# aleju/face-generator

Hardware: NVIDIA H100
Metric: 32x32 GAN train images/sec (1 D-iter + 1 G-iter per batch, batch 256/GPU) (higher is better)
Workload: dtype f32

## Files before the change

face_generator_b200/csrc/capi.cu:

```cuda
#include <algorithm>
#include <cstdarg>
#include <cstdlib>
#include <cstring>

#include "fg_internal.h"
#include "k_conv_tc.h"

static thread_local char g_err[1024] = "";
void fg_set_error(const char* fmt, ...) {
  va_list ap;
  va_start(ap, fmt);
  vsnprintf(g_err, sizeof(g_err), fmt, ap);
  va_end(ap);
}

#define ENTER(c)                                      \
  do {                                                \
    if (!(c)) {                                       \
      fg_set_error("null fg_ctx");                    \
      return FG_ERR_INVALID;                          \
    }                                                 \
    FG_CUDA(cudaSetDevice((c)->device));              \
  } while (0)

bool fg_is_dev(const void* p) {
  cudaPointerAttributes a;
  if (cudaPointerGetAttributes(&a, p) != cudaSuccess) {
    cudaGetLastError();
    return false;
  }
  return a.type == cudaMemoryTypeDevice || a.type == cudaMemoryTypeManaged;
}
int fg_to_dev(fg_ctx* c, const float* p, size_t n, float* staging, const float** out) {
  if (fg_is_dev(p)) {
    *out = p;
    return FG_OK;
  }
  FG_CUDA(cudaMemcpyAsync(staging, p, n * sizeof(float), cudaMemcpyHostToDevice, c->stream));
  *out = staging;
  return FG_OK;
}
int fg_to_user(fg_ctx* c, float* dst, const float* src_dev, size_t n) {
  if (dst == src_dev) return FG_OK;
  const bool dev = fg_is_dev(dst);
  FG_CUDA(cudaMemcpyAsync(dst, src_dev, n * sizeof(float), dev ? cudaMemcpyDeviceToDevice : cudaMemcpyDeviceToHost,
                          c->stream));
  if (!dev) FG_CUDA(cudaStreamSynchronize(c->stream));
  return FG_OK;
}
int64_t debug_tensor_copy(fg_ctx* c, const char* what, const DebugTensor* ents, size_t n_ents, const char* name, float* dst,
                          int64_t max_elems) {
  for (size_t i = 0; i < n_ents; ++i) {
    const DebugTensor& e = ents[i];
    if (strcmp(e.name, name)) continue;
    const int64_t n = e.per * e.B;
    if (!e.p) {
      fg_set_error("%s: '%s' has not been produced (Dstep.*: option \"debug_keep\" + a train step)", what, name);
      return -1;
    }
    if (dst) {
      if (n > max_elems) return -2;
      if (fg_to_user(c, dst, e.p, n) != FG_OK) return -3;
    }
    return n;
  }
  fg_set_error("%s: unknown tensor '%s'", what, name);
  return -1;
}

namespace {
int ctx_alloc(fg_ctx* c) {
  const size_t B = c->maxB, C = c->C;
  auto dalloc = [c](auto** p, size_t n) { return fg_dalloc(c, c->allocs, reinterpret_cast<float**>(p), n); };
  FG_TRY(dalloc(&c->lop_sx, 2));
  FG_TRY(dalloc(&c->lop_sy, 2));
  FG_TRY(dalloc(&c->seed_dev, 2 * kMaxIters));
  c->splitk_ws_elems = (size_t)c->sm_count * 4 * 128 * 128;
  FG_TRY(dalloc(&c->splitk_ws, c->splitk_ws_elems));
  c->red_ws_elems = (size_t)4 << 20;
  FG_TRY(dalloc(&c->red_ws, 2 * c->red_ws_elems));
  FG_TRY(dalloc(&c->red_ws_opt, 2 * kOptRedRows));
  FG_TRY(dalloc(&c->red_ticket, 2));
  FG_TRY(dalloc(&c->bwd_claim, 1));
  FG_TRY(dalloc(&c->small_ws, (size_t)kSmallMaxParts * 9 * 4 * 128));
  FG_TRY(dalloc(&c->bn_acc, 4 * 256 * 2));
  FG_TRY(dalloc(&c->bn_slice_acc, 32 * 4 * 256 * 2 + 64));
  FG_TRY(dalloc(&c->bn_parts, B * 3072));
  c->io_dev_elems = std::max<size_t>(B * 1024 * C, B * kMaskPerSample);
  return dalloc(&c->io_dev, c->io_dev_elems);
}
void ctx_free(fg_ctx* c) {
  for (void* p : c->allocs) cudaFree(p);
  c->allocs.clear();
  for (int i = 0; i < 8; ++i)
    if (c->scratch[i]) cudaFree(c->scratch[i]);
}
}

extern "C" {

const char* fg_version(void) { return "fg_b200 0.1 (sm_90a)"; }
const char* fg_last_error(void) { return g_err; }

void fg_hyper_default(fg_hyper* h) {
  if (!h) return;
  h->lr_D = 1e-3f; h->lr_G = 1e-3f;
  h->beta1 = 0.9f; h->beta2 = 0.999f; h->eps = 1e-8f;
  h->D_L1 = 0.f; h->D_L2 = 1e-4f;
  h->G_L1 = 0.f; h->G_L2 = 0.f;
  h->D_clamp = 1.f; h->G_clamp = 5.f;
  h->D_maxAcc = 1.01f;
  h->accs_interval = 20;
  h->p_spatial = 0.2f; h->p_drop = 0.5f;
}

int fg_create(fg_ctx** out, int device, int max_batch, int channels) {
  if (!out) { fg_set_error("fg_create: out is null"); return FG_ERR_INVALID; }
  *out = nullptr;
  FG_REQUIRE(channels == 1 || channels == 3, "fg_create: channels must be 1 or 3 (got %d)", channels);
  FG_REQUIRE(max_batch >= 4 && max_batch % 2 == 0, "fg_create: max_batch must be even and >= 4 (got %d)", max_batch);
  int ndev = 0;
  FG_CUDA(cudaGetDeviceCount(&ndev));
  FG_REQUIRE(device >= 0 && device < ndev, "fg_create: device %d not present (%d CUDA devices); there is no CPU fallback",
             device, ndev);
  FG_CUDA(cudaSetDevice(device));
  cudaDeviceProp prop;
  FG_CUDA(cudaGetDeviceProperties(&prop, device));
  if (prop.major != 9 || prop.minor != 0) {
    fg_set_error("fg_create: device %d is sm_%d%d; this library only contains sm_90a code", device, prop.major, prop.minor);
    return FG_ERR_UNSUPPORTED;
  }
  fg_ctx* c = new fg_ctx();
  c->device = device;
  c->maxB = max_batch;
  c->C = channels;
  c->sm_count = prop.multiProcessorCount;
  if (const char* e = getenv("FG_MMA_F16")) c->mma_f16 = atoi(e) != 0;
  if (const char* e = getenv("FG_DP_OVERLAP")) c->dp_overlap = atoi(e) != 0;
  if (cudaStreamCreateWithFlags(&c->stream, cudaStreamNonBlocking) != cudaSuccess) {
    fg_set_error("fg_create: cudaStreamCreate failed");
    delete c;
    return FG_ERR_CUDA;
  }
  int r = ctx_alloc(c);
  if (r == FG_OK) r = net32_alloc(c);
  if (r == FG_OK) r = tc_init(c);
  if (r != FG_OK) {
    net32_free(c);
    ctx_free(c);
    cudaStreamDestroy(c->stream);
    delete c;
    return r;
  }
  *out = c;
  return FG_OK;
}

int fg_destroy(fg_ctx* c) {
  if (!c) return FG_OK;
  cudaSetDevice(c->device);
  cudaStreamSynchronize(c->stream);
  if (c->comm_stream) {
    cudaStreamSynchronize(c->comm_stream);
    cudaStreamDestroy(c->comm_stream);
    cudaEventDestroy(c->ev_fork);
    cudaEventDestroy(c->ev_join);
  }
  tc_destroy(c);
  net32_free(c);
  ctx_free(c);
  for (auto& kv : c->timers)
    for (auto& pr : kv.second.pending) {
      cudaEventDestroy(pr.first);
      cudaEventDestroy(pr.second);
    }
  if (c->own_stream && c->stream) cudaStreamDestroy(c->stream);
  delete c;
  return FG_OK;
}

int fg_set_stream(fg_ctx* c, void* s) {
  ENTER(c);
  c->graph_epoch++;
  FG_CUDA(cudaStreamSynchronize(c->stream));
  if (s) {
    if (c->own_stream) cudaStreamDestroy(c->stream);
    c->stream = (cudaStream_t)s;
    c->own_stream = false;
  } else if (!c->own_stream) {
    FG_CUDA(cudaStreamCreateWithFlags(&c->stream, cudaStreamNonBlocking));
    c->own_stream = true;
  }
  return FG_OK;
}
int fg_sync(fg_ctx* c) {
  ENTER(c);
  FG_CUDA(cudaStreamSynchronize(c->stream));
  return FG_OK;
}
int fg_set_option(fg_ctx* c, const char* key, int64_t v) {
  ENTER(c);
  c->graph_epoch++;
  if (!strcmp(key, "conv_impl")) {
    FG_REQUIRE(v >= 0 && v <= 2, "conv_impl must be 0 (simt), 1 (tc dense) or 2 (tc collapsed)");
    c->conv_impl = (int)v;
    return FG_OK;
  }
  if (!strcmp(key, "params_dirty")) {
    NetPair& p = net32_pair(c);
    p.G_pack = p.D_pack = -1;
// ... 185 lines not shown
```

face_generator_b200/csrc/convl.cu:

```cuda
#include "convl.h"

#include "k_conv_tc.h"
#include "k_misc.h"

int convl_dalloc(ConvLEnv& e, float** p, size_t elems) { return fg_dalloc(e.c, *e.allocs, p, elems); }

int ScalePairs::alloc(fg_ctx* c, std::vector<void*>& allocs, int pairs) {
  n = pairs;
  used = 0;
  return fg_dalloc(c, allocs, &base, 2 * (size_t)pairs);
}
int ScalePairs::take(float** pair) {
  if (used == n) {
    fg_set_error("a block of %d FP16 scale pairs is full", n);
    return FG_ERR_UNSUPPORTED;
  }
  *pair = base + 2 * used++;
  return FG_OK;
}
int ScalePairs::reset(fg_ctx* c) const {
  if (!tc_f16(c)) return FG_OK;
  FG_CUDA(cudaMemset2DAsync(base, 2 * sizeof(float), 0, sizeof(float), n, c->stream));
  return FG_OK;
}

namespace {
inline bool tc_f(const fg_ctx* c, const ConvL& L, int B) { return c->conv_impl != FG_CONV_SIMT && tc_conv_eligible(L.geom_k(B)); }
inline bool tc_d(const fg_ctx* c, const ConvL& L, int B) { return c->conv_impl != FG_CONV_SIMT && tc_conv_eligible(L.geom_d(B)); }
inline bool tc_w(const fg_ctx* c, const ConvL& L, int B) { return tc_f(c, L, B) && L.Cout % 128 == 0 && L.geom_k(B).Cin % 64 == 0; }
}

bool convl_tc_fwd(const fg_ctx* c, const ConvL& L) { return tc_f(c, L, 1); }
bool convl_tc_bwd(const fg_ctx* c, const ConvL& L) { return tc_f(c, L, 1) && tc_d(c, L, 1); }

int tc_op_split(fg_ctx* c, TcOp& op, const float* x, int64_t n, bool f16) {
  if (!f16) {
    if (op.split_ready) {
      op.split_ready = false;
      return FG_OK;
    }
    return tc_split(c, x, op.hi, op.lo, n);
  }
  if (op.amax_ready) op.amax_ready = false;
  else FG_TRY(tc_amax(c, x, n, op.s));
  return tc_split_h(c, x, op.hi, op.lo, n, op.s);
}

int convl_alloc(ConvLEnv& e, ConvL& L) {
  const size_t nw = (size_t)L.k * L.k * L.Cout * L.Cin;
  FG_TRY(convl_dalloc(e, &L.Wp, nw));
  FG_TRY(convl_dalloc(e, &L.Wpd, nw));
  if (L.nA) FG_TRY(convl_dalloc(e, &L.bp, L.Cout));
  if (!L.x.s) FG_TRY(convl_dalloc(e, &L.x.s, 2));
  if (!e.dy.s) FG_TRY(convl_dalloc(e, &e.dy.s, 2));
  if (tc_conv_eligible(L.geom_k(e.maxB))) {
    const int K = L.geom_k(e.maxB).Cin;
    const size_t nk = (size_t)L.k * L.k * L.Cout * K, nx = (size_t)e.maxB * L.H * L.H * K;
    FG_TRY(convl_dalloc(e, &L.Wf_hi, nk));
    FG_TRY(convl_dalloc(e, &L.Wf_lo, nk));
    FG_TRY(convl_dalloc(e, &L.x.hi, nx));
    FG_TRY(convl_dalloc(e, &L.x.lo, nx));
    if (L.kpad) {
      FG_TRY(convl_dalloc(e, &L.Wpad, nk));
      FG_TRY(convl_dalloc(e, &L.xpad, nx));
    }
  }
  if (L.need_dgrad && tc_conv_eligible(L.geom_d(e.maxB))) {
    FG_TRY(convl_dalloc(e, &L.Wd_hi, nw));
    FG_TRY(convl_dalloc(e, &L.Wd_lo, nw));
  }
  const int B = e.maxB;
  if (L.pad_out && !(tc_conv_eligible(ConvGeom{B, L.H, L.H, L.Cin, L.pad_out, L.k, 1}) &&
                     tc_conv_eligible(ConvGeom{B, L.H, L.H, L.pad_out, L.Cin, L.k, 1}) && L.Cin % 128 == 0))
    L.pad_out = 0;
  if (L.pad_dy && !(L.x.hi && tc_conv_eligible(ConvGeom{B, L.H, L.H, L.Cin, L.pad_dy, L.k, 1}) && L.Cin % 64 == 0))
    L.pad_dy = 0;
  if (L.pad_out) {
    const size_t nq = (size_t)L.k * L.k * L.pad_out * L.Cin;
    FG_TRY(convl_dalloc(e, &L.Wq_hi, nq));
    FG_TRY(convl_dalloc(e, &L.Wq_lo, nq));
    const size_t nx = (size_t)B * L.H * L.H * L.Cin;
    FG_TRY(convl_dalloc(e, &L.x.hi, nx));
    FG_TRY(convl_dalloc(e, &L.x.lo, nx));
  }
  return FG_OK;
}

int convl_pack(fg_ctx* c, ConvL& L, const float* P) {
  const int KK = L.k * L.k;
  const bool tc_on = c->conv_impl != FG_CONV_SIMT;
  const bool h = tc_on && tc_f16(c) && L.geom_k(1).Cin % 64 == 0 && (L.Cout % 64 == 0 || L.pad_out);
  L.packed_f16 = h;
  if (KK > 1 && tc_on && !L.nA && !L.cA && !L.pad_out && !L.kpad && L.Wf_hi && (L.Wd_hi || !L.need_dgrad) && tc_f(c, L, 1) &&
      (!L.need_dgrad || tc_d(c, L, 1))) {
    if (h) return tc_pack_split_h(c, P + L.w_off, L.Wf_hi, L.Wf_lo, L.Wd_hi, L.Wd_lo, L.Cout, L.Cin, KK);
    return tc_pack_split(c, P + L.w_off, L.Wf_hi, L.Wf_lo, L.Wd_hi, L.Wd_lo, L.Cout, L.Cin, KK);
  }
  FG_TRY(k_pack_weights(c, P + L.w_off, L.Wp, L.need_dgrad ? L.Wpd : nullptr, L.Cout, L.Cin, KK, L.nA, L.nS, L.cA, L.cS));
  if (L.bp) FG_TRY(k_pack_weights(c, P + L.b_off, L.bp, nullptr, L.Cout, 1, 1, L.nA, L.nS, 0, 0));
  if (!tc_on) return FG_OK;
  if (L.kpad && L.Wf_hi) {
    FG_CUDA(cudaMemcpy2DAsync(L.Wpad, L.kpad * sizeof(float), L.Wp, L.Cin * sizeof(float), L.Cin * sizeof(float), L.Cout,
                              cudaMemcpyDeviceToDevice, c->stream));
    if (h) return tc_split_h(c, L.Wpad, L.Wf_hi, L.Wf_lo, (int64_t)L.Cout * L.kpad);
    return tc_split(c, L.Wpad, L.Wf_hi, L.Wf_lo, (int64_t)L.Cout * L.kpad);
  }
  const int64_t nw = (int64_t)KK * L.Cout * L.Cin;
  if (h) {
    if (L.Wf_hi) FG_TRY(tc_split_h(c, L.Wp, L.Wf_hi, L.Wf_lo, nw));
    if (L.Wd_hi) FG_TRY(tc_split_h(c, L.Wpd, L.Wd_hi, L.Wd_lo, nw));
    if (L.pad_out) FG_TRY(k_pack_pad_split_h(c, P + L.w_off, L.Wq_hi, L.Wq_lo, L.Cout, L.pad_out, L.Cin, KK));
    return FG_OK;
  }
  if (L.Wf_hi) FG_TRY(tc_split(c, L.Wp, L.Wf_hi, L.Wf_lo, nw));
  if (L.Wd_hi) FG_TRY(tc_split(c, L.Wpd, L.Wd_hi, L.Wd_lo, nw));
  if (L.pad_out) FG_TRY(k_pack_pad_split(c, P + L.w_off, L.Wq_hi, L.Wq_lo, L.Cout, L.pad_out, L.Cin, KK));
  return FG_OK;
}

int convl_fwd(ConvLEnv& e, ConvL& L, const float* in, const float* P, float* out, int B) {
  fg_ctx* c = e.c;
  const ConvGeom g = L.geom(B);
  const float* bias = L.bp ? L.bp : P + L.b_off;
  const bool h = L.packed_f16;
  const float* os = h ? L.x.s + 1 : nullptr;
  if (L.pad_out && c->conv_impl != FG_CONV_SIMT) {
    FG_TRY(tc_op_split(c, L.x, in, (int64_t)B * L.H * L.H * L.Cin, h));
    {
      ScopedTimer t(c, L.tf);
      FG_TRY(tc_conv_fwd(c, L.x.hi, L.x.lo, L.Wq_hi, L.Wq_lo, nullptr, e.ga, ConvGeom{B, L.H, L.H, L.Cin, L.pad_out, L.k, 1}, 0,
                         nullptr, nullptr, h, os));
    }
    return k_compact_bias(c, e.ga, bias, out, (int64_t)B * L.H * L.H, L.Cout, L.pad_out);
  }
  if (tc_f(c, L, B)) {
    const ConvGeom gk = L.geom_k(B);
    if (L.kpad) {
      FG_CUDA(cudaMemcpy2DAsync(L.xpad, L.kpad * sizeof(float), in, L.Cin * sizeof(float), L.Cin * sizeof(float), (size_t)B * L.H * L.H,
                                cudaMemcpyDeviceToDevice, c->stream));
      in = L.xpad;
    }
    FG_TRY(tc_op_split(c, L.x, in, (int64_t)B * L.H * L.H * gk.Cin, h));
    ScopedTimer t(c, L.tf);
    return tc_conv_fwd(c, L.x.hi, L.x.lo, L.Wf_hi, L.Wf_lo, bias, out, gk, 0, nullptr, nullptr, h, os);
  }
  ScopedTimer t(c, L.tf);
  if (c->edge_impl && k_edge_eligible(g)) return k_conv_edge(c, in, L.Wp, bias, out, g);
  return k_small_eligible(g) ? k_conv_small(c, in, L.Wp, bias, out, g) : k_conv_simt(c, in, L.Wp, bias, out, g);
}

int convl_bwd(ConvLEnv& e, ConvL& L, const float* in, const float* dy, float* G, float* din, int B) {
  fg_ctx* c = e.c;
  const ConvGeom g = L.geom(B), gd = L.geom_d(B);
  const bool w_tc = G && tc_w(c, L, B), d_tc = din && tc_d(c, L, B);
  const bool h = L.packed_f16;
  float* sdy = L.sdy ? L.sdy : e.dy.s;
  const bool split_ready = e.dy.split_ready, amax_ready = e.dy.amax_ready, bias_ready = e.dy.bias_ready;
  e.dy.split_ready = e.dy.amax_ready = e.dy.bias_ready = false;
  const float *osy = h ? sdy + 1 : nullptr, *osx = h ? L.x.s + 1 : nullptr;
  const bool tc_on = c->conv_impl != FG_CONV_SIMT;
  const int64_t P = (int64_t)B * L.H * L.H;
  if (h && !amax_ready && (w_tc || d_tc || (G && tc_on && (L.pad_out || L.pad_dy)))) FG_TRY(tc_amax(c, dy, P * L.Cout, sdy));
  if (w_tc || d_tc) {
    if (h) FG_TRY(tc_split_h(c, dy, e.dy.hi, e.dy.lo, P * L.Cout, sdy));
    else if (!split_ready) FG_TRY(tc_split(c, dy, e.dy.hi, e.dy.lo, P * L.Cout));
  }
  if (G && tc_on && L.pad_out) {
    if (h) FG_TRY(k_pad_split_h(c, dy, e.pad.hi, e.pad.lo, P, L.Cout, L.pad_out, sdy));
    else FG_TRY(k_pad_split(c, dy, e.pad.hi, e.pad.lo, P, L.Cout, L.pad_out));
    {
      ScopedTimer t(c, L.tw);
      FG_TRY(tc_conv_wgrad(c, e.pad.hi, e.pad.lo, L.x.hi, L.x.lo, e.ws, ConvGeom{B, L.H, L.H, L.pad_out, L.Cin, L.k, 1}, h, osy, osx));
    }
    FG_TRY(k_unpack_wgrad_swapped(c, e.ws, G + L.w_off, L.Cout, L.pad_out, L.Cin, L.k * L.k));
    if (!bias_ready) FG_TRY(k_colsum_add(c, dy, G + L.b_off, P, L.Cout, 0, 0));
  } else if (G && tc_on && L.pad_dy && !w_tc) {
    if (h) FG_TRY(k_pad_split_h(c, dy, e.pad.hi, e.pad.lo, P, L.Cout, L.pad_dy, sdy));
    else FG_TRY(k_pad_split(c, dy, e.pad.hi, e.pad.lo, P, L.Cout, L.pad_dy));
    {
      ScopedTimer t(c, L.tw);
      FG_TRY(tc_conv_wgrad(c, L.x.hi, L.x.lo, e.pad.hi, e.pad.lo, e.ws, ConvGeom{B, L.H, L.H, L.Cin, L.pad_dy, L.k, 1}, h, osy, osx));
    }
    FG_TRY(k_unpack_wgrad_pad(c, e.ws, G + L.w_off, L.Cout, L.pad_dy, L.Cin, L.k * L.k));
    if (!bias_ready) FG_TRY(k_colsum_add(c, dy, G + L.b_off, P, L.Cout, 0, 0));
  } else if (G) {
    const int64_t koff = L.kpad && w_tc ? (int64_t)L.Cout * L.Cin : 0;
    {
      ScopedTimer t(c, L.tw);
// ... 101 lines not shown
```

face_generator_b200/csrc/convl.h:

```cpp
#pragma once
#include <vector>

#include "fg_internal.h"

inline bool tc_f16(const fg_ctx* c) { return c->mma_f16 && c->conv_impl == FG_CONV_TC_COLLAPSED; }

struct AmaxInto {
  fg_ctx* c;
  AmaxInto(fg_ctx* c_, TcOp& op) : AmaxInto(c_, op.s, &op.amax_ready) {}
  AmaxInto(fg_ctx* c_, float* pair, bool* done) : c(c_) {
    if (tc_f16(c)) {
      c->amax_out = reinterpret_cast<unsigned*>(pair);
      c->amax_done = done;
    }
  }
  ~AmaxInto() { c->amax_out = nullptr; }
};

inline unsigned* take_amax(fg_ctx* c) {
  unsigned* p = c->amax_out;
  if (p) *c->amax_done = true;
  return p;
}

int tc_op_split(fg_ctx* c, TcOp& op, const float* x, int64_t n, bool f16);

inline int pack_key(const fg_ctx* c) { return c->conv_impl | (c->mma_f16 << 4); }
int convl_dalloc(ConvLEnv& e, float** p, size_t elems);
int convl_alloc(ConvLEnv& e, ConvL& L);
bool convl_tc_fwd(const fg_ctx* c, const ConvL& L);
bool convl_tc_bwd(const fg_ctx* c, const ConvL& L);
int convl_pack(fg_ctx* c, ConvL& L, const float* P);
int convl_fwd(ConvLEnv& e, ConvL& L, const float* in, const float* P, float* out, int B);
int convl_bwd(ConvLEnv& e, ConvL& L, const float* in, const float* dy, float* G, float* din, int B);

bool upsl_tc(const fg_ctx* c, const UpsL& U);
int upsl_alloc(ConvLEnv& e, UpsL& U);
int upsl_pack(fg_ctx* c, UpsL& U, const float* P);
int upsl_fwd(ConvLEnv& e, UpsL& U, const float* h, const float* P, float* z, int B, int* parts = nullptr);
int upsl_bwd(ConvLEnv& e, UpsL& U, TcOp& dy, const float* h, const float* dz, float* G, float* dh, int B, bool* pooled);

int gen_alloc(ConvLEnv& e, UpsGen& G, const GenDesc& d);
int gen_pack(fg_ctx* c, UpsGen& G, NetPair& p);
int gen_forward(ConvLEnv& e, UpsGen& G, NetPair& p, const float* noise, int B, bool training);
int gen_backward(ConvLEnv& e, UpsGen& G, NetPair& p, const float* dy, float* dnoise);
void gen_debug_rows(const UpsGen& G, std::vector<DebugTensor>& rows);
```

face_generator_b200/csrc/fg_internal.h:

```cpp
#pragma once
#include <cuda_runtime.h>
#include <cstdint>
#include <cstdio>
#include <deque>
#include <functional>
#include <initializer_list>
#include <map>
#include <string>
#include <vector>

#include "fg_b200.h"

void fg_set_error(const char* fmt, ...);

#define FG_CUDA(call)                                                                               \
  do {                                                                                              \
    cudaError_t e__ = (call);                                                                       \
    if (e__ != cudaSuccess) {                                                                       \
      fg_set_error("%s:%d: %s -> %s", __FILE__, __LINE__, #call, cudaGetErrorString(e__));          \
      return FG_ERR_CUDA;                                                                           \
    }                                                                                               \
  } while (0)
#define FG_TRY(call)                  \
  do {                                \
    int r__ = (call);                 \
    if (r__ != FG_OK) return r__;     \
  } while (0)
#define FG_REQUIRE(cond, ...)         \
  do {                                \
    if (!(cond)) {                    \
      fg_set_error(__VA_ARGS__);      \
      return FG_ERR_INVALID;          \
    }                                 \
  } while (0)
#define LAUNCH_CHECK(c)                 \
  do {                                  \
    (c)->launches++;                    \
    FG_CUDA(cudaGetLastError());        \
  } while (0)
inline int grid_for(int64_t n, int block, int cap = 132 * 16) {
  int64_t g = (n + block - 1) / block;
  if (g > cap) g = cap;
  if (g < 1) g = 1;
  return (int)g;
}
#define GRID_STRIDE(i, n) \
  for (int64_t i = blockIdx.x * (int64_t)blockDim.x + threadIdx.x; i < (n); i += (int64_t)gridDim.x * blockDim.x)

constexpr int kMaskPerSample = 1984;
constexpr int kNoiseDim = 100;
constexpr int kSmallMaxParts = 2048;
constexpr int kGradTail = 8;
constexpr int kOptRedRows = 132 * 2;

struct ConvGeom {
  int B, H, W, Cin, Cout, k, ups;
};

struct GLayout {
  int64_t L1W, L1b, a1, C1W, C1b, g1, be1, a2, C2W, C2b, g2, be2, a3, C3W, C3b, total;
};
GLayout make_g_layout(int C, int side);

struct DeviceStats {
  float loss_D, loss_G;
  int conf[4];
  int trained_D;
  int t_D, t_G;
  float acc_D;
  int acc_count, acc_head;
  float step_D, step_G;
  int do_train_D, do_train_G;
};
constexpr int kAccHistMax = 1024;
constexpr int kMaxIters = 16;
constexpr int kBnState = 768;

struct StepGraph {
  std::vector<uint8_t> key;
  cudaGraphExec_t exec = nullptr;
  int64_t launches = 0;
  bool failed = false;
};

struct NetPair {
  int64_t nG = 0, nD = 0;
  float *PG = nullptr, *PD = nullptr, *gG = nullptr, *gD = nullptr;
  float *tailG = nullptr, *tailD = nullptr;
  float *mG = nullptr, *vG = nullptr, *mD = nullptr, *vD = nullptr;
  float* bnG = nullptr;
  DeviceStats* dstats = nullptr;
  DeviceStats* hstats = nullptr;
  float* acc_hist = nullptr;
  int G_pack = -1, D_pack = -1;
  std::vector<StepGraph> graphs;
  const char* optim_timer[2] = {nullptr, nullptr};
  struct Keep {
    const char* name;
    const float* src;
    int64_t per;
    float* copy = nullptr;
  };
  std::vector<Keep> keep;
  int keep_B = 0;
};

struct ScalePairs {
  float* base = nullptr;
  int n = 0, used = 0;
  int alloc(fg_ctx* c, std::vector<void*>& allocs, int pairs);
  int take(float** pair);
  int reset(fg_ctx* c) const;
};

struct TcOp {
  float *hi = nullptr, *lo = nullptr;
  float* s = nullptr;
  bool split_ready = false, amax_ready = false, bias_ready = false;
};
struct ConvL {
  int Cin = 0, Cout = 0, k = 1, H = 1;
  int64_t w_off = 0, b_off = 0;
  int cA = 0, cS = 0;
  int nA = 0, nS = 0;
  float *Wp = nullptr, *Wpd = nullptr;
  float* bp = nullptr;
  float *Wf_hi = nullptr, *Wf_lo = nullptr, *Wd_hi = nullptr, *Wd_lo = nullptr;
  TcOp x;
  float* sdy = nullptr;
  int kpad = 0;
  float *xpad = nullptr, *Wpad = nullptr;
  bool packed_f16 = false;
  int pad_out = 0, pad_dy = 0;
  float *Wq_hi = nullptr, *Wq_lo = nullptr;
  bool need_dgrad = true;
  const char *tf = "", *td = "", *tw = "";
  ConvGeom geom(int B) const { return ConvGeom{B, H, H, Cin, Cout, k, 1}; }
  ConvGeom geom_k(int B) const { return ConvGeom{B, H, H, kpad ? kpad : Cin, Cout, k, 1}; }
  ConvGeom geom_d(int B) const { return ConvGeom{B, H, H, Cout, Cin, k, 1}; }
};

struct UpsL {
  int Cin = 0, Cout = 0, H = 0;
  int64_t w_off = 0, b_off = 0;
  float *Wp = nullptr, *Wpd = nullptr;
  float *Wf_hi = nullptr, *Wf_lo = nullptr, *Wd_hi = nullptr, *Wd_lo = nullptr;
  float *Wx_hi = nullptr, *Wx_lo = nullptr;
  TcOp x;
  const char *tf = "", *td = "", *tw = "", *tb = nullptr;
  ConvGeom geom(int B) const { return ConvGeom{B, H, H, Cin, Cout, 5, 2}; }
};

struct ConvLEnv {
  fg_ctx* c = nullptr;
  int maxB = 0;
  std::vector<void*>* allocs = nullptr;
  float *ga = nullptr;
  TcOp dy;
  TcOp pad;
  float* ws = nullptr;
};

struct GenDesc {
  int side;
  const char* prefix;
  int l1_kpad;
  bool bwd_merge;
};

struct UpsGen {
  int S = 32, C = 3;
  GLayout gl;
  ConvL GL1, GC3;
  UpsL GU[2];
  ScalePairs pairs;
  float* sdz[2] = {nullptr, nullptr};
  float *noise = nullptr, *z0 = nullptr, *h0 = nullptr, *z1 = nullptr, *h1 = nullptr, *z2 = nullptr, *h2 = nullptr,
        *z3 = nullptr, *y = nullptr;
  float *dz3 = nullptr, *dfull = nullptr, *dz2 = nullptr, *dz1 = nullptr, *dz0 = nullptr;
  float *bn_mean[2] = {nullptr, nullptr}, *bn_istd[2] = {nullptr, nullptr}, *bn_mg = nullptr;
  int B = 0;
  bool train = true, valid = false;
  std::deque<std::string> names;
  const char *t_bn2_finalize = nullptr, *t_bn2_stats = nullptr, *t_bn2_apply = nullptr, *t_bn2_bwd_reduce = nullptr,
             *t_bn2_bwd_apply = nullptr;
};

struct TimerRec {
  double ms = 0;
  int64_t launches = 0;
  std::vector<std::pair<cudaEvent_t, cudaEvent_t>> pending;
};

struct IterStage {
  float* p[8] = {};
  size_t cap[8] = {};
  int reserve(fg_ctx* c, std::vector<void*>& allocs, int k, size_t n);
  int in(fg_ctx* c, std::vector<void*>& allocs, int k, const float* p, size_t n, size_t cap_n, const float** out);
};

struct Net32;

struct fg_ctx {
  int device = 0, maxB = 0, C = 3;
  cudaStream_t stream = nullptr;
  bool own_stream = true;
  int64_t launches = 0;
  int conv_impl = FG_CONV_TC_COLLAPSED;
  int sm_count = 132;
  int opt_D = 0, opt_G = 0;
  float sgd_mom_D = 0.f, sgd_mom_G = 0.f;
  std::vector<void*> allocs;
  Net32* n32 = nullptr;
  float* small_ws = nullptr;
  float* splitk_ws = nullptr;
  size_t splitk_ws_elems = 0;
  double* red_ws = nullptr;
  size_t red_ws_elems = 0;
  double* red_ws_opt = nullptr;
  unsigned* red_ticket = nullptr;
  double* bn_slice_acc = nullptr;
  float* bn_parts = nullptr;
  int edge_impl = 1;
  int bn_epilogue = 1;
  int mma_f16 = 1;
  float* lop_sx = nullptr;
  float* lop_sy = nullptr;
  unsigned* amax_out = nullptr;
  bool* amax_done = nullptr;
  double* bn_acc = nullptr;
  float* io_dev = nullptr;
  size_t io_dev_elems = 0;
  float* scratch[8] = {nullptr, nullptr, nullptr, nullptr, nullptr, nullptr, nullptr, nullptr};
  size_t scratch_elems[8] = {0, 0, 0, 0, 0, 0, 0, 0};
  void* nccl_comm = nullptr;
  int world = 1, rank = 0;
  int dp_overlap = 1;
  int reserve_sms = 0;
  int last_conv_kind = 0, last_conv_tile_m = 0, last_conv_tile_n = 0, last_conv_format = 0, last_conv_splits = 0;
  int bwd_merge = 1, bwd_merge_ctas = 0;
  int* bwd_claim = nullptr;
  int use_graph = 1, graph_epoch = 0;
  uint64_t* seed_dev = nullptr;
  cudaStream_t comm_stream = nullptr;
  cudaEvent_t ev_fork = nullptr, ev_join = nullptr;
  bool debug_keep = false;
  cudaEvent_t events[16] = {};
  bool timing = false;
  std::map<std::string, TimerRec> timers;
};

inline void note_conv(fg_ctx* c, int kind, int tile_m, int tile_n, int format, int splits) {
  c->last_conv_kind = kind;
  c->last_conv_tile_m = tile_m;
  c->last_conv_tile_n = tile_n;
  c->last_conv_format = format;
  c->last_conv_splits = splits;
}

struct ScopedTimer {
  fg_ctx* c;
  TimerRec* rec = nullptr;
  cudaEvent_t e0 = nullptr, e1 = nullptr;
  ScopedTimer(fg_ctx* c_, const char* name) : c(c_) {
    if (c->timing && name) {
      rec = &c->timers[name];
      cudaEventCreate(&e0);
      cudaEventCreate(&e1);
      cudaEventRecord(e0, c->stream);
    }
  }
  ~ScopedTimer() {
    if (rec) {
      cudaEventRecord(e1, c->stream);
      rec->pending.emplace_back(e0, e1);
    }
  }
};

int k_fill(fg_ctx* c, float* p, float v, int64_t n);
int k_nchw_to_nhwc(fg_ctx* c, const float* src, float* dst, int B, int C, int HW);
int k_nhwc_to_nchw(fg_ctx* c, const float* src, float* dst, int B, int C, int HW);
int k_pack_weights(fg_ctx* c, const float* W, float* Wp, float* Wpd, int N, int Cc, int KK, int nA, int nS, int cA,
                   int cS);
int k_unpack_wgrad(fg_ctx* c, const float* dWp, float* dW, int N, int Cc, int KK, int nA, int nS, int cA, int cS);
int k_colsum_add(fg_ctx* c, const float* X, float* out, int64_t P, int N, int nA, int nS);
int k_prelu_fwd(fg_ctx* c, const float* z, const float* slope, float* h, int64_t n);
int k_prelu_bwd(fg_ctx* c, const float* dh, const float* z, const float* slope, float* dz, float* dslope, int B, int H,
                int W, int C, int pool);
int k_bn_stats(fg_ctx* c, const float* z, double* acc2C, int64_t P, int C);
bool k_bn4_ok(int C);
int k_bn_stats4(fg_ctx* c, const float* z, double* acc, int64_t P, int C);
int k_bn_bwd_reduce4(fg_ctx* c, const float* dh, const float* z, const float* mean, const float* istd, const float* gamma,
                     const float* beta, const float* slope, double* acc, float* dslope, int64_t P, int C);
int k_bn_finalize(fg_ctx* c, double* acc2C, float* mean, float* istd, float* run_mean, float* run_var, int64_t P,
                  int C);
int k_bn_finalize_parts(fg_ctx* c, const float* part, int nparts, int nphase, float* mean, float* istd, float* run_mean,
                        float* run_var, int64_t P, int C);
int k_bn_eval_prep(fg_ctx* c, const float* run_mean, const float* run_var, float* mean, float* istd, int C);
int k_bn_prelu_apply(fg_ctx* c, const float* z, const float* mean, const float* istd, const float* gamma,
                     const float* beta, const float* slope, float* h, int64_t P, int C, float* hi = nullptr,
                     float* lo = nullptr);
int k_bn_prelu_bwd_reduce(fg_ctx* c, const float* dh, const float* z, const float* mean, const float* istd,
                          const float* gamma, const float* beta, const float* slope, double* acc2C, float* dslope,
                          int B, int H, int W, int C, int pool);
int k_bn_bwd_finalize(fg_ctx* c, double* acc2C, float* mg2C, float* dgamma, float* dbeta, int64_t P, int C);
int k_bn_prelu_bwd_apply(fg_ctx* c, const float* dh, const float* z, const float* mean, const float* istd,
                         const float* gamma, const float* beta, const float* slope, const float* mg2C, float* dz,
                         int B, int H, int W, int C, int pool, float* hi = nullptr, float* lo = nullptr,
                         float* dbias = nullptr);
int k_sigmoid_fwd(fg_ctx* c, const float* z, float* y, int64_t n);
int k_sigmoid_bwd(fg_ctx* c, const float* dy, const float* y, float* dz, int64_t n);
int k_masks_generate(fg_ctx* c, float* masks, int B, uint64_t seed, float p_spatial, float p_drop,
                     const uint64_t* seed_dev = nullptr);
int k_set_u64(fg_ctx* c, uint64_t* dst, uint64_t v);
int k_seed_roots(fg_ctx* c, uint64_t* roots, int n);
int k_d_act_pool_fwd(fg_ctx* c, const float* z, const float* slope, const float* masks, int moff, float eval_scale,
                     float* p, int B, int H, int W, int C, float* hi = nullptr, float* lo = nullptr);
int k_d_act_pool_bwd(fg_ctx* c, const float* dp, const float* z, const float* slope, const float* masks, int moff,
                     float eval_scale, float* dz, float* dslope, int B, int H, int W, int C, float* hi = nullptr,
                     float* lo = nullptr, float* dbias = nullptr);
int k_lin_act_drop_fwd(fg_ctx* c, const float* z, const float* slope, const float* masks, int moff, float scale,
                       float* h, int B, int N);
int k_lin_act_drop_bwd(fg_ctx* c, const float* dh, const float* z, const float* slope, const float* masks, int moff,
                       float scale, float* dz, float* dslope, int B, int N);
int k_sigmoid_bce(fg_ctx* c, const float* logit, float* out, float* dlogit, float* loss_out, float* tail4, int B,
                  int n_ones);
int k_bce_fwd(fg_ctx* c, const float* x, const float* t, int n, float* loss_out);
int k_bce_bwd(fg_ctx* c, const float* x, const float* t, int n, float* dx);
int k_sigmoid_grad_mul(fg_ctx* c, const float* dout, const float* out, float* dlogit, int n);
int k_penalty_loss(fg_ctx* c, const float* p, int64_t n, float l1, float l2, float* loss_inout);
int k_gate_and_prep(fg_ctx* c, DeviceStats* st, float* acc_hist, int net, const fg_hyper* h, const float* tail4, int B,
                    float world, bool accumulate = false);
int k_optim_prep(fg_ctx* c, DeviceStats* st, int net, const fg_hyper* h);
int k_gemv_fwd(fg_ctx* c, const float* x, const float* w, const float* bias, float* out, int B, int K);
int k_gemv_dgrad(fg_ctx* c, const float* dy, const float* w, float* dx, int B, int K);
int k_gemv_wgrad_add(fg_ctx* c, const float* x, const float* dy, float* dw, float* db, int B, int K);
int k_adam(fg_ctx* c, float* p, const float* g, float* m, float* v, int64_t n, float beta1, float beta2, float eps,
           float l1_grad, float l2, float clampv, float grad_scale, const float* step_dev, const int* flag_dev,
           float step_host, float* g_out);
int k_optim_update(fg_ctx* c, int mode, float* p, float* g, float* m, float* v, int64_t n, float beta1, float beta2, float eps,
                   float mom, float l1_grad, float l2, float clampv, float grad_scale, const float* step_dev,
                   const int* flag_dev, const int* t_dev);

int k_conv_simt(fg_ctx* c, const float* in, const float* Wp, const float* bias, float* out, ConvGeom g);
int k_wgrad_simt(fg_ctx* c, const float* in, const float* dY, float* dWp, ConvGeom g);
bool k_small_eligible(const ConvGeom& g);
int k_conv_small(fg_ctx* c, const float* in, const float* Wp, const float* bias, float* out, ConvGeom g);
int k_wgrad_small(fg_ctx* c, const float* in, const float* dY, float* dWp, ConvGeom g);

bool k_edge_eligible(const ConvGeom& g);
int k_conv_edge(fg_ctx* c, const float* in, const float* Wp, const float* bias, float* out, ConvGeom g);

inline int red_check(fg_ctx* c, int64_t rows, int64_t n) {
  if (rows * n > (int64_t)c->red_ws_elems) {
    fg_set_error("ordered reduction of %lld x %lld partials exceeds its workspace", (long long)rows, (long long)n);
    return FG_ERR_UNSUPPORTED;
  }
  return FG_OK;
}
int k_splitk_reduce(fg_ctx* c, const float* parts, int splits, int64_t n, float* out);

int tc_init(fg_ctx* c);
void tc_destroy(fg_ctx* c);

int net32_alloc(fg_ctx* c);
void net32_free(fg_ctx* c);
NetPair& net32_pair(fg_ctx* c);

int net_allreduce(fg_ctx* c, float* buf, int64_t n);
int net_broadcast(fg_ctx* c, void* buf, size_t bytes);
int net_group(bool start);

int fg_dalloc(fg_ctx* c, std::vector<void*>& allocs, float** p, size_t n);
int pair_alloc(fg_ctx* c, std::vector<void*>& allocs, NetPair& p, int64_t nG, int64_t nD, bool bn);
void pair_clear_graphs(NetPair& p);
void pair_free(NetPair& p);
int pair_zero_grads(fg_ctx* c, NetPair& p, int net);
int pair_allreduce_grads(fg_ctx* c, NetPair& p, int net);
int pair_gate(fg_ctx* c, NetPair& p, int net, const fg_hyper* h, int B, float world, bool accumulate = false);
int pair_optim(fg_ctx* c, NetPair& p, int net, const fg_hyper* h, float grad_scale);
int k_adam_prep(fg_ctx* c, int* t_dev, float* step_dev, float lr, float beta1, float beta2);
int pair_broadcast(fg_ctx* c, NetPair& p);
int pair_step_stats(fg_ctx* c, const NetPair& p, fg_step_stats* stats);
int pair_set_params(fg_ctx* c, NetPair& p, int net, const float* src);
int pair_get_params(fg_ctx* c, const NetPair& p, int net, float* dst);
int pair_get_grads(fg_ctx* c, const NetPair& p, int net, float* dst);
int pair_set_adam_state(fg_ctx* c, NetPair& p, int net, const float* m, const float* v, int t);
int pair_get_adam_state(fg_ctx* c, const NetPair& p, int net, float* m, float* v, int* t);
int pair_set_bn_state(fg_ctx* c, NetPair& p, const float* src);
int pair_get_bn_state(fg_ctx* c, const NetPair& p, float* dst);
int net_graph_run(fg_ctx* c, NetPair& p, int B, const void* hyper, size_t hyper_bytes, std::initializer_list<const void*> inputs,
                  uint64_t seed, const std::function<int()>& body, int nd = 1, int ng = 1);

int step_check(fg_ctx* c, const char* what, int B, int nd, int ng, bool inputs, const fg_dataset* d = nullptr, bool fed = false);
struct StepNets {
  StepNets(fg_ctx* c, NetPair& pair, const fg_hyper* h, int B, float* logit, float* out, float* dlogit, float* masks,
           int64_t mask, bool gate, bool overlap)
      : c(c), pair(&pair), h(h), B(B), logit(logit), out(out), dlogit(dlogit), masks(masks), mask(mask), gate(gate),
        overlap(overlap) {}
  fg_ctx* c;
  NetPair* pair;
  const fg_hyper* h;
  int B;
  float *logit, *out, *dlogit;
  float* masks;
  int64_t mask;
  bool gate;
  bool overlap;
  virtual int g_forward(int j, bool d_iter) = 0;
  virtual int d_input(int j) = 0;
  virtual int draw_masks(int kind, const uint64_t* root) = 0;
  virtual int d_forward(bool on_g) = 0;
  virtual int d_backward(bool want_wgrad, bool want_dx) = 0;
  virtual int g_backward() = 0;
};
int pair_train_step(StepNets& s, int nd, int ng, const float* masksD, const float* masksG, uint64_t seed,
                    std::initializer_list<const void*> inputs, const std::function<int()>* feed, fg_step_stats* stats);
struct DebugTensor;
void pair_keep_rows(const NetPair& p, std::vector<DebugTensor>& ents);

int k_relu_fwd(fg_ctx* c, const float* z, float* h, int64_t n);
int k_relu_bwd(fg_ctx* c, const float* dh, const float* z, float* dz, int64_t n);
int k_tanh_dropout_fwd(fg_ctx* c, const float* z, const float* masks_in, const uint64_t* seed_dev, float p, float* code, float* h,
                       float* flags_out, int64_t n);
int k_tanh_dropout_bwd(fg_ctx* c, const float* dh, const float* masks, float p, const float* code, float* dz, int64_t n);
int k_abs_criterion(fg_ctx* c, bool sigmoid, const float* z, const float* t, float* y, float* dz, int64_t n, float* loss);

bool fg_is_dev(const void* p);
int fg_to_dev(fg_ctx* c, const float* p, size_t n, float* staging, const float** out);
int fg_to_user(fg_ctx* c, float* dst, const float* src_dev, size_t n);
struct DebugTensor {
  const char* name;
  const float* p;
  int64_t per;
  int B;
};
int64_t debug_tensor_copy(fg_ctx* c, const char* what, const DebugTensor* ents, size_t n_ents, const char* name, float* dst,
                          int64_t max_elems);

struct JpegScratch;
void jpeg_scratch_free(JpegScratch* s);
struct fg_dataset {
  fg_ctx* c = nullptr;
  int64_t N = 0;
  int Cs = 3, Hs = 64, Ws = 64;
  uint8_t* data = nullptr;
  int32_t* idx = nullptr;
  JpegScratch* jpeg = nullptr;
};
int dataset_check_feed(const fg_dataset* d, const fg_ctx* c, const char* what);
int dataset_draw_gather(fg_dataset* d, uint64_t seed, int B, int size, float* out_dev, const uint64_t* root = nullptr,
                        uint64_t kinds = 0);
int dataset_draw_gather_c2f(fg_dataset* d, uint64_t seed, int B, int fine_size, int coarse_size, float* fine, float* coarse,
                            float* diff, const uint64_t* root = nullptr, uint64_t kinds = 0);
int noise_uniform_dev(fg_ctx* c, uint64_t seed, int64_t n, float* out_dev, const uint64_t* root = nullptr, uint64_t kinds = 0);
```

face_generator_b200/csrc/gen.cu:

```cuda
#include "convl.h"

GLayout make_g_layout(int C, int side) {
  const int64_t n0 = 128 * (side / 4) * (side / 4);
  GLayout L;
  int64_t o = 0;
  L.L1W = o; o += n0 * kNoiseDim;
  L.L1b = o; o += n0;
  L.a1 = o; o += 1;
  L.C1W = o; o += 256 * 128 * 25;
  L.C1b = o; o += 256;
  L.g1 = o; o += 256;
  L.be1 = o; o += 256;
  L.a2 = o; o += 1;
  L.C2W = o; o += 128 * 256 * 25;
  L.C2b = o; o += 128;
  L.g2 = o; o += 128;
  L.be2 = o; o += 128;
  L.a3 = o; o += 1;
  L.C3W = o; o += (int64_t)C * 128 * 9;
  L.C3b = o; o += C;
  L.total = o;
  return L;
}

int gen_alloc(ConvLEnv& e, UpsGen& G, const GenDesc& d) {
  fg_ctx* c = e.c;
  const int S = d.side, C = c->C;
  G.S = S;
  G.C = C;
  G.gl = make_g_layout(C, S);
  const GLayout& gl = G.gl;
  auto timer = [&](const char* name) {
    G.names.push_back(std::string(d.prefix) + name);
    return G.names.back().c_str();
  };
  FG_TRY(G.pairs.alloc(c, *e.allocs, 8));
  ConvL& L1 = G.GL1;
  L1.Cin = kNoiseDim; L1.Cout = 128 * (S / 4) * (S / 4); L1.k = 1; L1.H = 1;
  L1.w_off = gl.L1W; L1.b_off = gl.L1b;
  L1.nA = 128; L1.nS = (S / 4) * (S / 4);
  L1.kpad = d.l1_kpad;
  L1.tf = timer("G.L1.fwd"); L1.td = timer("G.L1.dgrad"); L1.tw = timer("G.L1.wgrad");
  ConvL& C3 = G.GC3;
  C3.Cin = 128; C3.Cout = C; C3.k = 3; C3.H = S;
  C3.w_off = gl.C3W; C3.b_off = gl.C3b;
  C3.tf = timer("G.C3.fwd"); C3.td = timer("G.C3.dgrad"); C3.tw = timer("G.C3.wgrad");
  for (ConvL* L : {&L1, &C3}) {
    FG_TRY(G.pairs.take(&L->x.s));
    FG_TRY(G.pairs.take(&L->sdy));
    FG_TRY(convl_alloc(e, *L));
  }
  static const char* uf[2] = {"G.C1.fwd", "G.C2.fwd"};
  static const char* ud[2] = {"G.C1.dgrad", "G.C2.dgrad"};
  static const char* uw[2] = {"G.C1.wgrad", "G.C2.wgrad"};
  static const char* ub[2] = {"G.C1.wgrad+dgrad", "G.C2.wgrad+dgrad"};
  const int ci[2] = {128, 256}, co[2] = {256, 128}, hs[2] = {S / 2, S};
  const int64_t wo[2] = {gl.C1W, gl.C2W}, bo[2] = {gl.C1b, gl.C2b};
  for (int i = 0; i < 2; ++i) {
    UpsL& U = G.GU[i];
    U.Cin = ci[i]; U.Cout = co[i]; U.H = hs[i];
    U.w_off = wo[i]; U.b_off = bo[i];
    U.tf = timer(uf[i]); U.td = timer(ud[i]); U.tw = timer(uw[i]);
    U.tb = d.bwd_merge ? timer(ub[i]) : nullptr;
    FG_TRY(G.pairs.take(&U.x.s));
    FG_TRY(G.pairs.take(&G.sdz[i]));
    FG_TRY(upsl_alloc(e, U));
  }
  G.t_bn2_finalize = timer("G.bn2.finalize");
  G.t_bn2_stats = timer("hbm.G.bn2.stats");
  G.t_bn2_apply = timer("hbm.G.bn2.apply");
  G.t_bn2_bwd_reduce = timer("hbm.G.bn2.bwd_reduce");
  G.t_bn2_bwd_apply = timer("hbm.G.bn2.bwd_apply");
  const size_t B = e.maxB, n0 = L1.Cout, n1 = (size_t)256 * (S / 2) * (S / 2), n2 = (size_t)128 * S * S, n3 = (size_t)C * S * S;
  for (auto [p, n] : {std::pair<float**, size_t>{&G.noise, kNoiseDim}, {&G.z0, n0}, {&G.h0, n0}, {&G.z1, n1}, {&G.h1, n1},
                      {&G.z2, n2}, {&G.h2, n2}, {&G.z3, n3}, {&G.y, n3}, {&G.dz3, n3},
                      {&G.dfull, (size_t)256 * S * S},
                      {&G.dz2, n2}, {&G.dz1, n1}, {&G.dz0, n0}})
    FG_TRY(convl_dalloc(e, p, B * n));
  for (int i = 0; i < 2; ++i) {
    FG_TRY(convl_dalloc(e, &G.bn_mean[i], co[i]));
    FG_TRY(convl_dalloc(e, &G.bn_istd[i], co[i]));
  }
  return convl_dalloc(e, &G.bn_mg, 512);
}

int gen_pack(fg_ctx* c, UpsGen& G, NetPair& p) {
  if (p.G_pack == pack_key(c)) return FG_OK;
  FG_TRY(convl_pack(c, G.GL1, p.PG));
  for (int i = 0; i < 2; ++i) FG_TRY(upsl_pack(c, G.GU[i], p.PG));
  FG_TRY(convl_pack(c, G.GC3, p.PG));
  p.G_pack = pack_key(c);
  return FG_OK;
}

namespace {
int bn_stats(fg_ctx* c, UpsGen& G, NetPair& p, int i, const float* z, int B, bool training, int parts, const char* t_finalize,
             const char* t_stats) {
  const int Cc = G.GU[i].Cout;
  const int64_t P = (int64_t)B * G.GU[i].H * G.GU[i].H;
  float *rm = p.bnG + (i == 0 ? 0 : 512), *rv = rm + Cc;
  if (!training) return k_bn_eval_prep(c, rm, rv, G.bn_mean[i], G.bn_istd[i], Cc);
  if (parts) {
    ScopedTimer tm(c, t_finalize);
    return k_bn_finalize_parts(c, c->bn_parts, parts, 4, G.bn_mean[i], G.bn_istd[i], rm, rv, P, Cc);
  }
  {
    ScopedTimer tm(c, t_stats);
    FG_TRY(k_bn_stats(c, z, c->bn_acc, P, Cc));
  }
  return k_bn_finalize(c, c->bn_acc, G.bn_mean[i], G.bn_istd[i], rm, rv, P, Cc);
}
}

int gen_forward(ConvLEnv& e, UpsGen& G, NetPair& p, const float* noise, int B, bool training) {
  fg_ctx* c = e.c;
  FG_REQUIRE(B >= 1 && B <= e.maxB, "G forward: batch %d out of range [1,%d]", B, e.maxB);
  FG_TRY(gen_pack(c, G, p));
  const GLayout& L = G.gl;
  const float* P = p.PG;
  const int S = G.S;
  if (noise != G.noise)
    FG_CUDA(cudaMemcpyAsync(G.noise, noise, sizeof(float) * B * kNoiseDim, cudaMemcpyDeviceToDevice, c->stream));
  G.B = B;
  G.train = training;
  FG_TRY(G.pairs.reset(c));
  FG_TRY(convl_fwd(e, G.GL1, G.noise, P, G.z0, B));
  {
    AmaxInto am(c, G.GU[0].x);
    FG_TRY(k_prelu_fwd(c, G.z0, P + L.a1, G.h0, (int64_t)B * G.GL1.Cout));
  }
  int parts = training ? 1 : 0;
  FG_TRY(upsl_fwd(e, G.GU[0], G.h0, P, G.z1, B, &parts));
  FG_TRY(bn_stats(c, G, p, 0, G.z1, B, training, parts, nullptr, nullptr));
  UpsL& C2 = G.GU[1];
  C2.x.split_ready = training && upsl_tc(c, C2) && !tc_f16(c);
  {
    AmaxInto am(c, C2.x);
    FG_TRY(k_bn_prelu_apply(c, G.z1, G.bn_mean[0], G.bn_istd[0], P + L.g1, P + L.be1, P + L.a2, G.h1,
                            (int64_t)B * (S / 2) * (S / 2), 256, C2.x.split_ready ? C2.x.hi : nullptr,
                            C2.x.split_ready ? C2.x.lo : nullptr));
  }
  parts = training ? 1 : 0;
  FG_TRY(upsl_fwd(e, C2, G.h1, P, G.z2, B, &parts));
  FG_TRY(bn_stats(c, G, p, 1, G.z2, B, training, parts, G.t_bn2_finalize, G.t_bn2_stats));
  {
    ScopedTimer tm(c, G.t_bn2_apply);
    FG_TRY(k_bn_prelu_apply(c, G.z2, G.bn_mean[1], G.bn_istd[1], P + L.g2, P + L.be2, P + L.a3, G.h2, (int64_t)B * S * S, 128));
  }
  FG_TRY(convl_fwd(e, G.GC3, G.h2, P, G.z3, B));
  FG_TRY(k_sigmoid_fwd(c, G.z3, G.y, (int64_t)B * S * S * G.C));
  G.valid = true;
  return FG_OK;
}

int gen_backward(ConvLEnv& e, UpsGen& G, NetPair& p, const float* dy, float* dnoise) {
  fg_ctx* c = e.c;
  if (!G.valid || !G.train) {
    fg_set_error("G backward needs a preceding training-mode G forward");
    return FG_ERR_STATE;
  }
  const GLayout& L = G.gl;
  const float* P = p.PG;
  float* g = p.gG;
  const int B = G.B, S = G.S, h = S / 2;
  FG_TRY(G.pairs.reset(c));
  FG_TRY(k_sigmoid_bwd(c, dy, G.y, G.dz3, (int64_t)B * S * S * G.C));
  FG_TRY(convl_bwd(e, G.GC3, G.h2, G.dz3, g, G.dfull, B));
  {
    ScopedTimer tm(c, G.t_bn2_bwd_reduce);
    FG_TRY(k_bn_prelu_bwd_reduce(c, G.dfull, G.z2, G.bn_mean[1], G.bn_istd[1], P + L.g2, P + L.be2, P + L.a3, c->bn_acc,
                                 g + L.a3, B, S, S, 128, 0));
  }
  FG_TRY(k_bn_bwd_finalize(c, c->bn_acc, G.bn_mg, g + L.g2, g + L.be2, (int64_t)B * S * S, 128));
  const bool tf32 = !tc_f16(c);
  TcOp dz2{e.dy.hi, e.dy.lo, G.sdz[1]};
  dz2.split_ready = upsl_tc(c, G.GU[1]) && tf32;
  {
    ScopedTimer tm(c, G.t_bn2_bwd_apply);
    AmaxInto am(c, dz2);
    FG_TRY(k_bn_prelu_bwd_apply(c, G.dfull, G.z2, G.bn_mean[1], G.bn_istd[1], P + L.g2, P + L.be2, P + L.a3, G.bn_mg, G.dz2,
                                B, S, S, 128, 0, dz2.split_ready ? dz2.hi : nullptr, dz2.split_ready ? dz2.lo : nullptr,
                                g + L.C2b));
  }
  bool pooled = false;
  FG_TRY(upsl_bwd(e, G.GU[1], dz2, G.h1, G.dz2, g, G.dfull, B, &pooled));
  FG_TRY(k_bn_prelu_bwd_reduce(c, G.dfull, G.z1, G.bn_mean[0], G.bn_istd[0], P + L.g1, P + L.be1, P + L.a2, c->bn_acc,
                               g + L.a2, B, h, h, 256, pooled ? 0 : 1));
  FG_TRY(k_bn_bwd_finalize(c, c->bn_acc, G.bn_mg, g + L.g1, g + L.be1, (int64_t)B * h * h, 256));
  TcOp dz1{e.dy.hi, e.dy.lo, G.sdz[0]};
  dz1.split_ready = upsl_tc(c, G.GU[0]) && tf32 && pooled;
  {
    AmaxInto am(c, dz1);
    FG_TRY(k_bn_prelu_bwd_apply(c, G.dfull, G.z1, G.bn_mean[0], G.bn_istd[0], P + L.g1, P + L.be1, P + L.a2, G.bn_mg, G.dz1,
                                B, h, h, 256, pooled ? 0 : 1, dz1.split_ready ? dz1.hi : nullptr,
                                dz1.split_ready ? dz1.lo : nullptr, g + L.C1b));
  }
  FG_TRY(upsl_bwd(e, G.GU[0], dz1, G.h0, G.dz1, g, G.dfull, B, &pooled));
  {
    AmaxInto am(c, G.GL1.sdy, &e.dy.amax_ready);
    FG_TRY(k_prelu_bwd(c, G.dfull, G.z0, P + L.a1, G.dz0, g + L.a1, B, S / 4, S / 4, 128, pooled ? 0 : 1));
  }
  return convl_bwd(e, G.GL1, G.noise, G.dz0, g, dnoise, B);
}

void gen_debug_rows(const UpsGen& G, std::vector<DebugTensor>& rows) {
  const int64_t n0 = G.GL1.Cout, n1 = 256 * (G.S / 2) * (G.S / 2), n2 = 128 * G.S * G.S, n3 = (int64_t)G.C * G.S * G.S;
  const int B = G.B;
  for (const DebugTensor& r : {DebugTensor{"G.z0", G.z0, n0, B}, {"G.h0", G.h0, n0, B}, {"G.z1", G.z1, n1, B},
                               {"G.h1", G.h1, n1, B}, {"G.z2", G.z2, n2, B}, {"G.h2", G.h2, n2, B}, {"G.z3", G.z3, n3, B},
                               {"G.y", G.y, n3, B}, {"G.dz2", G.dz2, n2, B}, {"G.dz1", G.dz1, n1, B}, {"G.dz0", G.dz0, n0, B},
                               {"G.bn_mean1", G.bn_mean[0], 256, 1}, {"G.bn_istd1", G.bn_istd[0], 256, 1},
                               {"G.bn_mean2", G.bn_mean[1], 128, 1}, {"G.bn_istd2", G.bn_istd[1], 128, 1}})
    rows.push_back({r.name, G.valid ? r.p : nullptr, r.per, r.B});
}
```

face_generator_b200/csrc/k_bn.cu:

```cuda
#include "fg_internal.h"
#include "k_ordered.cuh"

namespace {
template <bool BWD>
__global__ void __launch_bounds__(256) bn_reduce4_kernel(const float* __restrict__ z, const float* __restrict__ dh,
                                                         const float* __restrict__ mean, const float* __restrict__ istd,
                                                         const float* __restrict__ gamma, const float* __restrict__ beta,
                                                         const float* __restrict__ slope, double* __restrict__ acc,
                                                         float* __restrict__ dslope, int64_t P, int C,
                                                         int64_t rows_per_block, double* __restrict__ ws,
                                                         unsigned* __restrict__ ticket) {
  extern __shared__ double sm[];
  const int C4 = C >> 2;
  const int lanes = blockDim.x / C4;
  const int c4 = threadIdx.x % C4, lane = threadIdx.x / C4;
  const int ch = c4 * 4;
  const int64_t r0 = blockIdx.x * rows_per_block, r1 = min(P, r0 + rows_per_block);
  const float4* z4 = reinterpret_cast<const float4*>(z);
  const float4* d4 = reinterpret_cast<const float4*>(dh);
  double s[4] = {0, 0, 0, 0}, q[4] = {0, 0, 0, 0}, ss = 0;
  float m[4], is[4], ga[4], be[4];
  float a = 1.f;
  bool act = false;
  if (BWD) {
#pragma unroll
    for (int j = 0; j < 4; ++j) {
      m[j] = mean[ch + j];
      is[j] = istd[ch + j];
      ga[j] = gamma[ch + j];
      be[j] = beta[ch + j];
    }
    act = slope != nullptr;
    if (act) a = *slope;
  }
  if (lane < lanes) {
    int64_t r = r0 + lane;
    if (!BWD) {
      for (; r + 3 * (int64_t)lanes < r1; r += 4 * (int64_t)lanes) {
        const float4 v0 = z4[r * C4 + c4], v1 = z4[(r + lanes) * C4 + c4], v2 = z4[(r + 2 * (int64_t)lanes) * C4 + c4],
                     v3 = z4[(r + 3 * (int64_t)lanes) * C4 + c4];
        const float a[4][4] = {{v0.x, v0.y, v0.z, v0.w}, {v1.x, v1.y, v1.z, v1.w}, {v2.x, v2.y, v2.z, v2.w}, {v3.x, v3.y, v3.z, v3.w}};
#pragma unroll
        for (int j = 0; j < 4; ++j) {
          s[j] += ((double)a[0][j] + (double)a[1][j]) + ((double)a[2][j] + (double)a[3][j]);
          q[j] += (double)a[0][j] * (double)a[0][j] + (double)a[1][j] * (double)a[1][j] + (double)a[2][j] * (double)a[2][j] +
                  (double)a[3][j] * (double)a[3][j];
        }
      }
    }
    auto bwd_row = [&](const float4& v, const float4& d) {
      const float zv[4] = {v.x, v.y, v.z, v.w};
      const float dv[4] = {d.x, d.y, d.z, d.w};
#pragma unroll
      for (int j = 0; j < 4; ++j) {
        const float xh = (zv[j] - m[j]) * is[j];
        float g = dv[j];
        if (act) {
          const float u = ga[j] * xh + be[j];
          if (!(u > 0.f)) {
            g = a * dv[j];
            ss += (double)dv[j] * (double)u;
          }
        }
        s[j] += (double)g;
        q[j] += (double)g * (double)xh;
      }
    };
    if (BWD) {
      for (; r + lanes < r1; r += 2 * (int64_t)lanes) {
        const float4 v0 = z4[r * C4 + c4], d0 = d4[r * C4 + c4], v1 = z4[(r + lanes) * C4 + c4], d1 = d4[(r + lanes) * C4 + c4];
        bwd_row(v0, d0);
        bwd_row(v1, d1);
      }
    }
    for (; r < r1; r += lanes) {
      const float4 v = z4[r * C4 + c4];
      if (!BWD) {
        const float zv[4] = {v.x, v.y, v.z, v.w};
#pragma unroll
        for (int j = 0; j < 4; ++j) {
          s[j] += (double)zv[j];
          q[j] += (double)zv[j] * (double)zv[j];
        }
      } else {
        bwd_row(v, d4[r * C4 + c4]);
      }
    }
  }
  double* s0 = sm;
  double* s1 = sm + (size_t)lanes * C;
  if (lane < lanes) {
#pragma unroll
    for (int j = 0; j < 4; ++j) {
      s0[lane * C + ch + j] = s[j];
      s1[lane * C + ch + j] = q[j];
    }
  }
  __syncthreads();
  double* row = ws + (int64_t)blockIdx.x * (2 * C + 1);
  for (int i = threadIdx.x; i < C; i += blockDim.x) {
    double a0 = 0, a1 = 0;
    for (int l = 0; l < lanes; ++l) {
      a0 += s0[l * C + i];
      a1 += s1[l * C + i];
    }
    row[i] = a0;
    row[C + i] = a1;
  }
  if (threadIdx.x == 0) row[2 * C] = 0.0;
  if (BWD && act && dslope) {
    __shared__ double red[32];
    __syncthreads();
#pragma unroll
    for (int o = 16; o > 0; o >>= 1) ss += __shfl_xor_sync(0xffffffffu, ss, o);
    if ((threadIdx.x & 31) == 0) red[threadIdx.x >> 5] = ss;
    __syncthreads();
    if (threadIdx.x < 32) {
      double v = threadIdx.x < (blockDim.x >> 5) ? red[threadIdx.x] : 0.0;
#pragma unroll
      for (int o = 16; o > 0; o >>= 1) v += __shfl_xor_sync(0xffffffffu, v, o);
      if (threadIdx.x == 0) row[2 * C] = v;
    }
  }
  if (ordered_last_block(ticket)) {
    for (int i = threadIdx.x; i < 2 * C; i += blockDim.x) acc[i] += ordered_sum(ws, gridDim.x, 2 * C + 1, i);
    if (BWD && dslope && threadIdx.x == 0) *dslope += (float)ordered_sum(ws, gridDim.x, 2 * C + 1, 2 * C);
    ordered_release(ticket);
  }
}
}

bool k_bn4_ok(int C) { return C % 4 == 0 && C >= 16 && C <= 1024 && 256 % (C / 4) == 0; }

int k_bn_stats4(fg_ctx* c, const float* z, double* acc, int64_t P, int C) {
  FG_CUDA(cudaMemsetAsync(acc, 0, sizeof(double) * 2 * C, c->stream));
  const int lanes = 256 / (C / 4);
  int grid = (int)std::min<int64_t>((int64_t)c->sm_count * 8, (P + lanes * 4 - 1) / (lanes * 4));
  if (grid < 1) grid = 1;
  const int64_t rpb = (P + grid - 1) / grid;
  FG_TRY(red_check(c, grid, 2 * C + 1));
  bn_reduce4_kernel<false><<<grid, 256, sizeof(double) * 2 * lanes * C, c->stream>>>(z, nullptr, nullptr, nullptr, nullptr, nullptr,
                                                                                   nullptr, acc, nullptr, P, C, rpb, c->red_ws,
                                                                                   c->red_ticket);
  LAUNCH_CHECK(c);
  return FG_OK;
}
int k_bn_bwd_reduce4(fg_ctx* c, const float* dh, const float* z, const float* mean, const float* istd, const float* gamma,
                     const float* beta, const float* slope, double* acc, float* dslope, int64_t P, int C) {
  FG_CUDA(cudaMemsetAsync(acc, 0, sizeof(double) * 2 * C, c->stream));
  const int lanes = 256 / (C / 4);
  int grid = (int)std::min<int64_t>((int64_t)c->sm_count * 8, (P + lanes * 4 - 1) / (lanes * 4));
  if (grid < 1) grid = 1;
  const int64_t rpb = (P + grid - 1) / grid;
  FG_TRY(red_check(c, grid, 2 * C + 1));
  bn_reduce4_kernel<true><<<grid, 256, sizeof(double) * 2 * lanes * C, c->stream>>>(z, dh, mean, istd, gamma, beta, slope, acc,
                                                                                  dslope, P, C, rpb, c->red_ws, c->red_ticket);
  LAUNCH_CHECK(c);
  return FG_OK;
}
```

face_generator_b200/csrc/k_elem.cu:

```cuda
#include <cmath>

#include "convl.h"
#include "fg_internal.h"
#include "k_f16split.cuh"
#include "k_ordered.cuh"

__device__ __forceinline__ int perm_idx(int j, int A, int S) {
  if (A == 0) return j;
  return (j % S) * A + (j / S);
}

__device__ __forceinline__ double warp_sum(double v) {
#pragma unroll
  for (int o = 16; o > 0; o >>= 1) v += __shfl_xor_sync(0xffffffffu, v, o);
  return v;
}
__device__ __forceinline__ double block_sum(double v) {
  __shared__ double red[32];
  __syncthreads();
  v = warp_sum(v);
  if ((threadIdx.x & 31) == 0) red[threadIdx.x >> 5] = v;
  __syncthreads();
  if (threadIdx.x < 32) {
    v = threadIdx.x < (blockDim.x + 31) / 32 ? red[threadIdx.x] : 0.0;
    v = warp_sum(v);
  }
  return v;
}

__global__ void fill_kernel(float* p, float v, int64_t n) {
  for (int64_t i = blockIdx.x * (int64_t)blockDim.x + threadIdx.x; i < n; i += (int64_t)gridDim.x * blockDim.x) p[i] = v;
}
int k_fill(fg_ctx* c, float* p, float v, int64_t n) {
  if (n <= 0) return FG_OK;
  fill_kernel<<<grid_for(n, 256), 256, 0, c->stream>>>(p, v, n);
  LAUNCH_CHECK(c);
  return FG_OK;
}

__global__ void nchw_to_nhwc_kernel(const float* __restrict__ src, float* __restrict__ dst, int B, int C, int HW) {
  const int64_t n = (int64_t)B * C * HW;
  for (int64_t i = blockIdx.x * (int64_t)blockDim.x + threadIdx.x; i < n; i += (int64_t)gridDim.x * blockDim.x) {
    const int ch = (int)(i % C);
    const int64_t r = i / C;
    const int p = (int)(r % HW);
    const int b = (int)(r / HW);
    dst[i] = src[((int64_t)b * C + ch) * HW + p];
  }
}
__global__ void nhwc_to_nchw_kernel(const float* __restrict__ src, float* __restrict__ dst, int B, int C, int HW) {
  const int64_t n = (int64_t)B * C * HW;
  for (int64_t i = blockIdx.x * (int64_t)blockDim.x + threadIdx.x; i < n; i += (int64_t)gridDim.x * blockDim.x) {
    const int p = (int)(i % HW);
    const int64_t r = i / HW;
    const int ch = (int)(r % C);
    const int b = (int)(r / C);
    dst[i] = src[((int64_t)b * HW + p) * C + ch];
  }
}
int k_nchw_to_nhwc(fg_ctx* c, const float* src, float* dst, int B, int C, int HW) {
  nchw_to_nhwc_kernel<<<grid_for((int64_t)B * C * HW, 256), 256, 0, c->stream>>>(src, dst, B, C, HW);
  LAUNCH_CHECK(c);
  return FG_OK;
}
int k_nhwc_to_nchw(fg_ctx* c, const float* src, float* dst, int B, int C, int HW) {
  nhwc_to_nchw_kernel<<<grid_for((int64_t)B * C * HW, 256), 256, 0, c->stream>>>(src, dst, B, C, HW);
  LAUNCH_CHECK(c);
  return FG_OK;
}

__global__ void pack_weights_kernel(const float* __restrict__ W, float* __restrict__ Wp, float* __restrict__ Wpd, int N,
                                    int Cc, int KK, int nA, int nS, int cA, int cS) {
  const int64_t total = (int64_t)N * Cc * KK;
  for (int64_t i = blockIdx.x * (int64_t)blockDim.x + threadIdx.x; i < total; i += (int64_t)gridDim.x * blockDim.x) {
    const int t = (int)(i % KK);
    const int64_t r = i / KK;
    const int ch = (int)(r % Cc);
    const int n = (int)(r / Cc);
    const int n2 = perm_idx(n, nA, nS), c2 = perm_idx(ch, cA, cS);
    const float w = W[i];
    if (Wp) Wp[((int64_t)t * N + n2) * Cc + c2] = w;
    if (Wpd) Wpd[((int64_t)(KK - 1 - t) * Cc + c2) * N + n2] = w;
  }
}
int k_pack_weights(fg_ctx* c, const float* W, float* Wp, float* Wpd, int N, int Cc, int KK, int nA, int nS, int cA,
                   int cS) {
  pack_weights_kernel<<<grid_for((int64_t)N * Cc * KK, 256), 256, 0, c->stream>>>(W, Wp, Wpd, N, Cc, KK, nA, nS, cA, cS);
  LAUNCH_CHECK(c);
  return FG_OK;
}
__global__ void unpack_wgrad_kernel(const float* __restrict__ dWp, float* __restrict__ dW, int N, int Cc, int KK, int nA,
                                    int nS, int cA, int cS) {
  const int64_t total = (int64_t)N * Cc * KK;
  for (int64_t i = blockIdx.x * (int64_t)blockDim.x + threadIdx.x; i < total; i += (int64_t)gridDim.x * blockDim.x) {
    const int t = (int)(i % KK);
    const int64_t r = i / KK;
    const int ch = (int)(r % Cc);
    const int n = (int)(r / Cc);
    const int n2 = perm_idx(n, nA, nS), c2 = perm_idx(ch, cA, cS);
    dW[i] += dWp[((int64_t)t * N + n2) * Cc + c2];
  }
}
int k_unpack_wgrad(fg_ctx* c, const float* dWp, float* dW, int N, int Cc, int KK, int nA, int nS, int cA, int cS) {
  unpack_wgrad_kernel<<<grid_for((int64_t)N * Cc * KK, 256), 256, 0, c->stream>>>(dWp, dW, N, Cc, KK, nA, nS, cA, cS);
  LAUNCH_CHECK(c);
  return FG_OK;
}

__global__ void colsum_kernel(const float* __restrict__ X, float* __restrict__ out, int64_t P, int N, int nA, int nS,
                              int64_t rows_per_block, double* __restrict__ ws, unsigned* __restrict__ ticket) {
  __shared__ double sm[8][33];
  const int col = blockIdx.x * 32 + threadIdx.x;
  const int64_t r0 = blockIdx.y * rows_per_block;
  const int64_t r1 = min(P, r0 + rows_per_block);
  double s = 0;
  if (col < N)
    for (int64_t r = r0 + threadIdx.y; r < r1; r += 8) s += X[r * N + col];
  sm[threadIdx.y][threadIdx.x] = s;
  __syncthreads();
  if (threadIdx.y == 0 && col < N) {
    double t = 0;
#pragma unroll
    for (int i = 0; i < 8; ++i) t += sm[i][threadIdx.x];
    const int j = nA == 0 ? col : (col % nA) * nS + (col / nA);
    ws[(int64_t)blockIdx.y * N + j] = t;
  }
  if (ordered_last_block(ticket)) {
    for (int j = threadIdx.y * blockDim.x + threadIdx.x; j < N; j += blockDim.x * blockDim.y)
      out[j] += (float)ordered_sum(ws, gridDim.y, N, j);
    ordered_release(ticket);
  }
}
int k_colsum_add(fg_ctx* c, const float* X, float* out, int64_t P, int N, int nA, int nS) {
  int gy = (int)std::min<int64_t>(256, (P + 255) / 256);
  if (gy < 1) gy = 1;
  const int64_t rpb = (P + gy - 1) / gy;
  dim3 grid((N + 31) / 32, gy), block(32, 8);
  FG_TRY(red_check(c, gy, N));
  colsum_kernel<<<grid, block, 0, c->stream>>>(X, out, P, N, nA, nS, rpb, c->red_ws, c->red_ticket);
  LAUNCH_CHECK(c);
  return FG_OK;
}

__global__ void prelu_fwd_kernel(const float* __restrict__ z, const float* __restrict__ slope, float* __restrict__ h,
                                 int64_t n, unsigned* __restrict__ amax) {
  const float a = *slope;
  float am = 0.f;
  for (int64_t i = blockIdx.x * (int64_t)blockDim.x + threadIdx.x; i < n; i += (int64_t)gridDim.x * blockDim.x) {
    const float v = z[i];
    const float o = v > 0.f ? v : a * v;
    h[i] = o;
    am = fmaxf(am, finite_abs(o));
  }
  amax_commit(amax, am);
}
int k_prelu_fwd(fg_ctx* c, const float* z, const float* slope, float* h, int64_t n) {
  prelu_fwd_kernel<<<grid_for(n, 256), 256, 0, c->stream>>>(z, slope, h, n, take_amax(c));
  LAUNCH_CHECK(c);
  return FG_OK;
}

__device__ __forceinline__ float load_dh(const float* __restrict__ dh, int b, int y, int x, int ch, int H, int W, int C,
                                         int pool) {
  if (!pool) return dh[(((int64_t)b * H + y) * W + x) * C + ch];
  const int64_t base = (((int64_t)b * 2 * H + 2 * y) * 2 * W + 2 * x) * C + ch;
  const int64_t rs = (int64_t)2 * W * C;
  return (dh[base] + dh[base + C]) + (dh[base + rs] + dh[base + rs + C]);
}

__global__ void prelu_bwd_kernel(const float* __restrict__ dh, const float* __restrict__ z,
                                 const float* __restrict__ slope, float* __restrict__ dz, float* __restrict__ dslope, int B,
                                 int H, int W, int C, int pool, unsigned* __restrict__ amax, double* __restrict__ ws,
                                 unsigned* __restrict__ ticket) {
  const float a = *slope;
  const int64_t n = (int64_t)B * H * W * C;
  double s = 0;
  float am = 0.f;
  for (int64_t i = blockIdx.x * (int64_t)blockDim.x + threadIdx.x; i < n; i += (int64_t)gridDim.x * blockDim.x) {
    const int ch = (int)(i % C);
    int64_t r = i / C;
    const int x = (int)(r % W);
    r /= W;
    const int y = (int)(r % H);
    const int b = (int)(r / H);
    const float g = load_dh(dh, b, y, x, ch, H, W, C, pool);
    const float v = z[i];
    if (v > 0.f) {
      dz[i] = g;
      am = fmaxf(am, finite_abs(g));
    } else {
      dz[i] = a * g;
      am = fmaxf(am, finite_abs(a * g));
      s += (double)g * (double)v;
    }
  }
  amax_commit(amax, am);
  s = block_sum(s);
  if (!dslope) return;
  if (threadIdx.x == 0) ws[blockIdx.x] = s;
  if (ordered_last_block(ticket)) {
    if (threadIdx.x == 0) *dslope += (float)ordered_sum(ws, gridDim.x, 1, 0);
    ordered_release(ticket);
  }
}
int k_prelu_bwd(fg_ctx* c, const float* dh, const float* z, const float* slope, float* dz, float* dslope, int B, int H,
                int W, int C, int pool) {
  const int64_t n = (int64_t)B * H * W * C;
  prelu_bwd_kernel<<<grid_for(n, 256, 132 * 8), 256, 0, c->stream>>>(dh, z, slope, dz, dslope, B, H, W, C, pool, take_amax(c),
                                                                    c->red_ws, c->red_ticket);
  LAUNCH_CHECK(c);
  return FG_OK;
}

__global__ void bn_stats_kernel(const float* __restrict__ z, double* __restrict__ acc, int64_t P, int C,
                                int64_t rows_per_block, double* __restrict__ ws, unsigned* __restrict__ ticket) {
  extern __shared__ double sm[];
  const int lanes = blockDim.x / C;
  const int ch = threadIdx.x % C, lane = threadIdx.x / C;
  const int64_t r0 = blockIdx.x * rows_per_block, r1 = min(P, r0 + rows_per_block);
  double s = 0, s2 = 0;
  for (int64_t r = r0 + lane; r < r1; r += lanes) {
    const double v = z[r * C + ch];
    s += v;
    s2 += v * v;
  }
  sm[threadIdx.x] = s;
  sm[blockDim.x + threadIdx.x] = s2;
  __syncthreads();
  if (lane == 0) {
    for (int l = 1; l < lanes; ++l) {
      s += sm[l * C + ch];
      s2 += sm[blockDim.x + l * C + ch];
    }
    ws[(int64_t)blockIdx.x * 2 * C + ch] = s;
    ws[(int64_t)blockIdx.x * 2 * C + C + ch] = s2;
  }
  if (ordered_last_block(ticket)) {
    for (int i = threadIdx.x; i < 2 * C; i += blockDim.x) acc[i] += ordered_sum(ws, gridDim.x, 2 * C, i);
    ordered_release(ticket);
  }
}
static inline int bn_block(int C) {
  int lanes = 256 / C;
  if (lanes < 1) lanes = 1;
  return C * lanes;
}
int k_bn_stats(fg_ctx* c, const float* z, double* acc, int64_t P, int C) {
  if (k_bn4_ok(C)) return k_bn_stats4(c, z, acc, P, C);
  if (C > 1024) {
    fg_set_error("BatchNorm with C=%d > 1024 unsupported", C);
    return FG_ERR_UNSUPPORTED;
  }
  FG_CUDA(cudaMemsetAsync(acc, 0, sizeof(double) * 2 * C, c->stream));
  const int block = bn_block(C);
  int grid = (int)std::min<int64_t>(c->sm_count * 4, (P + 63) / 64);
  if (grid < 1) grid = 1;
  const int64_t rpb = (P + grid - 1) / grid;
  FG_TRY(red_check(c, grid, 2 * C));
  bn_stats_kernel<<<grid, block, sizeof(double) * 2 * block, c->stream>>>(z, acc, P, C, rpb, c->red_ws, c->red_ticket);
  LAUNCH_CHECK(c);
  return FG_OK;
}
__global__ void bn_finalize_kernel(const double* __restrict__ acc, float* __restrict__ mean, float* __restrict__ istd,
                                   float* __restrict__ run_mean, float* __restrict__ run_var, int64_t P, int C) {
  const int ch = blockIdx.x * blockDim.x + threadIdx.x;
  if (ch >= C) return;
  const double n = (double)P;
  const double m = acc[ch] / n;
  double var = acc[C + ch] / n - m * m;
  if (var < 0) var = 0;
  mean[ch] = (float)m;
  istd[ch] = (float)(1.0 / sqrt(var + 1e-5));
  if (run_mean) run_mean[ch] = 0.9f * run_mean[ch] + 0.1f * (float)m;
  if (run_var) run_var[ch] = 0.9f * run_var[ch] + 0.1f * (float)(P > 1 ? var * n / (n - 1.0) : var);
}
int k_bn_finalize(fg_ctx* c, double* acc, float* mean, float* istd, float* run_mean, float* run_var, int64_t P, int C) {
  bn_finalize_kernel<<<(C + 127) / 128, 128, 0, c->stream>>>(acc, mean, istd, run_mean, run_var, P, C);
  LAUNCH_CHECK(c);
  return FG_OK;
}
constexpr int kBnSlices = 32;
constexpr double kBnOnePassRatio = 16.0;
__device__ __forceinline__ double bn_tile_count(int i, int nphase, int64_t phase_pixels) {
  return (double)min((int64_t)128, phase_pixels - (int64_t)(i / nphase) * 128);
}
__global__ void __launch_bounds__(256) bn_finalize_parts_kernel(const float* __restrict__ part, int nparts, int nphase,
                                                                double* __restrict__ slice_acc,
                                                                unsigned int* __restrict__ ticket, float* __restrict__ mean,
                                                                float* __restrict__ istd, float* __restrict__ run_mean,
                                                                float* __restrict__ run_var, int64_t P, int C) {
  __shared__ double sm[4][8][32];
  __shared__ bool last;
  const int lane = threadIdx.x & 31, g = threadIdx.x >> 5;
  const int ch = blockIdx.x * 32 + lane;
  const int per = (nparts + kBnSlices - 1) / kBnSlices;
  const int i0 = blockIdx.y * per, i1 = min(nparts, i0 + per);
  const int64_t pp = P / nphase;
  const double r = ch < C ? (double)part[ch] / bn_tile_count(0, nphase, pp) : 0.0;
  double s = 0, q = 0, ds = 0, dq = 0;
  if (ch < C)
    for (int i = i0 + g; i < i1; i += 8) {
      const double si = (double)part[((int64_t)i * 3 + 0) * C + ch];
      s += si;
      q += (double)part[((int64_t)i * 3 + 1) * C + ch];
      const double n = bn_tile_count(i, nphase, pp), d = si - n * r;
      ds += d;
      dq += (double)part[((int64_t)i * 3 + 2) * C + ch] + d * d * (n == 128.0 ? 1.0 / 128 : 1.0 / n);
    }
  sm[0][g][lane] = s;
  sm[1][g][lane] = q;
  sm[2][g][lane] = ds;
  sm[3][g][lane] = dq;
  __syncthreads();
  if (g == 0 && ch < C) {
    for (int k = 1; k < 8; ++k) {
      s += sm[0][k][lane];
      q += sm[1][k][lane];
      ds += sm[2][k][lane];
      dq += sm[3][k][lane];
    }
    slice_acc[((int64_t)blockIdx.y * 4 + 0) * C + ch] = s;
    slice_acc[((int64_t)blockIdx.y * 4 + 1) * C + ch] = q;
    slice_acc[((int64_t)blockIdx.y * 4 + 2) * C + ch] = ds;
    slice_acc[((int64_t)blockIdx.y * 4 + 3) * C + ch] = dq;
  }
  __threadfence();
  __syncthreads();
  if (threadIdx.x == 0) last = atomicAdd(ticket + blockIdx.x, 1u) == (unsigned)kBnSlices - 1;
  __syncthreads();
  if (!last) return;
  __threadfence();
  if (threadIdx.x == 0) ticket[blockIdx.x] = 0;
  if (g != 0 || ch >= C) return;
  s = q = ds = dq = 0;
  for (int k = 0; k < kBnSlices; ++k) {
    s += slice_acc[((int64_t)k * 4 + 0) * C + ch];
    q += slice_acc[((int64_t)k * 4 + 1) * C + ch];
    ds += slice_acc[((int64_t)k * 4 + 2) * C + ch];
    dq += slice_acc[((int64_t)k * 4 + 3) * C + ch];
  }
  const double n = (double)P;
  const double m = s / n;
  double var = q / n - m * m;
  if (var < 0) var = 0;
  if (q / n > kBnOnePassRatio * (var + 1e-5)) var = fmax(0.0, (dq - ds * (ds / n)) / n);
  mean[ch] = (float)m;
  istd[ch] = (float)(1.0 / sqrt(var + 1e-5));
  if (run_mean) run_mean[ch] = 0.9f * run_mean[ch] + 0.1f * (float)m;
  if (run_var) run_var[ch] = 0.9f * run_var[ch] + 0.1f * (float)(P > 1 ? var * n / (n - 1.0) : var);
}
int k_bn_finalize_parts(fg_ctx* c, const float* part, int nparts, int nphase, float* mean, float* istd, float* run_mean,
                        float* run_var, int64_t P, int C) {
  double* acc = c->bn_slice_acc;
  unsigned int* ticket = reinterpret_cast<unsigned int*>(acc + (size_t)kBnSlices * 4 * 256);
  bn_finalize_parts_kernel<<<dim3((C + 31) / 32, kBnSlices), 256, 0, c->stream>>>(part, nparts, nphase, acc, ticket, mean, istd,
                                                                                run_mean, run_var, P, C);
  LAUNCH_CHECK(c);
  return FG_OK;
}
__global__ void bn_eval_prep_kernel(const float* __restrict__ rm, const float* __restrict__ rv, float* __restrict__ mean,
                                    float* __restrict__ istd, int C) {
  const int ch = blockIdx.x * blockDim.x + threadIdx.x;
  if (ch >= C) return;
  mean[ch] = rm[ch];
  istd[ch] = 1.0f / sqrtf(rv[ch] + 1e-5f);
}
int k_bn_eval_prep(fg_ctx* c, const float* rm, const float* rv, float* mean, float* istd, int C) {
  bn_eval_prep_kernel<<<(C + 127) / 128, 128, 0, c->stream>>>(rm, rv, mean, istd, C);
  LAUNCH_CHECK(c);
  return FG_OK;
}
__global__ void bn_prelu_apply_kernel(const float* __restrict__ z, const float* __restrict__ mean,
                                      const float* __restrict__ istd, const float* __restrict__ gamma,
                                      const float* __restrict__ beta, const float* __restrict__ slope,
                                      float* __restrict__ h, float* __restrict__ hi, float* __restrict__ lo, int64_t n4,
                                      int C, unsigned* __restrict__ amax) {
  float am = 0.f;
  const bool act = slope != nullptr;
  const float a = act ? *slope : 1.f;
  const float4* z4 = reinterpret_cast<const float4*>(z);
  float4* h4 = reinterpret_cast<float4*>(h);
  float4* hi4 = reinterpret_cast<float4*>(hi);
  float4* lo4 = reinterpret_cast<float4*>(lo);
  for (int64_t i = blockIdx.x * (int64_t)blockDim.x + threadIdx.x; i < n4; i += (int64_t)gridDim.x * blockDim.x) {
    const int ch = (int)((i * 4) % C);
    const float4 v = z4[i];
    const float4 m = *reinterpret_cast<const float4*>(mean + ch);
    const float4 s = *reinterpret_cast<const float4*>(istd + ch);
    const float4 g = make_float4(gamma[ch], gamma[ch + 1], gamma[ch + 2], gamma[ch + 3]);
    const float4 b = make_float4(beta[ch], beta[ch + 1], beta[ch + 2], beta[ch + 3]);
    float4 o;
    o.x = g.x * ((v.x - m.x) * s.x) + b.x;
    o.y = g.y * ((v.y - m.y) * s.y) + b.y;
    o.z = g.z * ((v.z - m.z) * s.z) + b.z;
    o.w = g.w * ((v.w - m.w) * s.w) + b.w;
    if (act) {
      o.x = o.x > 0.f ? o.x : a * o.x;
      o.y = o.y > 0.f ? o.y : a * o.y;
      o.z = o.z > 0.f ? o.z : a * o.z;
      o.w = o.w > 0.f ? o.w : a * o.w;
    }
    if (h) h4[i] = o;
    am = amax4(am, o.x, o.y, o.z, o.w);
    if (hi) {
      float4 vh, vl;
      vh.x = __uint_as_float((__float_as_uint(o.x) + 0x1000u) & 0xFFFFE000u);
      vh.y = __uint_as_float((__float_as_uint(o.y) + 0x1000u) & 0xFFFFE000u);
      vh.z = __uint_as_float((__float_as_uint(o.z) + 0x1000u) & 0xFFFFE000u);
      vh.w = __uint_as_float((__float_as_uint(o.w) + 0x1000u) & 0xFFFFE000u);
      vl = make_float4(o.x - vh.x, o.y - vh.y, o.z - vh.z, o.w - vh.w);
      hi4[i] = vh;
      lo4[i] = vl;
    }
  }
  amax_commit(amax, am);
}
__global__ void bn_prelu_apply_scalar_kernel(const float* __restrict__ z, const float* __restrict__ mean,
                                             const float* __restrict__ istd, const float* __restrict__ gamma,
                                             const float* __restrict__ beta, const float* __restrict__ slope,
                                             float* __restrict__ h, int64_t n, int C) {
  const bool act = slope != nullptr;
  const float a = act ? *slope : 1.f;
  for (int64_t i = blockIdx.x * (int64_t)blockDim.x + threadIdx.x; i < n; i += (int64_t)gridDim.x * blockDim.x) {
    const int ch = (int)(i % C);
    float o = gamma[ch] * ((z[i] - mean[ch]) * istd[ch]) + beta[ch];
    if (act) o = o > 0.f ? o : a * o;
    h[i] = o;
  }
}
int k_bn_prelu_apply(fg_ctx* c, const float* z, const float* mean, const float* istd, const float* gamma,
                     const float* beta, const float* slope, float* h, int64_t P, int C, float* hi, float* lo) {
  const int64_t n = P * C;
  if (C % 4 == 0) {
    bn_prelu_apply_kernel<<<grid_for(n / 4, 256), 256, 0, c->stream>>>(z, mean, istd, gamma, beta, slope, h, hi, lo, n / 4, C,
                                                                       take_amax(c));
  } else {
    if (hi || !h) {
      fg_set_error("bn_prelu_apply: hi/lo outputs need C %% 4 == 0");
      return FG_ERR_UNSUPPORTED;
    }
    bn_prelu_apply_scalar_kernel<<<grid_for(n, 256), 256, 0, c->stream>>>(z, mean, istd, gamma, beta, slope, h, n, C);
  }
  LAUNCH_CHECK(c);
  return FG_OK;
}

__global__ void bn_prelu_bwd_reduce_kernel(const float* __restrict__ dh, const float* __restrict__ z,
                                           const float* __restrict__ mean, const float* __restrict__ istd,
                                           const float* __restrict__ gamma, const float* __restrict__ beta,
                                           const float* __restrict__ slope, double* __restrict__ acc,
                                           float* __restrict__ dslope, int B, int H, int W, int C, int pool,
                                           int64_t rows_per_block, double* __restrict__ ws, unsigned* __restrict__ ticket) {
  extern __shared__ double sm[];
  const int lanes = blockDim.x / C;
  const int ch = threadIdx.x % C, lane = threadIdx.x / C;
  const int64_t P = (int64_t)B * H * W;
  const int64_t r0 = blockIdx.x * rows_per_block, r1 = min(P, r0 + rows_per_block);
  const bool act = slope != nullptr;
  const float a = act ? *slope : 1.f;
  const float m = mean[ch], is = istd[ch], ga = gamma[ch], be = beta[ch];
  double sg = 0, sgx = 0, ss = 0;
  for (int64_t r = r0 + lane; r < r1; r += lanes) {
    float d;
    if (pool) {
      const uint32_t ru = (uint32_t)r;
      const int x = (int)(ru % (uint32_t)W);
      const uint32_t q = ru / (uint32_t)W;
      d = load_dh(dh, (int)(q / (uint32_t)H), (int)(q % (uint32_t)H), x, ch, H, W, C, 1);
    } else {
      d = dh[r * C + ch];
    }
    const float xh = (z[r * C + ch] - m) * is;
    float g = d;
    if (act) {
      const float u = ga * xh + be;
      if (!(u > 0.f)) {
        g = a * d;
        ss += (double)d * (double)u;
      }
    }
    sg += g;
    sgx += (double)g * (double)xh;
  }
  sm[threadIdx.x] = sg;
  sm[blockDim.x + threadIdx.x] = sgx;
  __syncthreads();
  if (lane == 0) {
    for (int l = 1; l < lanes; ++l) {
      sg += sm[l * C + ch];
      sgx += sm[blockDim.x + l * C + ch];
    }
    ws[(int64_t)blockIdx.x * (2 * C + 1) + ch] = sg;
    ws[(int64_t)blockIdx.x * (2 * C + 1) + C + ch] = sgx;
  }
  if (act) ss = block_sum(ss);
  if (threadIdx.x == 0) ws[(int64_t)blockIdx.x * (2 * C + 1) + 2 * C] = ss;
  if (ordered_last_block(ticket)) {
    for (int i = threadIdx.x; i < 2 * C; i += blockDim.x) acc[i] += ordered_sum(ws, gridDim.x, 2 * C + 1, i);
    if (act && dslope && threadIdx.x == 0) *dslope += (float)ordered_sum(ws, gridDim.x, 2 * C + 1, 2 * C);
    ordered_release(ticket);
  }
}
int k_bn_prelu_bwd_reduce(fg_ctx* c, const float* dh, const float* z, const float* mean, const float* istd,
                          const float* gamma, const float* beta, const float* slope, double* acc, float* dslope, int B,
                          int H, int W, int C, int pool) {
  if (!pool && k_bn4_ok(C))
    return k_bn_bwd_reduce4(c, dh, z, mean, istd, gamma, beta, slope, acc, dslope, (int64_t)B * H * W, C);
  if (C > 1024) return FG_ERR_UNSUPPORTED;
  FG_CUDA(cudaMemsetAsync(acc, 0, sizeof(double) * 2 * C, c->stream));
  const int64_t P = (int64_t)B * H * W;
  const int block = bn_block(C);
  int grid = (int)std::min<int64_t>(c->sm_count * 4, (P + 63) / 64);
  if (grid < 1) grid = 1;
  const int64_t rpb = (P + grid - 1) / grid;
  FG_TRY(red_check(c, grid, 2 * C + 1));
  bn_prelu_bwd_reduce_kernel<<<grid, block, sizeof(double) * 2 * block, c->stream>>>(dh, z, mean, istd, gamma, beta, slope,
                                                                                  acc, dslope, B, H, W, C, pool, rpb, c->red_ws,
                                                                                  c->red_ticket);
  LAUNCH_CHECK(c);
  return FG_OK;
}
__global__ void bn_bwd_finalize_kernel(const double* __restrict__ acc, float* __restrict__ mg, float* __restrict__ dgamma,
                                       float* __restrict__ dbeta, int64_t P, int C) {
  const int ch = blockIdx.x * blockDim.x + threadIdx.x;
  if (ch >= C) return;
  mg[ch] = (float)(acc[ch] / (double)P);
  mg[C + ch] = (float)(acc[C + ch] / (double)P);
  if (dgamma) dgamma[ch] += (float)acc[C + ch];
  if (dbeta) dbeta[ch] += (float)acc[ch];
}
int k_bn_bwd_finalize(fg_ctx* c, double* acc, float* mg, float* dgamma, float* dbeta, int64_t P, int C) {
  bn_bwd_finalize_kernel<<<(C + 127) / 128, 128, 0, c->stream>>>(acc, mg, dgamma, dbeta, P, C);
  LAUNCH_CHECK(c);
  return FG_OK;
}
__global__ void bn_prelu_bwd_apply_kernel(const float* __restrict__ dh, const float* __restrict__ z,
                                          const float* __restrict__ mean, const float* __restrict__ istd,
                                          const float* __restrict__ gamma, const float* __restrict__ beta,
                                          const float* __restrict__ slope, const float* __restrict__ mg,
                                          float* __restrict__ dz, int B, int H, int W, int C, int pool) {
  const bool act = slope != nullptr;
  const float a = act ? *slope : 1.f;
  const int64_t n = (int64_t)B * H * W * C;
  for (int64_t i = blockIdx.x * (int64_t)blockDim.x + threadIdx.x; i < n; i += (int64_t)gridDim.x * blockDim.x) {
    const int ch = (int)(i % C);
    int64_t r = i / C;
    const int x = (int)(r % W);
    r /= W;
    const int y = (int)(r % H);
    const int b = (int)(r / H);
    const float d = load_dh(dh, b, y, x, ch, H, W, C, pool);
    const float is = istd[ch], ga = gamma[ch];
    const float xh = (z[i] - mean[ch]) * is;
    float g = d;
    if (act) {
      const float u = ga * xh + beta[ch];
      if (!(u > 0.f)) g = a * d;
    }
    dz[i] = ga * is * (g - mg[ch] - xh * mg[C + ch]);
  }
}
__device__ void block_colsum_rows(const float (&bs)[4], int C, int n, double* ws, unsigned* ticket, float* dst,
                                  float* extra_dst, double extra = 0.0) {
  __shared__ float tb[256][4];
#pragma unroll
  for (int j = 0; j < 4; ++j) tb[threadIdx.x][j] = bs[j];
  __syncthreads();
  const int C4 = C / 4;
  double* row = ws + (int64_t)blockIdx.x * n;
  for (int i = threadIdx.x; i < C; i += blockDim.x) {
    double s = 0;
    for (int t = i / 4; t < (int)blockDim.x; t += C4) s += tb[t][i & 3];
    row[i] = s;
  }
  if (n > C && threadIdx.x == 0) row[C] = extra;
  if (ordered_last_block(ticket)) {
    if (dst)
      for (int i = threadIdx.x; i < C; i += blockDim.x) dst[i] += (float)ordered_sum(ws, gridDim.x, n, i);
    if (extra_dst && threadIdx.x == 0) *extra_dst += (float)ordered_sum(ws, gridDim.x, n, C);
    ordered_release(ticket);
  }
}

__global__ void bn_prelu_bwd_apply4_kernel(const float* __restrict__ dh, const float* __restrict__ z,
                                           const float* __restrict__ mean, const float* __restrict__ istd,
                                           const float* __restrict__ gamma, const float* __restrict__ beta,
                                           const float* __restrict__ slope, const float* __restrict__ mg,
                                           float* __restrict__ dz, float* __restrict__ hi, float* __restrict__ lo,
                                           float* __restrict__ dbias, int64_t n4, int C, unsigned* __restrict__ amax,
                                           double* __restrict__ ws, unsigned* __restrict__ ticket) {
  float am = 0.f;
  float bs[4] = {0.f, 0.f, 0.f, 0.f};
  const bool act = slope != nullptr;
  const float a = act ? *slope : 1.f;
  const float4* dh4 = reinterpret_cast<const float4*>(dh);
  const float4* z4 = reinterpret_cast<const float4*>(z);
  float4* dz4 = reinterpret_cast<float4*>(dz);
  float4* hi4 = reinterpret_cast<float4*>(hi);
  float4* lo4 = reinterpret_cast<float4*>(lo);
  const int C4 = C / 4;
  for (int64_t i = blockIdx.x * (int64_t)blockDim.x + threadIdx.x; i < n4; i += (int64_t)gridDim.x * blockDim.x) {
    const int ch = (int)(i % C4) * 4;
    const float4 d = dh4[i], v = z4[i];
    const float dv[4] = {d.x, d.y, d.z, d.w}, zv[4] = {v.x, v.y, v.z, v.w};
    float o[4];
#pragma unroll
    for (int j = 0; j < 4; ++j) {
      const float is = istd[ch + j], ga = gamma[ch + j];
      const float xh = (zv[j] - mean[ch + j]) * is;
      float g = dv[j];
      if (act) {
        const float u = ga * xh + beta[ch + j];
        if (!(u > 0.f)) g = a * g;
      }
      o[j] = ga * is * (g - mg[ch + j] - xh * mg[C + ch + j]);
    }
    dz4[i] = make_float4(o[0], o[1], o[2], o[3]);
    am = amax4(am, o[0], o[1], o[2], o[3]);
    bs[0] += o[0]; bs[1] += o[1]; bs[2] += o[2]; bs[3] += o[3];
    if (hi) {
      float h[4];
#pragma unroll
      for (int j = 0; j < 4; ++j) h[j] = __uint_as_float((__float_as_uint(o[j]) + 0x1000u) & 0xFFFFE000u);
      hi4[i] = make_float4(h[0], h[1], h[2], h[3]);
      lo4[i] = make_float4(o[0] - h[0], o[1] - h[1], o[2] - h[2], o[3] - h[3]);
    }
  }
  amax_commit(amax, am);
  if (dbias) block_colsum_rows(bs, C, C, ws, ticket, dbias, nullptr);
}
int k_bn_prelu_bwd_apply(fg_ctx* c, const float* dh, const float* z, const float* mean, const float* istd,
                         const float* gamma, const float* beta, const float* slope, const float* mg, float* dz, int B,
                         int H, int W, int C, int pool, float* hi, float* lo, float* dbias) {
  const int64_t n = (int64_t)B * H * W * C;
  if (!pool && C % 4 == 0 && C <= 1024 && 256 % (C / 4) == 0) {
    const int grid = grid_for(n / 4, 256);
    FG_TRY(red_check(c, grid, C));
    bn_prelu_bwd_apply4_kernel<<<grid, 256, 0, c->stream>>>(dh, z, mean, istd, gamma, beta, slope, mg, dz, hi, lo, dbias, n / 4,
                                                           C, take_amax(c), c->red_ws, c->red_ticket);
    LAUNCH_CHECK(c);
    return FG_OK;
  }
  if (hi) {
    fg_set_error("bn_prelu_bwd_apply: hi/lo outputs need the un-pooled float4 path");
    return FG_ERR_UNSUPPORTED;
  }
  bn_prelu_bwd_apply_kernel<<<grid_for(n, 256), 256, 0, c->stream>>>(dh, z, mean, istd, gamma, beta, slope, mg, dz, B, H,
                                                                    W, C, pool);
  LAUNCH_CHECK(c);
  if (dbias) return k_colsum_add(c, dz, dbias, (int64_t)B * H * W, C, 0, 0);
  return FG_OK;
}

__device__ __forceinline__ float sigmoidf_(float x) { return 1.0f / (1.0f + expf(-x)); }
__global__ void sigmoid_fwd_kernel(const float* __restrict__ z, float* __restrict__ y, int64_t n) {
  for (int64_t i = blockIdx.x * (int64_t)blockDim.x + threadIdx.x; i < n; i += (int64_t)gridDim.x * blockDim.x)
    y[i] = sigmoidf_(z[i]);
}
int k_sigmoid_fwd(fg_ctx* c, const float* z, float* y, int64_t n) {
  sigmoid_fwd_kernel<<<grid_for(n, 256), 256, 0, c->stream>>>(z, y, n);
  LAUNCH_CHECK(c);
  return FG_OK;
}
__global__ void sigmoid_bwd_kernel(const float* __restrict__ dy, const float* __restrict__ y, float* __restrict__ dz,
                                   int64_t n) {
  for (int64_t i = blockIdx.x * (int64_t)blockDim.x + threadIdx.x; i < n; i += (int64_t)gridDim.x * blockDim.x) {
    const float v = y[i];
    dz[i] = dy[i] * v * (1.0f - v);
  }
}
int k_sigmoid_bwd(fg_ctx* c, const float* dy, const float* y, float* dz, int64_t n) {
  sigmoid_bwd_kernel<<<grid_for(n, 256), 256, 0, c->stream>>>(dy, y, dz, n);
  LAUNCH_CHECK(c);
  return FG_OK;
}
int k_sigmoid_grad_mul(fg_ctx* c, const float* dout, const float* out, float* dlogit, int n) {
  return k_sigmoid_bwd(c, dout, out, dlogit, n);
}

__device__ __forceinline__ uint64_t splitmix64(uint64_t x) {
  x += 0x9E3779B97F4A7C15ull;
  x = (x ^ (x >> 30)) * 0xBF58476D1CE4E5B9ull;
  x = (x ^ (x >> 27)) * 0x94D049BB133111EBull;
  return x ^ (x >> 31);
}
__global__ void masks_generate_kernel(float* __restrict__ masks, int B, uint64_t seed, float p_spatial, float p_drop,
                                      const uint64_t* __restrict__ seed_dev) {
  if (seed_dev) seed += *seed_dev * 2;
  const int64_t n = (int64_t)B * kMaskPerSample;
  for (int64_t i = blockIdx.x * (int64_t)blockDim.x + threadIdx.x; i < n; i += (int64_t)gridDim.x * blockDim.x) {
    const int j = (int)(i % kMaskPerSample);
    const uint64_t r = splitmix64(seed * 0x100000001B3ull + (uint64_t)i);
    const float u = (float)(r >> 40) * (1.0f / 16777216.0f);
    masks[i] = u >= (j < 960 ? p_spatial : p_drop) ? 1.f : 0.f;
  }
}
__global__ void set_u64_kernel(uint64_t* dst, uint64_t v) { *dst = v; }
int k_set_u64(fg_ctx* c, uint64_t* dst, uint64_t v) {
  set_u64_kernel<<<1, 1, 0, c->stream>>>(dst, v);
  LAUNCH_CHECK(c);
  return FG_OK;
}
__global__ void seed_roots_kernel(uint64_t* roots, int n) {
  const int j = threadIdx.x;
  if (j >= 1 && j < n) roots[j] = (1ull << 60) | (roots[0] << 8) | (uint64_t)j;
}
int k_seed_roots(fg_ctx* c, uint64_t* roots, int n) {
  seed_roots_kernel<<<1, 32, 0, c->stream>>>(roots, n);
  LAUNCH_CHECK(c);
  return FG_OK;
}
int k_masks_generate(fg_ctx* c, float* masks, int B, uint64_t seed, float p_spatial, float p_drop, const uint64_t* seed_dev) {
  masks_generate_kernel<<<grid_for((int64_t)B * kMaskPerSample, 256), 256, 0, c->stream>>>(masks, B, seed, p_spatial,
                                                                                          p_drop, seed_dev);
  LAUNCH_CHECK(c);
  return FG_OK;
}

__device__ __forceinline__ float4 prelu4(float4 v, float a) {
  v.x = v.x > 0.f ? v.x : a * v.x;
  v.y = v.y > 0.f ? v.y : a * v.y;
  v.z = v.z > 0.f ? v.z : a * v.z;
  v.w = v.w > 0.f ? v.w : a * v.w;
  return v;
}
__device__ __forceinline__ void split4(const float4& o, float4* hi, float4* lo, uint32_t i) {
  float4 h;
  h.x = __uint_as_float((__float_as_uint(o.x) + 0x1000u) & 0xFFFFE000u);
  h.y = __uint_as_float((__float_as_uint(o.y) + 0x1000u) & 0xFFFFE000u);
  h.z = __uint_as_float((__float_as_uint(o.z) + 0x1000u) & 0xFFFFE000u);
  h.w = __uint_as_float((__float_as_uint(o.w) + 0x1000u) & 0xFFFFE000u);
  hi[i] = h;
  lo[i] = make_float4(o.x - h.x, o.y - h.y, o.z - h.z, o.w - h.w);
}
__global__ void d_act_pool_fwd_kernel(const float* __restrict__ z, const float* __restrict__ slope,
                                      const float* __restrict__ masks, int moff, float eval_scale, float* __restrict__ p,
                                      float4* __restrict__ hi, float4* __restrict__ lo, int B, int H, int W, int C,
                                      unsigned* __restrict__ amax) {
  float am = 0.f;
  const float a = *slope;
  const uint32_t Ho = H / 2, Wo = W / 2, C4 = C / 4;
  const uint32_t n = (uint32_t)B * Ho * Wo * C4;
  const float4* z4 = reinterpret_cast<const float4*>(z);
  float4* p4 = reinterpret_cast<float4*>(p);
  for (uint32_t i = blockIdx.x * blockDim.x + threadIdx.x; i < n; i += gridDim.x * blockDim.x) {
    const uint32_t c4 = i % C4;
    uint32_t r = i / C4;
    const uint32_t xo = r % Wo;
    r /= Wo;
    const uint32_t yo = r % Ho, b = r / Ho;
    float4 m = make_float4(eval_scale, eval_scale, eval_scale, eval_scale);
    if (masks) m = *reinterpret_cast<const float4*>(masks + (size_t)b * kMaskPerSample + moff + c4 * 4);
    const uint32_t base = ((b * H + 2 * yo) * W + 2 * xo) * C4 + c4, rs = (uint32_t)W * C4;
    const float4 v0 = prelu4(z4[base], a), v1 = prelu4(z4[base + C4], a), v2 = prelu4(z4[base + rs], a),
                 v3 = prelu4(z4[base + rs + C4], a);
    float4 o;
    o.x = (v0.x * m.x + v1.x * m.x + v2.x * m.x + v3.x * m.x) * 0.25f;
    o.y = (v0.y * m.y + v1.y * m.y + v2.y * m.y + v3.y * m.y) * 0.25f;
    o.z = (v0.z * m.z + v1.z * m.z + v2.z * m.z + v3.z * m.z) * 0.25f;
    o.w = (v0.w * m.w + v1.w * m.w + v2.w * m.w + v3.w * m.w) * 0.25f;
    p4[i] = o;
    am = amax4(am, o.x, o.y, o.z, o.w);
    if (hi) split4(o, hi, lo, i);
  }
  amax_commit(amax, am);
}
int k_d_act_pool_fwd(fg_ctx* c, const float* z, const float* slope, const float* masks, int moff, float eval_scale,
                     float* p, int B, int H, int W, int C, float* hi, float* lo) {
  const int64_t n = (int64_t)B * (H / 2) * (W / 2) * C / 4;
  if (C % 4 || (moff % 4) || (int64_t)B * H * W * C >= ((int64_t)1 << 31)) {
    fg_set_error("d_act_pool_fwd: unsupported shape (C %% 4, size)");
    return FG_ERR_UNSUPPORTED;
  }
  d_act_pool_fwd_kernel<<<grid_for(n, 256), 256, 0, c->stream>>>(z, slope, masks, moff, eval_scale, p, reinterpret_cast<float4*>(hi),
                                                                 reinterpret_cast<float4*>(lo), B, H, W, C, take_amax(c));
  LAUNCH_CHECK(c);
  return FG_OK;
}
__global__ void d_act_pool_bwd_kernel(const float* __restrict__ dp, const float* __restrict__ z,
                                      const float* __restrict__ slope, const float* __restrict__ masks, int moff,
                                      float eval_scale, float* __restrict__ dz, float* __restrict__ dslope,
                                      float4* __restrict__ hi, float4* __restrict__ lo, float* __restrict__ dbias, int B,
                                      int H, int W, int C, unsigned* __restrict__ amax, double* __restrict__ ws,
                                      unsigned* __restrict__ ticket) {
  float am = 0.f;
  float bs[4] = {0.f, 0.f, 0.f, 0.f};
  const float a = *slope;
  const uint32_t Ho = H / 2, Wo = W / 2, C4 = C / 4;
  const uint32_t n = (uint32_t)B * Ho * Wo * C4;
  const float4* z4 = reinterpret_cast<const float4*>(z);
  const float4* dp4 = reinterpret_cast<const float4*>(dp);
  float4* dz4 = reinterpret_cast<float4*>(dz);
  float s = 0.f;
  double sd = 0;
  for (uint32_t i = blockIdx.x * blockDim.x + threadIdx.x; i < n; i += gridDim.x * blockDim.x) {
    const uint32_t c4 = i % C4;
// ... 363 lines not shown
```

face_generator_b200/csrc/nets.cu:

```cuda
#include <algorithm>

#include "convl.h"
#include "fg_internal.h"
#include "k_conv_tc.h"

namespace {
struct DLayout {
  int64_t cW[4], cb[4], ca[4], L1W, L1b, a5, L2W, L2b, a6, L3W, L3b, total;
};

DLayout make_d_layout(int C) {
  DLayout L;
  const int cin[4] = {C, 64, 128, 256}, cout[4] = {64, 128, 256, 512};
  int64_t o = 0;
  for (int i = 0; i < 4; ++i) {
    L.cW[i] = o; o += (int64_t)cout[i] * cin[i] * 9;
    L.cb[i] = o; o += cout[i];
    L.ca[i] = o; o += 1;
  }
  L.L1W = o; o += 512 * 2048;
  L.L1b = o; o += 512;
  L.a5 = o; o += 1;
  L.L2W = o; o += 512 * 512;
  L.L2b = o; o += 512;
// ... 70 lines not shown
  FG_TRY(dalloc(n, &n->io_dev2, c->io_dev_elems));
  {
    ConvLEnv& e = n->env;
    e.c = c;
    e.maxB = c->maxB;
    e.allocs = &n->allocs;
    FG_TRY(dalloc(n, &e.dy.hi, B * 131072));
    FG_TRY(dalloc(n, &e.dy.lo, B * 131072));
    static const GenDesc g32{32, "", 128, true};
    FG_TRY(gen_alloc(e, n->G, g32));
    ScalePairs& sp = n->D_pairs;
    FG_TRY(sp.alloc(c, n->allocs, 1 + 2 * 6));
    FG_TRY(sp.take(&e.dy.s));
    const DLayout& dl = n->dl;
    auto conv = [&](ConvL& L, int Cin, int Cout, int k, int H, int64_t w_off, int64_t b_off, const char* tf, const char* td,
                    const char* tw) {
      L.Cin = Cin; L.Cout = Cout; L.k = k; L.H = H;
      L.w_off = w_off; L.b_off = b_off;
      L.tf = tf; L.td = td; L.tw = tw;
    };
    static const char* tf[4] = {"D.C1.fwd", "D.C2.fwd", "D.C3.fwd", "D.C4.fwd"};
    static const char* td[4] = {"D.C1.dgrad", "D.C2.dgrad", "D.C3.dgrad", "D.C4.dgrad"};
    static const char* tw[4] = {"D.C1.wgrad", "D.C2.wgrad", "D.C3.wgrad", "D.C4.wgrad"};
    for (int i = 0; i < 4; ++i) conv(n->Dc[i], dcin(c, i), kDcout[i], 3, kDhw[i], dl.cW[i], dl.cb[i], tf[i], td[i], tw[i]);
    conv(n->DL1, 2048, 512, 1, 1, dl.L1W, dl.L1b, "D.L1.fwd", "D.L1.dgrad", "D.L1.wgrad");
    n->DL1.cA = 512; n->DL1.cS = 4;
    conv(n->DL2, 512, 512, 1, 1, dl.L2W, dl.L2b, "D.L2.fwd", "D.L2.dgrad", "D.L2.wgrad");
    for (ConvL* L : {&n->Dc[0], &n->Dc[1], &n->Dc[2], &n->Dc[3], &n->DL1, &n->DL2}) {
      FG_TRY(sp.take(&L->x.s));
      FG_TRY(sp.take(&L->sdy));
      FG_TRY(convl_alloc(e, *L));
    }
  }
  FG_TRY(dalloc(n, &n->in_noiseD, B * kNoiseDim));
  FG_TRY(dalloc(n, &n->in_noiseG, B * kNoiseDim));
  p.keep = {{"Dstep.z1", n->D_z[0], 65536}, {"Dstep.z2", n->D_z[1], 32768}, {"Dstep.z3", n->D_z[2], 16384},
            {"Dstep.z4", n->D_z[3], 8192},  {"Dstep.zl1", n->D_zl1, 512},    {"Dstep.zl2", n->D_zl2, 512},
            {"Dstep.logit", n->D_logit, 1}, {"Dstep.out", n->D_out, 1}};
  FG_CUDA(cudaStreamSynchronize(c->stream));
  return FG_OK;
}

int pack_D(Net32* n) {
  fg_ctx* c = n->c;
  if (n->net.D_pack == pack_key(c)) return FG_OK;
  for (int i = 0; i < 4; ++i) FG_TRY(convl_pack(c, n->Dc[i], n->net.PD));
  FG_TRY(convl_pack(c, n->DL1, n->net.PD));
  FG_TRY(convl_pack(c, n->DL2, n->net.PD));
  n->net.D_pack = pack_key(c);
  return FG_OK;
}

int D_forward(Net32* n, const float* x, int B, bool training, const fg_hyper* h) {
  fg_ctx* c = n->c;
  FG_REQUIRE(B >= 1 && B <= c->maxB, "D forward: batch %d out of range [1,%d]", B, c->maxB);
  FG_TRY(pack_D(n));
  FG_TRY(n->D_pairs.reset(c));
  const DLayout& L = n->dl;
  float* P = n->net.PD;
  if (x != n->D_x)
    FG_CUDA(cudaMemcpyAsync(n->D_x, x, sizeof(float) * (size_t)B * 1024 * c->C, cudaMemcpyDeviceToDevice, c->stream));
  n->D_B = B;
  n->D_train = training;
  const float* masks = training ? n->D_masks : nullptr;
  const float* cur = n->D_x;
  for (int i = 0; i < 4; ++i) {
    const int H = kDhw[i];
    FG_TRY(convl_fwd(n->env, n->Dc[i], cur, P, n->D_z[i], B));
    TcOp& nx = (i < 3 ? n->Dc[i + 1] : n->DL1).x;
    nx.split_ready = convl_tc_fwd(c, i < 3 ? n->Dc[i + 1] : n->DL1) && !tc_f16(c);
    {
      AmaxInto am(c, nx);
      FG_TRY(k_d_act_pool_fwd(c, n->D_z[i], P + L.ca[i], masks, kDmoff[i], 1.0f - h->p_spatial, n->D_p[i], B, H, H,
                              kDcout[i], nx.split_ready ? nx.hi : nullptr, nx.split_ready ? nx.lo : nullptr));
    }
    cur = n->D_p[i];
  }
  const float scale = 1.0f / (1.0f - h->p_drop);
  n->D_drop_scale = scale;
  n->D_spatial_eval = 1.0f - h->p_spatial;
  FG_TRY(convl_fwd(n->env, n->DL1, n->D_p[3], P, n->D_zl1, B));
  {
    AmaxInto am(c, n->DL2.x);
    FG_TRY(k_lin_act_drop_fwd(c, n->D_zl1, P + L.a5, masks, 960, scale, n->D_hl1, B, 512));
  }
  FG_TRY(convl_fwd(n->env, n->DL2, n->D_hl1, P, n->D_zl2, B));
  FG_TRY(k_lin_act_drop_fwd(c, n->D_zl2, P + L.a6, masks, 1472, scale, n->D_hl2, B, 512));
  {
    ScopedTimer tm(c, "D.L3.fwd");
    FG_TRY(k_gemv_fwd(c, n->D_hl2, P + L.L3W, P + L.L3b, n->D_logit, B, 512));
  }
  n->D_fwd_valid = true;
  return FG_OK;
}

int D_backward(Net32* n, const float* dlogit, bool want_wgrad, bool want_dx) {
  fg_ctx* c = n->c;
  if (!n->D_fwd_valid) {
    fg_set_error("D backward needs a preceding D forward");
    return FG_ERR_STATE;
  }
  const DLayout& L = n->dl;
  float *P = n->net.PD, *G = n->net.gD;
  const int B = n->D_B;
  const float* masks = n->D_train ? n->D_masks : nullptr;
  const float scale = n->D_drop_scale, eval_scale = n->D_spatial_eval;
  FG_TRY(n->D_pairs.reset(c));
  if (want_wgrad) {
    ScopedTimer tm(c, "D.L3.wgrad");
    FG_TRY(k_gemv_wgrad_add(c, n->D_hl2, dlogit, G + L.L3W, G + L.L3b, B, 512));
  }
  {
    ScopedTimer tm(c, "D.L3.dgrad");
    FG_TRY(k_gemv_dgrad(c, dlogit, P + L.L3W, n->D_dh, B, 512));
  }
  TcOp& dy = n->env.dy;
  float* GD = want_wgrad ? G : nullptr;
  {
    AmaxInto am(c, n->DL2.sdy, &dy.amax_ready);
    FG_TRY(k_lin_act_drop_bwd(c, n->D_dh, n->D_zl2, P + L.a6, masks, 1472, scale, n->D_dzl, want_wgrad ? G + L.a6 : nullptr, B,
                              512));
  }
  FG_TRY(convl_bwd(n->env, n->DL2, n->D_hl1, n->D_dzl, GD, n->D_dh, B));
  {
    AmaxInto am(c, n->DL1.sdy, &dy.amax_ready);
    FG_TRY(k_lin_act_drop_bwd(c, n->D_dh, n->D_zl1, P + L.a5, masks, 960, scale, n->D_dzl, want_wgrad ? G + L.a5 : nullptr, B,
                              512));
  }
  FG_TRY(convl_bwd(n->env, n->DL1, n->D_p[3], n->D_dzl, GD, n->D_dp, B));
  for (int i = 3; i >= 0; --i) {
    const int H = kDhw[i];
    dy.split_ready = convl_tc_bwd(c, n->Dc[i]) && !tc_f16(c);
    dy.bias_ready = want_wgrad;
    {
      AmaxInto am(c, n->Dc[i].sdy, &dy.amax_ready);
      FG_TRY(k_d_act_pool_bwd(c, n->D_dp, n->D_z[i], P + L.ca[i], masks, kDmoff[i], eval_scale, n->D_dz,
                              want_wgrad ? G + L.ca[i] : nullptr, B, H, H, kDcout[i], dy.split_ready ? dy.hi : nullptr,
                              dy.split_ready ? dy.lo : nullptr, want_wgrad ? G + L.cb[i] : nullptr));
    }
    float* din = i > 0 ? n->D_dp : want_dx ? n->D_dx : nullptr;
    FG_TRY(convl_bwd(n->env, n->Dc[i], i == 0 ? n->D_x : n->D_p[i - 1], n->D_dz, GD, din, B));
  }
  return FG_OK;
}

struct NetStep final : StepNets {
  Net32* n;
  const float *real, *noiseD, *noiseG;
  NetStep(Net32* n, const fg_hyper* h, int B, const float* real, const float* noiseD, const float* noiseG)
      : StepNets(n->c, n->net, h, B, n->D_logit, n->D_out, n->D_dlogit, n->D_masks, kMaskPerSample, true, true), n(n),
        real(real), noiseD(noiseD), noiseG(noiseG) {}
  int g_forward(int j, bool d_iter) override {
    const int rows = d_iter ? B / 2 : B;
    return gen_forward(n->env, n->G, n->net, (d_iter ? noiseD : noiseG) + (size_t)j * rows * kNoiseDim, rows, true);
  }
  int d_input(int j) override {
    const int Bh = B / 2;
    const size_t img = (size_t)c->C * 1024;
    FG_TRY(k_nchw_to_nhwc(c, real + (size_t)j * Bh * img, n->D_x, Bh, c->C, 1024));
    FG_CUDA(cudaMemcpyAsync(n->D_x + Bh * img, n->G.y, sizeof(float) * Bh * img, cudaMemcpyDeviceToDevice, c->stream));
    return FG_OK;
  }
  int draw_masks(int kind, const uint64_t* root) override {
    return k_masks_generate(c, n->D_masks, B, kind, h->p_spatial, h->p_drop, root);
  }
  int d_forward(bool on_g) override { return D_forward(n, on_g ? n->G.y : n->D_x, B, true, h); }
  int d_backward(bool want_wgrad, bool want_dx) override { return D_backward(n, n->D_dlogit, want_wgrad, want_dx); }
  int g_backward() override { return gen_backward(n->env, n->G, n->net, n->D_dx, nullptr); }
};
}

int net32_alloc(fg_ctx* c) {
  c->n32 = new Net32();
  c->n32->c = c;
  return n32_alloc(c->n32);
}
void net32_free(fg_ctx* c) {
  Net32* n = c->n32;
  if (!n) return;
  pair_free(n->net);
  for (void* p : n->allocs) cudaFree(p);
  delete n;
  c->n32 = nullptr;
}
NetPair& net32_pair(fg_ctx* c) { return c->n32->net; }

#define ENTER(c)                                      \
  do {                                                \
    if (!(c)) {                                       \
      fg_set_error("null fg_ctx");                    \
      return FG_ERR_INVALID;                          \
    }                                                 \
    FG_CUDA(cudaSetDevice((c)->device));              \
  } while (0)

namespace {
int train_step_iters(fg_ctx* c, const char* what, const fg_hyper* h, int B, int d_iters, int g_iters, const float* real,
                     const float* noise_D, const float* noise_G, const float* masks_D, const float* masks_G, uint64_t seed,
                     fg_step_stats* stats) {
  ENTER(c);
  FG_TRY(step_check(c, what, B, d_iters, g_iters, h && real && noise_D && noise_G));
  Net32* n = c->n32;
  const size_t nd = d_iters, ng = g_iters, Bh = B / 2, M = c->maxB, img = (size_t)c->C * 1024;
  IterStage& s = n->iter_stage;
  const float *r, *zd, *zg, *md, *mg;
  FG_TRY(s.in(c, n->allocs, 0, real, nd * Bh * img, nd * M / 2 * img, &r));
  FG_TRY(s.in(c, n->allocs, 1, noise_D, nd * Bh * kNoiseDim, nd * M / 2 * kNoiseDim, &zd));
  FG_TRY(s.in(c, n->allocs, 2, noise_G, ng * B * kNoiseDim, ng * M * kNoiseDim, &zg));
  FG_TRY(s.in(c, n->allocs, 3, masks_D, nd * B * kMaskPerSample, nd * M * kMaskPerSample, &md));
  FG_TRY(s.in(c, n->allocs, 4, masks_G, ng * B * kMaskPerSample, ng * M * kMaskPerSample, &mg));
  NetStep st(n, h, B, r, zd, zg);
  return pair_train_step(st, d_iters, g_iters, md, mg, seed, {r, zd, zg, md, mg, nullptr}, nullptr, stats);
}

int train_step_dataset_iters(fg_ctx* c, fg_dataset* d, const char* what, const fg_hyper* h, int B, int d_iters, int g_iters,
                             uint64_t seed, fg_step_stats* stats) {
  if (!d || !d->c) {
    fg_set_error("null fg_dataset");
    return FG_ERR_INVALID;
  }
  FG_CUDA(cudaSetDevice(d->c->device));
  FG_TRY(step_check(c, what, B, d_iters, g_iters, h, d, true));
  Net32* n = c->n32;
  const int Bh = B / 2;
  const size_t M = c->maxB, img = (size_t)c->C * 1024;
  IterStage& s = n->iter_stage;
  FG_TRY(s.reserve(c, n->allocs, 0, d_iters * M / 2 * img));
  FG_TRY(s.reserve(c, n->allocs, 1, d_iters * M / 2 * kNoiseDim));
  FG_TRY(s.reserve(c, n->allocs, 2, g_iters * M * kNoiseDim));
  float *real = s.p[0], *zd = s.p[1], *zg = s.p[2];
  const std::function<int()> feed = [&]() -> int {
    for (int j = 0; j < d_iters; ++j) {
      FG_TRY(dataset_draw_gather(d, 0, Bh, 32, real + (size_t)j * Bh * img, c->seed_dev + j, 4));
      FG_TRY(noise_uniform_dev(c, 1, (int64_t)Bh * kNoiseDim, zd + (size_t)j * Bh * kNoiseDim, c->seed_dev + j, 4));
    }
    for (int j = 0; j < g_iters; ++j)
      FG_TRY(noise_uniform_dev(c, 2, (int64_t)B * kNoiseDim, zg + (size_t)j * B * kNoiseDim, c->seed_dev + j, 4));
    return FG_OK;
  };
  NetStep st(n, h, B, real, zd, zg);
  return pair_train_step(st, d_iters, g_iters, nullptr, nullptr, seed, {real, zd, zg, nullptr, nullptr, d}, &feed, stats);
}
}

extern "C" {

int64_t fg_param_count(int net, int channels) {
  if (channels != 1 && channels != 3) return -1;
  return net == FG_NET_G ? make_g_layout(channels, 32).total : net == FG_NET_D ? make_d_layout(channels).total : -1;
}
int fg_set_params(fg_ctx* c, int net, const float* src) {
  ENTER(c);
  FG_REQUIRE(net == FG_NET_G || net == FG_NET_D, "net must be FG_NET_G or FG_NET_D");
  return pair_set_params(c, c->n32->net, net, src);
}
int fg_get_params(fg_ctx* c, int net, float* dst) {
  ENTER(c);
  FG_REQUIRE(net == FG_NET_G || net == FG_NET_D, "net must be FG_NET_G or FG_NET_D");
  return pair_get_params(c, c->n32->net, net, dst);
}
int fg_get_grads(fg_ctx* c, int net, float* dst) {
  ENTER(c);
  FG_REQUIRE(net == FG_NET_G || net == FG_NET_D, "net must be FG_NET_G or FG_NET_D");
  return pair_get_grads(c, c->n32->net, net, dst);
}
int fg_zero_grads(fg_ctx* c, int net) {
  ENTER(c);
  FG_REQUIRE(net == FG_NET_G || net == FG_NET_D, "net must be FG_NET_G or FG_NET_D");
  return pair_zero_grads(c, c->n32->net, net);
}
int fg_bind_params(fg_ctx* c, int net, float* params_dev, float* grads_dev) {
  ENTER(c);
  c->graph_epoch++;
  FG_REQUIRE(net == FG_NET_G || net == FG_NET_D, "net must be FG_NET_G or FG_NET_D");
  for (const float* p : {params_dev, grads_dev}) {
    if (!p) continue;
    FG_REQUIRE(fg_is_dev(p), "fg_bind_params: buffers must be DEVICE memory (CudaTensor:data())");
    FG_REQUIRE(reinterpret_cast<uintptr_t>(p) % 16 == 0, "fg_bind_params: buffers must be 16-byte aligned");
  }
  FG_CUDA(cudaStreamSynchronize(c->stream));
  Net32* n = c->n32;
  NetPair& np = n->net;
  const bool d = net == FG_NET_D;
  (d ? np.PD : np.PG) = params_dev ? params_dev : (d ? n->ownPD : n->ownPG);
  float* own_g = d ? n->ownGD : n->ownGG;
  const int64_t len = d ? np.nD : np.nG;
  (d ? np.gD : np.gG) = grads_dev ? grads_dev : own_g;
  (d ? np.tailD : np.tailG) = grads_dev ? n->tail_sep + (d ? kGradTail : 0) : own_g + len;
  np.G_pack = np.D_pack = -1;
  return FG_OK;
}
float* fg_params_ptr(fg_ctx* c, int net) {
  return !c ? nullptr : net == FG_NET_D ? c->n32->net.PD : net == FG_NET_G ? c->n32->net.PG : nullptr;
}
float* fg_grads_ptr(fg_ctx* c, int net) {
  return !c ? nullptr : net == FG_NET_D ? c->n32->net.gD : net == FG_NET_G ? c->n32->net.gG : nullptr;
}

int fg_set_adam_state(fg_ctx* c, int net, const float* m, const float* v, int t) {
  ENTER(c);
  FG_REQUIRE(net == FG_NET_G || net == FG_NET_D, "net must be FG_NET_G or FG_NET_D");
  return pair_set_adam_state(c, c->n32->net, net, m, v, t);
}
int fg_get_adam_state(fg_ctx* c, int net, float* m, float* v, int* t) {
  ENTER(c);
  FG_REQUIRE(net == FG_NET_G || net == FG_NET_D, "net must be FG_NET_G or FG_NET_D");
  return pair_get_adam_state(c, c->n32->net, net, m, v, t);
}
int fg_set_bn_state(fg_ctx* c, const float* src) {
  ENTER(c);
  return pair_set_bn_state(c, c->n32->net, src);
}
int fg_get_bn_state(fg_ctx* c, float* dst) {
  ENTER(c);
  return pair_get_bn_state(c, c->n32->net, dst);
}

int fg_G_forward(fg_ctx* c, const float* noise, int B, int training, float* images_out) {
  ENTER(c);
  FG_REQUIRE(noise && B >= 1 && B <= c->maxB, "fg_G_forward: bad arguments (B=%d, max %d)", B, c->maxB);
  Net32* n = c->n32;
  n->net.G_pack = -1;
  const float* nd;
  FG_TRY(fg_to_dev(c, noise, (size_t)B * kNoiseDim, n->in_noiseG, &nd));
  FG_TRY(gen_forward(n->env, n->G, n->net, nd, B, training != 0));
  if (images_out) {
    FG_TRY(k_nhwc_to_nchw(c, n->G.y, c->io_dev, B, c->C, 1024));
    FG_TRY(fg_to_user(c, images_out, c->io_dev, (size_t)B * c->C * 1024));
  }
  return FG_OK;
}
int fg_G_backward(fg_ctx* c, const float* d_images, float* d_noise) {
  ENTER(c);
  FG_REQUIRE(d_images, "fg_G_backward: d_images is null");
  Net32* n = c->n32;
  const int B = n->G.B;
  const float* dd;
  FG_TRY(fg_to_dev(c, d_images, (size_t)B * c->C * 1024, c->io_dev, &dd));
  FG_TRY(k_nchw_to_nhwc(c, dd, n->io_dev2, B, c->C, 1024));
  float* dn = nullptr;
  if (d_noise) dn = fg_is_dev(d_noise) ? d_noise : n->in_noiseD;
  FG_TRY(gen_backward(n->env, n->G, n->net, n->io_dev2, dn));
  if (d_noise && dn != d_noise) FG_TRY(fg_to_user(c, d_noise, dn, (size_t)B * kNoiseDim));
  return FG_OK;
}
int fg_D_forward(fg_ctx* c, const float* images, int B, int training, const float* masks, uint64_t seed, float* out) {
  ENTER(c);
  FG_REQUIRE(images && B >= 1 && B <= c->maxB, "fg_D_forward: bad arguments (B=%d, max %d)", B, c->maxB);
  Net32* n = c->n32;
  n->net.D_pack = -1;
  fg_hyper h;
  fg_hyper_default(&h);
  const float* xd;
  FG_TRY(fg_to_dev(c, images, (size_t)B * c->C * 1024, c->io_dev, &xd));
  FG_TRY(k_nchw_to_nhwc(c, xd, n->D_x, B, c->C, 1024));
  if (training) {
    if (masks) {
      FG_CUDA(cudaMemcpyAsync(n->D_masks, masks, sizeof(float) * (size_t)B * kMaskPerSample, cudaMemcpyDefault, c->stream));
    } else {
      FG_TRY(k_masks_generate(c, n->D_masks, B, seed, h.p_spatial, h.p_drop));
    }
  }
  FG_TRY(D_forward(n, n->D_x, B, training != 0, &h));
  FG_TRY(k_sigmoid_fwd(c, n->D_logit, n->D_out, B));
  if (out) FG_TRY(fg_to_user(c, out, n->D_out, B));
  return FG_OK;
}
int fg_D_backward(fg_ctx* c, const float* d_out, int want_wgrad, float* d_images) {
  ENTER(c);
  FG_REQUIRE(d_out, "fg_D_backward: d_out is null");
  Net32* n = c->n32;
  const int B = n->D_B;
  const float* dd;
  FG_TRY(fg_to_dev(c, d_out, B, n->D_targets, &dd));
  FG_TRY(k_sigmoid_grad_mul(c, dd, n->D_out, n->D_dlogit, B));
  FG_TRY(D_backward(n, n->D_dlogit, want_wgrad != 0, d_images != nullptr));
  if (d_images) {
    FG_TRY(k_nhwc_to_nchw(c, n->D_dx, c->io_dev, B, c->C, 1024));
    FG_TRY(fg_to_user(c, d_images, c->io_dev, (size_t)B * c->C * 1024));
  }
  return FG_OK;
}
int fg_bce_forward(fg_ctx* c, const float* x, const float* t, int n, float* loss_out) {
  ENTER(c);
  FG_REQUIRE(x && t && loss_out && n > 0 && n <= c->maxB, "fg_bce_forward: bad arguments");
  const float *xd, *td;
  FG_TRY(fg_to_dev(c, x, n, c->io_dev, &xd));
  FG_TRY(fg_to_dev(c, t, n, c->n32->io_dev2, &td));
  FG_TRY(k_bce_fwd(c, xd, td, n, c->n32->D_targets));
  return fg_to_user(c, loss_out, c->n32->D_targets, 1);
}
int fg_bce_backward(fg_ctx* c, const float* x, const float* t, int n, float* dx) {
  ENTER(c);
  FG_REQUIRE(x && t && dx && n > 0 && n <= c->maxB, "fg_bce_backward: bad arguments");
  const float *xd, *td;
  FG_TRY(fg_to_dev(c, x, n, c->io_dev, &xd));
  FG_TRY(fg_to_dev(c, t, n, c->n32->io_dev2, &td));
  FG_TRY(k_bce_bwd(c, xd, td, n, c->n32->D_targets));
  return fg_to_user(c, dx, c->n32->D_targets, n);
}
int fg_optim_step(fg_ctx* c, int net, const fg_hyper* h, float grad_scale) {
  ENTER(c);
  FG_REQUIRE(h && (net == FG_NET_G || net == FG_NET_D), "fg_optim_step: bad arguments");
  FG_TRY(k_optim_prep(c, c->n32->net.dstats, net, h));
  return pair_optim(c, c->n32->net, net, h, grad_scale);
}

int fg_train_step(fg_ctx* c, const fg_hyper* h, int B, const float* real, const float* noise_D, const float* noise_G,
                  const float* masks_D, const float* masks_G, uint64_t seed, fg_step_stats* stats) {
  return train_step_iters(c, "fg_train_step", h, B, 1, 1, real, noise_D, noise_G, masks_D, masks_G, seed, stats);
}
int fg_train_step_iters(fg_ctx* c, const fg_hyper* h, int B, int d_iters, int g_iters, const float* real,
                        const float* noise_D, const float* noise_G, const float* masks_D, const float* masks_G, uint64_t seed,
                        fg_step_stats* stats) {
  return train_step_iters(c, "fg_train_step_iters", h, B, d_iters, g_iters, real, noise_D, noise_G, masks_D, masks_G, seed,
                          stats);
}
int fg_train_step_dataset(fg_ctx* c, fg_dataset* d, const fg_hyper* h, int B, uint64_t seed, fg_step_stats* stats) {
  return train_step_dataset_iters(c, d, "fg_train_step_dataset", h, B, 1, 1, seed, stats);
}
int fg_train_step_dataset_iters(fg_ctx* c, fg_dataset* d, const fg_hyper* h, int B, int d_iters, int g_iters, uint64_t seed,
                                fg_step_stats* stats) {
  return train_step_dataset_iters(c, d, "fg_train_step_dataset_iters", h, B, d_iters, g_iters, seed, stats);
}

int fg_sample(fg_ctx* c, const float* noise, int N, int chunk, float* images_out) {
  ENTER(c);
  FG_REQUIRE(noise && images_out && N >= 1 && chunk >= 1 && chunk <= c->maxB, "fg_sample: bad arguments (chunk %d, max %d)",
             chunk, c->maxB);
  Net32* n = c->n32;
  const bool out_dev = fg_is_dev(images_out);
  const size_t img = (size_t)c->C * 1024;
  n->net.G_pack = -1;
  for (int s = 0; s < N; s += chunk) {
    const int b = std::min(chunk, N - s);
    const float* nd;
    FG_TRY(fg_to_dev(c, noise + (size_t)s * kNoiseDim, (size_t)b * kNoiseDim, n->in_noiseG, &nd));
    FG_TRY(gen_forward(n->env, n->G, n->net, nd, b, true));
    float* dst = images_out + (size_t)s * img;
    if (out_dev) {
      FG_TRY(k_nhwc_to_nchw(c, n->G.y, dst, b, c->C, 1024));
    } else {
      FG_TRY(k_nhwc_to_nchw(c, n->G.y, c->io_dev, b, c->C, 1024));
      FG_CUDA(cudaMemcpyAsync(dst, c->io_dev, b * img * sizeof(float), cudaMemcpyDeviceToHost, c->stream));
      if (s + chunk < N) FG_CUDA(cudaStreamSynchronize(c->stream));
    }
  }
  if (!out_dev) FG_CUDA(cudaStreamSynchronize(c->stream));
  return FG_OK;
}

int64_t fg_debug_tensor(fg_ctx* c, const char* name, float* dst, int64_t max_elems) {
  if (!c || !name) return -1;
  cudaSetDevice(c->device);
  const Net32* n = c->n32;
  const int db = n->D_B;
  std::vector<DebugTensor> ents = {
      {"D.z1", n->D_z[0], 65536, db}, {"D.z2", n->D_z[1], 32768, db}, {"D.z3", n->D_z[2], 16384, db},
      {"D.z4", n->D_z[3], 8192, db}, {"D.p4", n->D_p[3], 2048, db}, {"D.logit", n->D_logit, 1, db},
      {"D.out", n->D_out, 1, db}, {"D.dx", n->D_dx, 1024 * c->C, db}, {"D.masks", n->D_masks, kMaskPerSample, db},
      {"D.zl1", n->D_zl1, 512, db}, {"D.zl2", n->D_zl2, 512, db}};
  pair_keep_rows(n->net, ents);
  gen_debug_rows(n->G, ents);
  return debug_tensor_copy(c, "fg_debug_tensor", ents.data(), ents.size(), name, dst, max_elems);
}

}
```

face_generator_b200/csrc/nets_s16.cu:

```cuda
#include <algorithm>

#include "convl.h"
#include "fg_internal.h"
#include "k_misc.h"

namespace {
constexpr int kS16Mask = 1024 + 128;
constexpr int kSide = 16;

__global__ void avgpool2_fwd_kernel(const float* __restrict__ x, float* __restrict__ y, int B, int H, int W, int C) {
  const int Ho = H / 2, Wo = W / 2;
  const int64_t n = (int64_t)B * Ho * Wo * C;
  GRID_STRIDE(i, n) {
    const int ch = (int)(i % C);
    int64_t r = i / C;
    const int xo = (int)(r % Wo); r /= Wo;
    const int yo = (int)(r % Ho);
    const int64_t b = r / Ho;
    const float* p = x + (((b * H + 2 * yo) * W + 2 * xo) * (int64_t)C + ch);
    y[i] = 0.25f * ((p[0] + p[C]) + (p[(int64_t)W * C] + p[(int64_t)W * C + C]));
  }
}
__global__ void avgpool2_bwd_kernel(const float* __restrict__ dy, float* __restrict__ dx, int B, int H, int W, int C) {
  const int Ho = H / 2, Wo = W / 2;
// ... 157 lines not shown
  FG_TRY(dalloc(n, &n->D_dhe2, B * 128));
  FG_TRY(dalloc(n, &n->D_logit, B));
  FG_TRY(dalloc(n, &n->D_out, B));
  FG_TRY(dalloc(n, &n->D_dlogit, B));
  FG_TRY(dalloc(n, &n->D_masks, B * kS16Mask));
  FG_TRY(dalloc(n, &n->D_dx, B * 256 * C));
  FG_TRY(dalloc(n, &n->D_dx2, B * 256 * C));
  const size_t big = B * 256 * 128;
  FG_TRY(dalloc(n, &n->ga, big));
  FG_TRY(dalloc(n, &n->gb, big));
  FG_TRY(dalloc(n, &n->env.dy.hi, big));
  FG_TRY(dalloc(n, &n->env.dy.lo, big));
  FG_TRY(dalloc(n, &n->ws, (size_t)9 * 1024 * 512));
  n->env.ga = n->ga; n->env.ws = n->ws;
  static const GenDesc g16{kSide, "s16.", 0, false};
  FG_TRY(gen_alloc(n->env, n->G, g16));
  FG_TRY(dalloc(n, &n->in_a, B * 256 * C));
  FG_TRY(dalloc(n, &n->in_b, B * 100));
  FG_TRY(dalloc(n, &n->in_c, B * 100));
  FG_TRY(dalloc(n, &n->io, B * 256 * C));
  n->net.keep = {{"Dstep.z1", n->D_z[0], 256 * 128}, {"Dstep.z2", n->D_z[1], 256 * 128}, {"Dstep.z3", n->D_z[2], 16 * 512},
                 {"Dstep.z4", n->D_z[3], 4 * 1024},  {"Dstep.zf", n->D_zf, 1024},        {"Dstep.ze1", n->D_ze1, 128},
                 {"Dstep.ze2", n->D_ze2, 128},       {"Dstep.logit", n->D_logit, 1},     {"Dstep.out", n->D_out, 1}};
  FG_CUDA(cudaStreamSynchronize(n->c->stream));
  return FG_OK;
}

int pack_D(fg_s16* n) {
  fg_ctx* c = n->c;
  if (n->net.D_pack == pack_key(c)) return FG_OK;
  for (int i = 0; i < 4; ++i) FG_TRY(convl_pack(c, n->Dc[i], n->net.PD));
  FG_TRY(convl_pack(c, n->DF1, n->net.PD));
  FG_TRY(convl_pack(c, n->DE1, n->net.PD));
  FG_TRY(convl_pack(c, n->DE2, n->net.PD));
  n->net.D_pack = pack_key(c);
  return FG_OK;
}

int D_forward(fg_s16* n, const float* x, int B, bool training) {
  fg_ctx* c = n->c;
  FG_REQUIRE(B >= 1 && B <= n->maxB, "s16 D forward: batch %d out of range [1,%d]", B, n->maxB);
  FG_TRY(pack_D(n));
  const float* P = n->net.PD;
  if (x != n->D_x) FG_CUDA(cudaMemcpyAsync(n->D_x, x, sizeof(float) * (size_t)B * 256 * n->C, cudaMemcpyDeviceToDevice, c->stream));
  const float* masks = training ? n->D_masks : nullptr;
  FG_TRY(convl_fwd(n->env, n->Dc[0], n->D_x, P, n->D_z[0], B));
  FG_TRY(k_prelu_fwd(c, n->D_z[0], P + n->Dca[0], n->D_h[0], (int64_t)B * 256 * 128));
  FG_TRY(convl_fwd(n->env, n->Dc[1], n->D_h[0], P, n->D_z[1], B));
  FG_TRY(k_prelu_fwd(c, n->D_z[1], P + n->Dca[1], n->D_h[1], (int64_t)B * 256 * 128));
  avgpool2_fwd_kernel<<<grid_for((int64_t)B * 64 * 128, 256), 256, 0, c->stream>>>(n->D_h[1], n->D_p1, B, 16, 16, 128);
  LAUNCH_CHECK(c);
  FG_TRY(convl_fwd(n->env, n->Dc[2], n->D_p1, P, n->D_zfull, B));
  subsample2_kernel<<<grid_for((int64_t)B * 16 * 512, 256), 256, 0, c->stream>>>(n->D_zfull, n->D_z[2], B, 8, 8, 512);
  LAUNCH_CHECK(c);
  FG_TRY(k_prelu_fwd(c, n->D_z[2], P + n->Dca[2], n->D_h[2], (int64_t)B * 16 * 512));
  FG_TRY(convl_fwd(n->env, n->Dc[3], n->D_h[2], P, n->D_zfull, B));
  subsample2_kernel<<<grid_for((int64_t)B * 4 * 1024, 256), 256, 0, c->stream>>>(n->D_zfull, n->D_z[3], B, 4, 4, 1024);
  LAUNCH_CHECK(c);
  FG_TRY(k_prelu_fwd(c, n->D_z[3], P + n->Dca[3], n->D_h[3], (int64_t)B * 4096));
  plane_dropout_kernel<<<grid_for((int64_t)B * 4096, 256), 256, 0, c->stream>>>(n->D_h[3], masks, kS16Mask, 0, 0.5f, n->D_d3, B, 4,
                                                                                1024);
  LAUNCH_CHECK(c);
  FG_TRY(convl_fwd(n->env, n->DF1, n->D_d3, P, n->D_zf, B));
  FG_TRY(k_prelu_fwd(c, n->D_zf, P + n->Daf, n->D_hf, (int64_t)B * 1024));
  FG_TRY(convl_fwd(n->env, n->DE1, n->D_x, P, n->D_ze1, B));
  FG_TRY(k_prelu_fwd(c, n->D_ze1, P + n->Dae1, n->D_he1, (int64_t)B * 128));
  const float* de1 = n->D_he1;
  if (training) {
    FG_TRY(k_dropout_nhwc(c, n->D_he1, n->D_masks, kS16Mask, 1024, 1, 128, 2.0f, n->D_de1, B));
    de1 = n->D_de1;
  }
  FG_TRY(convl_fwd(n->env, n->DE2, de1, P, n->D_ze2, B));
  FG_TRY(k_prelu_fwd(c, n->D_ze2, P + n->Dae2, n->D_he2, (int64_t)B * 128));
  join2_kernel<<<grid_for((int64_t)B * 1152, 256), 256, 0, c->stream>>>(n->D_hf, n->D_he2, n->D_joint, B, 1024, 128);
  LAUNCH_CHECK(c);
  FG_TRY(k_gemv_fwd(c, n->D_joint, P + n->DJW, P + n->DJb, n->D_logit, B, 1152));
  n->D_B = B;
  n->D_train = training;
  n->D_valid = true;
  return FG_OK;
}
int D_backward(fg_s16* n, const float* dlogit, bool want_wgrad, bool want_dx) {
  fg_ctx* c = n->c;
  if (!n->D_valid) {
    fg_set_error("s16 D backward needs a preceding D forward");
    return FG_ERR_STATE;
  }
  const int B = n->D_B;
  const float* P = n->net.PD;
  float* G = want_wgrad ? n->net.gD : nullptr;
  const bool tr = n->D_train;
  const float* masks = tr ? n->D_masks : nullptr;
  if (G) FG_TRY(k_gemv_wgrad_add(c, n->D_joint, dlogit, G + n->DJW, G + n->DJb, B, 1152));
  FG_TRY(k_gemv_dgrad(c, dlogit, P + n->DJW, n->D_djoint, B, 1152));
  split2_kernel<<<grid_for((int64_t)B * 1152, 256), 256, 0, c->stream>>>(n->D_djoint, n->D_dhf, n->D_dhe2, B, 1024, 128);
  LAUNCH_CHECK(c);
  float *cur = n->ga, *oth = n->gb;
  {
    FG_TRY(k_prelu_bwd(c, n->D_dhe2, n->D_ze2, P + n->Dae2, cur, G ? G + n->Dae2 : nullptr, B, 1, 1, 128, 0));
    FG_TRY(convl_bwd(n->env, n->DE2, tr ? n->D_de1 : n->D_he1, cur, G, oth, B));
    std::swap(cur, oth);
    if (tr) {
      FG_TRY(k_dropout_nhwc(c, cur, n->D_masks, kS16Mask, 1024, 1, 128, 2.0f, oth, B));
      std::swap(cur, oth);
    }
    FG_TRY(k_prelu_bwd(c, cur, n->D_ze1, P + n->Dae1, oth, G ? G + n->Dae1 : nullptr, B, 1, 1, 128, 0));
    std::swap(cur, oth);
    FG_TRY(convl_bwd(n->env, n->DE1, n->D_x, cur, G, want_dx ? n->D_dx2 : nullptr, B));
  }
  {
    FG_TRY(k_prelu_bwd(c, n->D_dhf, n->D_zf, P + n->Daf, cur, G ? G + n->Daf : nullptr, B, 1, 1, 1024, 0));
    FG_TRY(convl_bwd(n->env, n->DF1, n->D_d3, cur, G, oth, B));
    std::swap(cur, oth);
    plane_dropout_kernel<<<grid_for((int64_t)B * 4096, 256), 256, 0, c->stream>>>(cur, masks, kS16Mask, 0, 0.5f, oth, B, 4, 1024);
    LAUNCH_CHECK(c);
    std::swap(cur, oth);
    FG_TRY(k_prelu_bwd(c, cur, n->D_z[3], P + n->Dca[3], oth, G ? G + n->Dca[3] : nullptr, B, 2, 2, 1024, 0));
    std::swap(cur, oth);
    zero_insert2_kernel<<<grid_for((int64_t)B * 16 * 1024, 256), 256, 0, c->stream>>>(cur, oth, B, 4, 4, 1024);
    LAUNCH_CHECK(c);
    std::swap(cur, oth);
    FG_TRY(convl_bwd(n->env, n->Dc[3], n->D_h[2], cur, G, oth, B));
    std::swap(cur, oth);
    FG_TRY(k_prelu_bwd(c, cur, n->D_z[2], P + n->Dca[2], oth, G ? G + n->Dca[2] : nullptr, B, 4, 4, 512, 0));
    std::swap(cur, oth);
    zero_insert2_kernel<<<grid_for((int64_t)B * 64 * 512, 256), 256, 0, c->stream>>>(cur, oth, B, 8, 8, 512);
    LAUNCH_CHECK(c);
    std::swap(cur, oth);
    FG_TRY(convl_bwd(n->env, n->Dc[2], n->D_p1, cur, G, oth, B));
    std::swap(cur, oth);
    avgpool2_bwd_kernel<<<grid_for((int64_t)B * 256 * 128, 256), 256, 0, c->stream>>>(cur, oth, B, 16, 16, 128);
    LAUNCH_CHECK(c);
    std::swap(cur, oth);
    FG_TRY(k_prelu_bwd(c, cur, n->D_z[1], P + n->Dca[1], oth, G ? G + n->Dca[1] : nullptr, B, 16, 16, 128, 0));
    std::swap(cur, oth);
    FG_TRY(convl_bwd(n->env, n->Dc[1], n->D_h[0], cur, G, oth, B));
    std::swap(cur, oth);
    FG_TRY(k_prelu_bwd(c, cur, n->D_z[0], P + n->Dca[0], oth, G ? G + n->Dca[0] : nullptr, B, 16, 16, 128, 0));
    std::swap(cur, oth);
    FG_TRY(convl_bwd(n->env, n->Dc[0], n->D_x, cur, G, want_dx ? n->D_dx : nullptr, B));
  }
  if (want_dx) FG_TRY(k_add(c, n->D_dx, n->D_dx2, n->D_dx, (int64_t)B * 256 * n->C));
  return FG_OK;
}

struct S16Step final : StepNets {
  fg_s16* n;
  const float *real, *noiseD, *noiseG;
  S16Step(fg_s16* n, const fg_hyper* h, int B, const float* real, const float* noiseD, const float* noiseG)
      : StepNets(n->c, n->net, h, B, n->D_logit, n->D_out, n->D_dlogit, n->D_masks, kS16Mask, true, false), n(n), real(real),
        noiseD(noiseD), noiseG(noiseG) {}
  int g_forward(int j, bool d_iter) override {
    const int rows = d_iter ? B / 2 : B;
    return gen_forward(n->env, n->G, n->net, (d_iter ? noiseD : noiseG) + (size_t)j * rows * 100, rows, true);
  }
  int d_input(int j) override {
    const int Bh = B / 2;
    const size_t img = (size_t)n->C * 256;
    FG_TRY(k_nchw_to_nhwc(c, real + (size_t)j * Bh * img, n->D_x, Bh, n->C, 256));
    FG_CUDA(cudaMemcpyAsync(n->D_x + Bh * img, n->G.y, sizeof(float) * Bh * img, cudaMemcpyDeviceToDevice, c->stream));
    return FG_OK;
  }
  int draw_masks(int kind, const uint64_t* root) override {
    return k_bernoulli_keep(c, n->D_masks, (int64_t)B * kS16Mask, kind, 0.5f, root);
  }
  int d_forward(bool on_g) override { return D_forward(n, on_g ? n->G.y : n->D_x, B, true); }
  int d_backward(bool want_wgrad, bool want_dx) override { return D_backward(n, n->D_dlogit, want_wgrad, want_dx); }
  int g_backward() override { return gen_backward(n->env, n->G, n->net, n->D_dx, nullptr); }
};

}

#define ENTER(n)                                         \
  do {                                                   \
    if (!(n) || !(n)->c) {                               \
      fg_set_error("null fg_s16");                       \
      return FG_ERR_INVALID;                             \
    }                                                    \
    FG_CUDA(cudaSetDevice((n)->c->device));              \
  } while (0)

namespace {
int train_step_iters(fg_s16* n, const char* what, const fg_hyper* h, int B, int d_iters, int g_iters, const float* real,
                     const float* noise_D, const float* noise_G, const float* masks_D, const float* masks_G, uint64_t seed,
                     fg_step_stats* stats) {
  ENTER(n);
  fg_ctx* c = n->c;
  FG_TRY(step_check(c, what, B, d_iters, g_iters, h && real && noise_D && noise_G));
  const size_t nd = d_iters, ng = g_iters, Bh = B / 2, M = n->maxB, img = (size_t)n->C * 256;
  IterStage& s = n->iter_stage;
  const float *rd, *zd, *zg, *md, *mg;
  FG_TRY(s.in(c, n->allocs, 0, real, nd * Bh * img, nd * M / 2 * img, &rd));
  FG_TRY(s.in(c, n->allocs, 1, noise_D, nd * Bh * 100, nd * M / 2 * 100, &zd));
  FG_TRY(s.in(c, n->allocs, 2, noise_G, ng * B * 100, ng * M * 100, &zg));
  FG_TRY(s.in(c, n->allocs, 3, masks_D, nd * B * kS16Mask, nd * M * kS16Mask, &md));
  FG_TRY(s.in(c, n->allocs, 4, masks_G, ng * B * kS16Mask, ng * M * kS16Mask, &mg));
  S16Step st(n, h, B, rd, zd, zg);
  return pair_train_step(st, d_iters, g_iters, md, mg, seed, {rd, zd, zg, md, mg, nullptr}, nullptr, stats);
}

int train_step_dataset_iters(fg_s16* n, fg_dataset* d, const char* what, const fg_hyper* h, int B, int d_iters, int g_iters,
                             uint64_t seed, fg_step_stats* stats) {
  ENTER(n);
  fg_ctx* c = n->c;
  FG_TRY(step_check(c, what, B, d_iters, g_iters, h, d, true));
  const int Bh = B / 2;
  const size_t M = n->maxB, img = (size_t)n->C * 256;
  IterStage& s = n->iter_stage;
  FG_TRY(s.reserve(c, n->allocs, 0, d_iters * M / 2 * img));
  FG_TRY(s.reserve(c, n->allocs, 1, d_iters * M / 2 * 100));
  FG_TRY(s.reserve(c, n->allocs, 2, g_iters * M * 100));
  float *real = s.p[0], *zd = s.p[1], *zg = s.p[2];
  const std::function<int()> feed = [&]() -> int {
    for (int j = 0; j < d_iters; ++j) {
      FG_TRY(dataset_draw_gather(d, 0, Bh, kSide, real + (size_t)j * Bh * img, c->seed_dev + j, 4));
      FG_TRY(noise_uniform_dev(c, 1, (int64_t)Bh * 100, zd + (size_t)j * Bh * 100, c->seed_dev + j, 4));
    }
    for (int j = 0; j < g_iters; ++j)
      FG_TRY(noise_uniform_dev(c, 2, (int64_t)B * 100, zg + (size_t)j * B * 100, c->seed_dev + j, 4));
    return FG_OK;
  };
  S16Step st(n, h, B, real, zd, zg);
  return pair_train_step(st, d_iters, g_iters, nullptr, nullptr, seed, {real, zd, zg, nullptr, nullptr, d}, &feed, stats);
}
}

extern "C" {

int fg_s16_create(fg_ctx* ctx, fg_s16** out) {
  if (!ctx || !out) {
    fg_set_error("fg_s16_create: null argument");
    return FG_ERR_INVALID;
  }
  *out = nullptr;
  FG_CUDA(cudaSetDevice(ctx->device));
  fg_s16* n = new fg_s16();
  n->c = ctx;
  n->maxB = ctx->maxB;
  n->C = ctx->C;
  const int r = s16_alloc(n);
  if (r != FG_OK) {
    fg_s16_destroy(n);
    return r;
  }
  *out = n;
  return FG_OK;
}
int fg_s16_destroy(fg_s16* n) {
  if (!n) return FG_OK;
  if (n->c) {
    cudaSetDevice(n->c->device);
    cudaStreamSynchronize(n->c->stream);
  }
  pair_free(n->net);
  for (void* p : n->allocs) cudaFree(p);
  delete n;
  return FG_OK;
}
int64_t fg_s16_param_count(int net, int channels) {
  if (net != FG_NET_D) return make_g_layout(channels, kSide).total;
  fg_s16 tmp;
  tmp.C = channels;
  make_d16_layout(&tmp);
  return tmp.net.nD;
}
int fg_s16_mask_per_sample(void) { return kS16Mask; }

int fg_s16_set_params(fg_s16* n, int net, const float* src) {
  ENTER(n);
  FG_REQUIRE(src && (net == FG_NET_G || net == FG_NET_D), "fg_s16_set_params: bad arguments");
  return pair_set_params(n->c, n->net, net, src);
}
int fg_s16_get_params(fg_s16* n, int net, float* dst) {
  ENTER(n);
  FG_REQUIRE(dst && (net == FG_NET_G || net == FG_NET_D), "fg_s16_get_params: bad arguments");
  return pair_get_params(n->c, n->net, net, dst);
}
int fg_s16_get_grads(fg_s16* n, int net, float* dst) {
  ENTER(n);
  FG_REQUIRE(dst && (net == FG_NET_G || net == FG_NET_D), "fg_s16_get_grads: bad arguments");
  return pair_get_grads(n->c, n->net, net, dst);
}
int fg_s16_zero_grads(fg_s16* n, int net) {
  ENTER(n);
  return pair_zero_grads(n->c, n->net, net);
}
float* fg_s16_params_ptr(fg_s16* n, int net) { return !n ? nullptr : (net == FG_NET_D ? n->net.PD : n->net.PG); }
float* fg_s16_grads_ptr(fg_s16* n, int net) { return !n ? nullptr : (net == FG_NET_D ? n->net.gD : n->net.gG); }

int fg_s16_set_adam_state(fg_s16* n, int net, const float* m, const float* v, int t) {
  ENTER(n);
  return pair_set_adam_state(n->c, n->net, net, m, v, t);
}
int fg_s16_get_adam_state(fg_s16* n, int net, float* m, float* v, int* t) {
  ENTER(n);
  return pair_get_adam_state(n->c, n->net, net, m, v, t);
}
int fg_s16_set_bn_state(fg_s16* n, const float* src768) {
  ENTER(n);
  FG_REQUIRE(src768, "fg_s16_set_bn_state: null source");
  return pair_set_bn_state(n->c, n->net, src768);
}
int fg_s16_get_bn_state(fg_s16* n, float* dst768) {
  ENTER(n);
  FG_REQUIRE(dst768, "fg_s16_get_bn_state: null destination");
  return pair_get_bn_state(n->c, n->net, dst768);
}

int fg_s16_G_forward(fg_s16* n, const float* noise, int B, int training, float* img_out) {
  ENTER(n);
  FG_REQUIRE(noise && B >= 1 && B <= n->maxB, "fg_s16_G_forward: bad arguments (batch %d, max %d)", B, n->maxB);
  const float* nd;
  FG_TRY(fg_to_dev(n->c, noise, (size_t)B * 100, n->in_b, &nd));
  FG_TRY(gen_forward(n->env, n->G, n->net, nd, B, training != 0));
  if (img_out) {
    FG_TRY(k_nhwc_to_nchw(n->c, n->G.y, n->io, B, n->C, 256));
    FG_TRY(fg_to_user(n->c, img_out, n->io, (size_t)B * n->C * 256));
  }
  return FG_OK;
}
int fg_s16_G_backward(fg_s16* n, const float* d_img, float* d_noise) {
  ENTER(n);
  FG_REQUIRE(d_img, "fg_s16_G_backward: null gradient");
  const float* dd;
  FG_TRY(fg_to_dev(n->c, d_img, (size_t)n->G.B * n->C * 256, n->in_a, &dd));
  FG_TRY(k_nchw_to_nhwc(n->c, dd, n->io, n->G.B, n->C, 256));
  FG_TRY(gen_backward(n->env, n->G, n->net, n->io, d_noise ? n->in_c : nullptr));
  if (d_noise) FG_TRY(fg_to_user(n->c, d_noise, n->in_c, (size_t)n->G.B * 100));
  return FG_OK;
}
int fg_s16_D_forward(fg_s16* n, const float* img, int B, int training, const float* masks, uint64_t seed, float* out) {
  ENTER(n);
  FG_REQUIRE(img && B >= 1 && B <= n->maxB, "fg_s16_D_forward: bad arguments (batch %d, max %d)", B, n->maxB);
  fg_ctx* c = n->c;
  const float* id;
  FG_TRY(fg_to_dev(c, img, (size_t)B * n->C * 256, n->in_a, &id));
  FG_TRY(k_nchw_to_nhwc(c, id, n->D_x, B, n->C, 256));
  if (training) {
    if (masks)
      FG_CUDA(cudaMemcpyAsync(n->D_masks, masks, sizeof(float) * (size_t)B * kS16Mask, cudaMemcpyDefault, c->stream));
    else
      FG_TRY(k_bernoulli_keep(c, n->D_masks, (int64_t)B * kS16Mask, seed, 0.5f));
  }
  FG_TRY(D_forward(n, n->D_x, B, training != 0));
  FG_TRY(k_sigmoid_fwd(c, n->D_logit, n->D_out, B));
  if (out) FG_TRY(fg_to_user(c, out, n->D_out, B));
  return FG_OK;
}
int fg_s16_D_backward(fg_s16* n, const float* d_out, int want_wgrad, float* d_img) {
  ENTER(n);
  FG_REQUIRE(d_out, "fg_s16_D_backward: null gradient");
  fg_ctx* c = n->c;
  const float* dd;
  FG_TRY(fg_to_dev(c, d_out, (size_t)n->D_B, n->in_b, &dd));
  FG_TRY(k_sigmoid_bwd(c, dd, n->D_out, n->D_dlogit, n->D_B));
  FG_TRY(D_backward(n, n->D_dlogit, want_wgrad != 0, d_img != nullptr));
  if (d_img) {
    FG_TRY(k_nhwc_to_nchw(c, n->D_dx, n->io, n->D_B, n->C, 256));
    FG_TRY(fg_to_user(c, d_img, n->io, (size_t)n->D_B * n->C * 256));
  }
  return FG_OK;
}

int fg_s16_dp_broadcast_params(fg_s16* n) {
  ENTER(n);
  return pair_broadcast(n->c, n->net);
}

int fg_s16_train_step(fg_s16* n, const fg_hyper* h, int B, const float* real, const float* noise_D, const float* noise_G,
                      const float* masks_D, const float* masks_G, uint64_t seed, fg_step_stats* stats) {
  return train_step_iters(n, "fg_s16_train_step", h, B, 1, 1, real, noise_D, noise_G, masks_D, masks_G, seed, stats);
}

int fg_s16_train_step_dataset(fg_s16* n, fg_dataset* d, const fg_hyper* h, int B, uint64_t seed, fg_step_stats* stats) {
  return train_step_dataset_iters(n, d, "fg_s16_train_step_dataset", h, B, 1, 1, seed, stats);
}

int fg_s16_train_step_iters(fg_s16* n, const fg_hyper* h, int B, int d_iters, int g_iters, const float* real,
                            const float* noise_D, const float* noise_G, const float* masks_D, const float* masks_G,
                            uint64_t seed, fg_step_stats* stats) {
  return train_step_iters(n, "fg_s16_train_step_iters", h, B, d_iters, g_iters, real, noise_D, noise_G, masks_D, masks_G, seed,
                          stats);
}

int fg_s16_train_step_dataset_iters(fg_s16* n, fg_dataset* d, const fg_hyper* h, int B, int d_iters, int g_iters,
                                    uint64_t seed, fg_step_stats* stats) {
  return train_step_dataset_iters(n, d, "fg_s16_train_step_dataset_iters", h, B, d_iters, g_iters, seed, stats);
}

int64_t fg_s16_debug_tensor(fg_s16* n, const char* name, float* dst, int64_t max_elems) {
  if (!n || !n->c || !name) {
    fg_set_error("fg_s16_debug_tensor: null argument");
    return -1;
  }
  cudaSetDevice(n->c->device);
  const int db = n->D_B;
  auto d = [&](const float* p) { return n->D_valid ? p : nullptr; };
  std::vector<DebugTensor> ents = {
      {"D.z1", d(n->D_z[0]), 256 * 128, db}, {"D.z2", d(n->D_z[1]), 256 * 128, db}, {"D.z3", d(n->D_z[2]), 16 * 512, db},
      {"D.z4", d(n->D_z[3]), 4 * 1024, db}, {"D.p1", d(n->D_p1), 64 * 128, db}, {"D.zf", d(n->D_zf), 1024, db},
      {"D.ze1", d(n->D_ze1), 128, db}, {"D.ze2", d(n->D_ze2), 128, db}, {"D.logit", d(n->D_logit), 1, db},
      {"D.out", d(n->D_out), 1, db}};
  pair_keep_rows(n->net, ents);
  gen_debug_rows(n->G, ents);
  return debug_tensor_copy(n->c, "fg_s16_debug_tensor", ents.data(), ents.size(), name, dst, max_elems);
}

}
```

Measured before the change: 37370.

## Fuse FP16 operand split and scale into generator BN producer kernels

In FP16 tensor-core mode, the generator's BN+PReLU apply kernels (forward h1, backward dz2/dz1) now write the FP16 hi/lo split directly. The scale pair is computed from per-channel maxima gathered in the BN reduce/finalize kernels. This removes the separate amax and split_h passes and, in training, the FP32 write of the intermediate tensors. It adds per-channel max tracking with shared and global atomics to the reduce kernel, and the FP32 debug tensors are no longer kept during train steps.

```diff
diff --git a/face_generator_b200/csrc/capi.cu b/face_generator_b200/csrc/capi.cu
--- a/face_generator_b200/csrc/capi.cu
+++ b/face_generator_b200/csrc/capi.cu
@@ -55,7 +55,8 @@
     if (strcmp(e.name, name)) continue;
     const int64_t n = e.per * e.B;
     if (!e.p) {
-      fg_set_error("%s: '%s' has not been produced (Dstep.*: option \"debug_keep\" + a train step)", what, name);
+      fg_set_error("%s: '%s' has not been produced (Dstep.*: option \"debug_keep\" + a train step; G.h1, G.dz2, G.dz1: "
+                   "the layer-level G calls, a train step feeds their FP16 split to the tensor cores directly)", what, name);
       return -1;
     }
     if (dst) {
diff --git a/face_generator_b200/csrc/convl.cu b/face_generator_b200/csrc/convl.cu
--- a/face_generator_b200/csrc/convl.cu
+++ b/face_generator_b200/csrc/convl.cu
@@ -34,6 +34,10 @@
 bool convl_tc_bwd(const fg_ctx* c, const ConvL& L) { return tc_f(c, L, 1) && tc_d(c, L, 1); }
 
 int tc_op_split(fg_ctx* c, TcOp& op, const float* x, int64_t n, bool f16) {
+  if (op.f16_ready) {
+    op.f16_ready = false;
+    return FG_OK;
+  }
   if (!f16) {
     if (op.split_ready) {
       op.split_ready = false;
diff --git a/face_generator_b200/csrc/convl.h b/face_generator_b200/csrc/convl.h
--- a/face_generator_b200/csrc/convl.h
+++ b/face_generator_b200/csrc/convl.h
@@ -42,6 +42,6 @@
 
 int gen_alloc(ConvLEnv& e, UpsGen& G, const GenDesc& d);
 int gen_pack(fg_ctx* c, UpsGen& G, NetPair& p);
-int gen_forward(ConvLEnv& e, UpsGen& G, NetPair& p, const float* noise, int B, bool training);
-int gen_backward(ConvLEnv& e, UpsGen& G, NetPair& p, const float* dy, float* dnoise);
+int gen_forward(ConvLEnv& e, UpsGen& G, NetPair& p, const float* noise, int B, bool training, bool keep_fp32);
+int gen_backward(ConvLEnv& e, UpsGen& G, NetPair& p, const float* dy, float* dnoise, bool keep_fp32);
 void gen_debug_rows(const UpsGen& G, std::vector<DebugTensor>& rows);
diff --git a/face_generator_b200/csrc/fg_internal.h b/face_generator_b200/csrc/fg_internal.h
--- a/face_generator_b200/csrc/fg_internal.h
+++ b/face_generator_b200/csrc/fg_internal.h
@@ -116,7 +116,7 @@
 struct TcOp {
   float *hi = nullptr, *lo = nullptr;
   float* s = nullptr;
-  bool split_ready = false, amax_ready = false, bias_ready = false;
+  bool split_ready = false, amax_ready = false, f16_ready = false, bias_ready = false;
 };
 struct ConvL {
   int Cin = 0, Cout = 0, k = 1, H = 1;
@@ -181,6 +181,7 @@
   float *bn_mean[2] = {nullptr, nullptr}, *bn_istd[2] = {nullptr, nullptr}, *bn_mg = nullptr;
   int B = 0;
   bool train = true, valid = false;
+  bool h1_kept = true, dz_kept = true;
   std::deque<std::string> names;
   const char *t_bn2_finalize = nullptr, *t_bn2_stats = nullptr, *t_bn2_apply = nullptr, *t_bn2_bwd_reduce = nullptr,
              *t_bn2_bwd_apply = nullptr;
@@ -292,23 +293,34 @@
 bool k_bn4_ok(int C);
 int k_bn_stats4(fg_ctx* c, const float* z, double* acc, int64_t P, int C);
 int k_bn_bwd_reduce4(fg_ctx* c, const float* dh, const float* z, const float* mean, const float* istd, const float* gamma,
-                     const float* beta, const float* slope, double* acc, float* dslope, int64_t P, int C);
+                     const float* beta, const float* slope, double* acc, float* dslope, int64_t P, int C, bool maxima = false);
+struct BnFwdBound {
+  const float *gamma = nullptr, *beta = nullptr, *slope = nullptr;
+  float* pair = nullptr;
+};
+struct BnBwdBound {
+  const unsigned* chmax = nullptr;
+  const float *gamma = nullptr, *istd = nullptr;
+  float* pair = nullptr;
+};
 int k_bn_finalize(fg_ctx* c, double* acc2C, float* mean, float* istd, float* run_mean, float* run_var, int64_t P,
-                  int C);
+                  int C, BnFwdBound fb = {});
 int k_bn_finalize_parts(fg_ctx* c, const float* part, int nparts, int nphase, float* mean, float* istd, float* run_mean,
-                        float* run_var, int64_t P, int C);
+                        float* run_var, int64_t P, int C, BnFwdBound fb = {});
 int k_bn_eval_prep(fg_ctx* c, const float* run_mean, const float* run_var, float* mean, float* istd, int C);
 int k_bn_prelu_apply(fg_ctx* c, const float* z, const float* mean, const float* istd, const float* gamma,
                      const float* beta, const float* slope, float* h, int64_t P, int C, float* hi = nullptr,
-                     float* lo = nullptr);
+                     float* lo = nullptr, float* f16_pair = nullptr);
 int k_bn_prelu_bwd_reduce(fg_ctx* c, const float* dh, const float* z, const float* mean, const float* istd,
                           const float* gamma, const float* beta, const float* slope, double* acc2C, float* dslope,
-                          int B, int H, int W, int C, int pool);
-int k_bn_bwd_finalize(fg_ctx* c, double* acc2C, float* mg2C, float* dgamma, float* dbeta, int64_t P, int C);
+                          int B, int H, int W, int C, int pool, bool maxima = false);
+int k_bn_bwd_finalize(fg_ctx* c, double* acc2C, float* mg2C, float* dgamma, float* dbeta, int64_t P, int C,
+                      BnBwdBound bb = {});
 int k_bn_prelu_bwd_apply(fg_ctx* c, const float* dh, const float* z, const float* mean, const float* istd,
                          const float* gamma, const float* beta, const float* slope, const float* mg2C, float* dz,
                          int B, int H, int W, int C, int pool, float* hi = nullptr, float* lo = nullptr,
-                         float* dbias = nullptr);
+                         float* dbias = nullptr,
+                         float* f16_pair = nullptr);
 int k_sigmoid_fwd(fg_ctx* c, const float* z, float* y, int64_t n);
 int k_sigmoid_bwd(fg_ctx* c, const float* dy, const float* y, float* dz, int64_t n);
 int k_masks_generate(fg_ctx* c, float* masks, int B, uint64_t seed, float p_spatial, float p_drop,
diff --git a/face_generator_b200/csrc/gen.cu b/face_generator_b200/csrc/gen.cu
--- a/face_generator_b200/csrc/gen.cu
+++ b/face_generator_b200/csrc/gen.cu
@@ -95,24 +95,24 @@
 
 namespace {
 int bn_stats(fg_ctx* c, UpsGen& G, NetPair& p, int i, const float* z, int B, bool training, int parts, const char* t_finalize,
-             const char* t_stats) {
+             const char* t_stats, BnFwdBound fb = {}) {
   const int Cc = G.GU[i].Cout;
   const int64_t P = (int64_t)B * G.GU[i].H * G.GU[i].H;
   float *rm = p.bnG + (i == 0 ? 0 : 512), *rv = rm + Cc;
   if (!training) return k_bn_eval_prep(c, rm, rv, G.bn_mean[i], G.bn_istd[i], Cc);
   if (parts) {
     ScopedTimer tm(c, t_finalize);
-    return k_bn_finalize_parts(c, c->bn_parts, parts, 4, G.bn_mean[i], G.bn_istd[i], rm, rv, P, Cc);
+    return k_bn_finalize_parts(c, c->bn_parts, parts, 4, G.bn_mean[i], G.bn_istd[i], rm, rv, P, Cc, fb);
   }
   {
     ScopedTimer tm(c, t_stats);
     FG_TRY(k_bn_stats(c, z, c->bn_acc, P, Cc));
   }
-  return k_bn_finalize(c, c->bn_acc, G.bn_mean[i], G.bn_istd[i], rm, rv, P, Cc);
-}
-}
-
-int gen_forward(ConvLEnv& e, UpsGen& G, NetPair& p, const float* noise, int B, bool training) {
+  return k_bn_finalize(c, c->bn_acc, G.bn_mean[i], G.bn_istd[i], rm, rv, P, Cc, fb);
+}
+}
+
+int gen_forward(ConvLEnv& e, UpsGen& G, NetPair& p, const float* noise, int B, bool training, bool keep_fp32) {
   fg_ctx* c = e.c;
   FG_REQUIRE(B >= 1 && B <= e.maxB, "G forward: batch %d out of range [1,%d]", B, e.maxB);
   FG_TRY(gen_pack(c, G, p));
@@ -131,10 +131,16 @@
   }
   int parts = training ? 1 : 0;
   FG_TRY(upsl_fwd(e, G.GU[0], G.h0, P, G.z1, B, &parts));
-  FG_TRY(bn_stats(c, G, p, 0, G.z1, B, training, parts, nullptr, nullptr));
   UpsL& C2 = G.GU[1];
   C2.x.split_ready = training && upsl_tc(c, C2) && !tc_f16(c);
-  {
+  C2.x.f16_ready = training && upsl_tc(c, C2) && tc_f16(c);
+  const BnFwdBound fb1{P + L.g1, P + L.be1, P + L.a2, C2.x.s};
+  FG_TRY(bn_stats(c, G, p, 0, G.z1, B, training, parts, nullptr, nullptr, C2.x.f16_ready ? fb1 : BnFwdBound{}));
+  G.h1_kept = keep_fp32 || !C2.x.f16_ready;
+  if (C2.x.f16_ready) {
+    FG_TRY(k_bn_prelu_apply(c, G.z1, G.bn_mean[0], G.bn_istd[0], P + L.g1, P + L.be1, P + L.a2, keep_fp32 ? G.h1 : nullptr,
+                            (int64_t)B * (S / 2) * (S / 2), 256, C2.x.hi, C2.x.lo, C2.x.s));
+  } else {
     AmaxInto am(c, C2.x);
     FG_TRY(k_bn_prelu_apply(c, G.z1, G.bn_mean[0], G.bn_istd[0], P + L.g1, P + L.be1, P + L.a2, G.h1,
                             (int64_t)B * (S / 2) * (S / 2), 256, C2.x.split_ready ? C2.x.hi : nullptr,
@@ -153,7 +159,7 @@
   return FG_OK;
 }
 
-int gen_backward(ConvLEnv& e, UpsGen& G, NetPair& p, const float* dy, float* dnoise) {
+int gen_backward(ConvLEnv& e, UpsGen& G, NetPair& p, const float* dy, float* dnoise, bool keep_fp32) {
   fg_ctx* c = e.c;
   if (!G.valid || !G.train) {
     fg_set_error("G backward needs a preceding training-mode G forward");
@@ -166,35 +172,47 @@
   FG_TRY(G.pairs.reset(c));
   FG_TRY(k_sigmoid_bwd(c, dy, G.y, G.dz3, (int64_t)B * S * S * G.C));
   FG_TRY(convl_bwd(e, G.GC3, G.h2, G.dz3, g, G.dfull, B));
+  const bool tf32 = !tc_f16(c);
+  auto chmax = [c](int C) { return reinterpret_cast<const unsigned*>(c->bn_acc + 2 * C); };
+  TcOp dz2{e.dy.hi, e.dy.lo, G.sdz[1]};
+  dz2.split_ready = upsl_tc(c, G.GU[1]) && tf32;
+  dz2.f16_ready = upsl_tc(c, G.GU[1]) && !tf32;
   {
     ScopedTimer tm(c, G.t_bn2_bwd_reduce);
     FG_TRY(k_bn_prelu_bwd_reduce(c, G.dfull, G.z2, G.bn_mean[1], G.bn_istd[1], P + L.g2, P + L.be2, P + L.a3, c->bn_acc,
-                                 g + L.a3, B, S, S, 128, 0));
-  }
-  FG_TRY(k_bn_bwd_finalize(c, c->bn_acc, G.bn_mg, g + L.g2, g + L.be2, (int64_t)B * S * S, 128));
-  const bool tf32 = !tc_f16(c);
-  TcOp dz2{e.dy.hi, e.dy.lo, G.sdz[1]};
-  dz2.split_ready = upsl_tc(c, G.GU[1]) && tf32;
+                                 g + L.a3, B, S, S, 128, 0, dz2.f16_ready));
+  }
+  const BnBwdBound bb2{chmax(128), P + L.g2, G.bn_istd[1], G.sdz[1]};
+  FG_TRY(k_bn_bwd_finalize(c, c->bn_acc, G.bn_mg, g + L.g2, g + L.be2, (int64_t)B * S * S, 128, dz2.f16_ready ? bb2 : BnBwdBound{}));
   {
     ScopedTimer tm(c, G.t_bn2_bwd_apply);
-    AmaxInto am(c, dz2);
-    FG_TRY(k_bn_prelu_bwd_apply(c, G.dfull, G.z2, G.bn_mean[1], G.bn_istd[1], P + L.g2, P + L.be2, P + L.a3, G.bn_mg, G.dz2,
-                                B, S, S, 128, 0, dz2.split_ready ? dz2.hi : nullptr, dz2.split_ready ? dz2.lo : nullptr,
-                                g + L.C2b));
-  }
+    AmaxInto am(c, dz2.f16_ready ? nullptr : dz2.s, &dz2.amax_ready);
+    FG_TRY(k_bn_prelu_bwd_apply(c, G.dfull, G.z2, G.bn_mean[1], G.bn_istd[1], P + L.g2, P + L.be2, P + L.a3, G.bn_mg,
+                                dz2.f16_ready && !keep_fp32 ? nullptr : G.dz2, B, S, S, 128, 0,
+                                dz2.split_ready || dz2.f16_ready ? dz2.hi : nullptr,
+                                dz2.split_ready || dz2.f16_ready ? dz2.lo : nullptr,
+                                g + L.C2b,
+                                dz2.f16_ready ? dz2.s : nullptr));
+  }
+  const bool dz2_kept = keep_fp32 || !dz2.f16_ready;
   bool pooled = false;
   FG_TRY(upsl_bwd(e, G.GU[1], dz2, G.h1, G.dz2, g, G.dfull, B, &pooled));
-  FG_TRY(k_bn_prelu_bwd_reduce(c, G.dfull, G.z1, G.bn_mean[0], G.bn_istd[0], P + L.g1, P + L.be1, P + L.a2, c->bn_acc,
-                               g + L.a2, B, h, h, 256, pooled ? 0 : 1));
-  FG_TRY(k_bn_bwd_finalize(c, c->bn_acc, G.bn_mg, g + L.g1, g + L.be1, (int64_t)B * h * h, 256));
   TcOp dz1{e.dy.hi, e.dy.lo, G.sdz[0]};
   dz1.split_ready = upsl_tc(c, G.GU[0]) && tf32 && pooled;
-  {
-    AmaxInto am(c, dz1);
-    FG_TRY(k_bn_prelu_bwd_apply(c, G.dfull, G.z1, G.bn_mean[0], G.bn_istd[0], P + L.g1, P + L.be1, P + L.a2, G.bn_mg, G.dz1,
-                                B, h, h, 256, pooled ? 0 : 1, dz1.split_ready ? dz1.hi : nullptr,
-                                dz1.split_ready ? dz1.lo : nullptr, g + L.C1b));
-  }
+  dz1.f16_ready = upsl_tc(c, G.GU[0]) && !tf32 && pooled;
+  FG_TRY(k_bn_prelu_bwd_reduce(c, G.dfull, G.z1, G.bn_mean[0], G.bn_istd[0], P + L.g1, P + L.be1, P + L.a2, c->bn_acc,
+                               g + L.a2, B, h, h, 256, pooled ? 0 : 1, dz1.f16_ready));
+  const BnBwdBound bb1{chmax(256), P + L.g1, G.bn_istd[0], G.sdz[0]};
+  FG_TRY(k_bn_bwd_finalize(c, c->bn_acc, G.bn_mg, g + L.g1, g + L.be1, (int64_t)B * h * h, 256, dz1.f16_ready ? bb1 : BnBwdBound{}));
+  {
+    AmaxInto am(c, dz1.f16_ready ? nullptr : dz1.s, &dz1.amax_ready);
+    FG_TRY(k_bn_prelu_bwd_apply(c, G.dfull, G.z1, G.bn_mean[0], G.bn_istd[0], P + L.g1, P + L.be1, P + L.a2, G.bn_mg,
+                                dz1.f16_ready && !keep_fp32 ? nullptr : G.dz1, B, h, h, 256, pooled ? 0 : 1,
+                                dz1.split_ready || dz1.f16_ready ? dz1.hi : nullptr,
+                                dz1.split_ready || dz1.f16_ready ? dz1.lo : nullptr, g + L.C1b,
+                                dz1.f16_ready ? dz1.s : nullptr));
+  }
+  G.dz_kept = dz2_kept && (keep_fp32 || !dz1.f16_ready);
   FG_TRY(upsl_bwd(e, G.GU[0], dz1, G.h0, G.dz1, g, G.dfull, B, &pooled));
   {
     AmaxInto am(c, G.GL1.sdy, &e.dy.amax_ready);
@@ -206,10 +224,13 @@
 void gen_debug_rows(const UpsGen& G, std::vector<DebugTensor>& rows) {
   const int64_t n0 = G.GL1.Cout, n1 = 256 * (G.S / 2) * (G.S / 2), n2 = 128 * G.S * G.S, n3 = (int64_t)G.C * G.S * G.S;
   const int B = G.B;
+  const float *h1 = G.h1_kept ? G.h1 : nullptr, *dz2 = G.dz_kept ? G.dz2 : nullptr, *dz1 = G.dz_kept ? G.dz1 : nullptr;
   for (const DebugTensor& r : {DebugTensor{"G.z0", G.z0, n0, B}, {"G.h0", G.h0, n0, B}, {"G.z1", G.z1, n1, B},
-                               {"G.h1", G.h1, n1, B}, {"G.z2", G.z2, n2, B}, {"G.h2", G.h2, n2, B}, {"G.z3", G.z3, n3, B},
-                               {"G.y", G.y, n3, B}, {"G.dz2", G.dz2, n2, B}, {"G.dz1", G.dz1, n1, B}, {"G.dz0", G.dz0, n0, B},
+                               {"G.h1", h1, n1, B}, {"G.z2", G.z2, n2, B}, {"G.h2", G.h2, n2, B}, {"G.z3", G.z3, n3, B},
+                               {"G.y", G.y, n3, B}, {"G.dz2", dz2, n2, B}, {"G.dz1", dz1, n1, B}, {"G.dz0", G.dz0, n0, B},
                                {"G.bn_mean1", G.bn_mean[0], 256, 1}, {"G.bn_istd1", G.bn_istd[0], 256, 1},
-                               {"G.bn_mean2", G.bn_mean[1], 128, 1}, {"G.bn_istd2", G.bn_istd[1], 128, 1}})
+                               {"G.bn_mean2", G.bn_mean[1], 128, 1}, {"G.bn_istd2", G.bn_istd[1], 128, 1},
+                               {"G.h1.hi", G.GU[1].x.hi, n1 / 2, B}, {"G.h1.lo", G.GU[1].x.lo, n1 / 2, B},
+                               {"G.h1.s", G.GU[1].x.s, 2, 1}, {"G.dz2.s", G.sdz[1], 2, 1}, {"G.dz1.s", G.sdz[0], 2, 1}})
     rows.push_back({r.name, G.valid ? r.p : nullptr, r.per, r.B});
 }
diff --git a/face_generator_b200/csrc/k_bn.cu b/face_generator_b200/csrc/k_bn.cu
--- a/face_generator_b200/csrc/k_bn.cu
+++ b/face_generator_b200/csrc/k_bn.cu
@@ -1,4 +1,5 @@
 #include "fg_internal.h"
+#include "k_f16split.cuh"
 #include "k_ordered.cuh"
 
 namespace {
@@ -9,7 +10,7 @@
                                                          const float* __restrict__ slope, double* __restrict__ acc,
                                                          float* __restrict__ dslope, int64_t P, int C,
                                                          int64_t rows_per_block, double* __restrict__ ws,
-                                                         unsigned* __restrict__ ticket) {
+                                                         unsigned* __restrict__ ticket, unsigned* __restrict__ chmax) {
   extern __shared__ double sm[];
   const int C4 = C >> 2;
   const int lanes = blockDim.x / C4;
@@ -19,6 +20,7 @@
   const float4* z4 = reinterpret_cast<const float4*>(z);
   const float4* d4 = reinterpret_cast<const float4*>(dh);
   double s[4] = {0, 0, 0, 0}, q[4] = {0, 0, 0, 0}, ss = 0;
+  float gx[4] = {0.f, 0.f, 0.f, 0.f}, xx[4] = {0.f, 0.f, 0.f, 0.f};
   float m[4], is[4], ga[4], be[4];
   float a = 1.f;
   bool act = false;
@@ -64,6 +66,8 @@
         }
         s[j] += (double)g;
         q[j] += (double)g * (double)xh;
+        gx[j] = fmaxf(gx[j], finite_abs(g));
+        xx[j] = fmaxf(xx[j], finite_abs(xh));
       }
     };
     if (BWD) {
@@ -122,6 +126,24 @@
       if (threadIdx.x == 0) row[2 * C] = v;
     }
   }
+  if (BWD && chmax) {
+    __syncthreads();
+    unsigned* mx = reinterpret_cast<unsigned*>(sm);
+    for (int i = threadIdx.x; i < 2 * C; i += blockDim.x) mx[i] = 0u;
+    __syncthreads();
+    if (lane < lanes) {
+#pragma unroll
+      for (int j = 0; j < 4; ++j) {
+        atomicMax(mx + ch + j, __float_as_uint(gx[j]));
+        atomicMax(mx + C + ch + j, __float_as_uint(xx[j]));
+      }
+    }
+    __syncthreads();
+    for (int i = threadIdx.x; i < 2 * C; i += blockDim.x) {
+      const unsigned v = mx[i];
+      if (v > *reinterpret_cast<volatile unsigned*>(chmax + i)) atomicMax(chmax + i, v);
+    }
+  }
   if (ordered_last_block(ticket)) {
     for (int i = threadIdx.x; i < 2 * C; i += blockDim.x) acc[i] += ordered_sum(ws, gridDim.x, 2 * C + 1, i);
     if (BWD && dslope && threadIdx.x == 0) *dslope += (float)ordered_sum(ws, gridDim.x, 2 * C + 1, 2 * C);
@@ -141,20 +163,22 @@
   FG_TRY(red_check(c, grid, 2 * C + 1));
   bn_reduce4_kernel<false><<<grid, 256, sizeof(double) * 2 * lanes * C, c->stream>>>(z, nullptr, nullptr, nullptr, nullptr, nullptr,
                                                                                    nullptr, acc, nullptr, P, C, rpb, c->red_ws,
-                                                                                   c->red_ticket);
+                                                                                   c->red_ticket, nullptr);
   LAUNCH_CHECK(c);
   return FG_OK;
 }
 int k_bn_bwd_reduce4(fg_ctx* c, const float* dh, const float* z, const float* mean, const float* istd, const float* gamma,
-                     const float* beta, const float* slope, double* acc, float* dslope, int64_t P, int C) {
-  FG_CUDA(cudaMemsetAsync(acc, 0, sizeof(double) * 2 * C, c->stream));
+                     const float* beta, const float* slope, double* acc, float* dslope, int64_t P, int C, bool maxima) {
+  unsigned* chmax = maxima ? reinterpret_cast<unsigned*>(acc + 2 * C) : nullptr;
+  FG_CUDA(cudaMemsetAsync(acc, 0, sizeof(double) * 2 * C + (maxima ? sizeof(unsigned) * 2 * C : 0), c->stream));
   const int lanes = 256 / (C / 4);
   int grid = (int)std::min<int64_t>((int64_t)c->sm_count * 8, (P + lanes * 4 - 1) / (lanes * 4));
   if (grid < 1) grid = 1;
   const int64_t rpb = (P + grid - 1) / grid;
   FG_TRY(red_check(c, grid, 2 * C + 1));
   bn_reduce4_kernel<true><<<grid, 256, sizeof(double) * 2 * lanes * C, c->stream>>>(z, dh, mean, istd, gamma, beta, slope, acc,
-                                                                                  dslope, P, C, rpb, c->red_ws, c->red_ticket);
+                                                                                  dslope, P, C, rpb, c->red_ws, c->red_ticket,
+                                                                                  chmax);
   LAUNCH_CHECK(c);
   return FG_OK;
 }
diff --git a/face_generator_b200/csrc/k_elem.cu b/face_generator_b200/csrc/k_elem.cu
--- a/face_generator_b200/csrc/k_elem.cu
+++ b/face_generator_b200/csrc/k_elem.cu
@@ -4,6 +4,30 @@
 #include "fg_internal.h"
 #include "k_f16split.cuh"
 #include "k_ordered.cuh"
+
+namespace {
+__device__ __forceinline__ void bound_commit(float* pair, float b) {
+  b = finite_abs(b) * (1.f + 1.f / 1024.f);
+  if (pair && b > 0.f) atomicMax(reinterpret_cast<unsigned*>(pair), __float_as_uint(b));
+}
+__device__ __forceinline__ float bn_prelu_fwd_bound(const float* gamma, const float* beta, const float* slope, int ch,
+                                                    int64_t P) {
+  const float a = slope ? fmaxf(1.f, fabsf(*slope)) : 1.f;
+  return a * (fabsf(gamma[ch]) * sqrtf((float)(P - 1)) + fabsf(beta[ch]));
+}
+__device__ __forceinline__ void store_split_h4(const float (&o)[4], float s, float* hi, float* lo, int64_t i) {
+  __half h[4], l[4];
+#pragma unroll
+  for (int j = 0; j < 4; ++j) split_f16(o[j] * s, h[j], l[j]);
+  reinterpret_cast<uint2*>(hi)[i] = *reinterpret_cast<uint2*>(h);
+  reinterpret_cast<uint2*>(lo)[i] = *reinterpret_cast<uint2*>(l);
+}
+__device__ __forceinline__ float pair_scale(float* pair) {
+  const float s = scale_for_amax(pair[0]);
+  if (blockIdx.x == 0 && threadIdx.x == 0) pair[1] = 1.f / s;
+  return s;
+}
+}
 
 __device__ __forceinline__ int perm_idx(int j, int A, int S) {
   if (A == 0) return j;
@@ -262,9 +286,11 @@
   return FG_OK;
 }
 __global__ void bn_finalize_kernel(const double* __restrict__ acc, float* __restrict__ mean, float* __restrict__ istd,
-                                   float* __restrict__ run_mean, float* __restrict__ run_var, int64_t P, int C) {
+                                   float* __restrict__ run_mean, float* __restrict__ run_var, int64_t P, int C,
+                                   BnFwdBound fb) {
   const int ch = blockIdx.x * blockDim.x + threadIdx.x;
   if (ch >= C) return;
+  if (fb.pair) bound_commit(fb.pair, bn_prelu_fwd_bound(fb.gamma, fb.beta, fb.slope, ch, P));
   const double n = (double)P;
   const double m = acc[ch] / n;
   double var = acc[C + ch] / n - m * m;
@@ -274,8 +300,9 @@
   if (run_mean) run_mean[ch] = 0.9f * run_mean[ch] + 0.1f * (float)m;
   if (run_var) run_var[ch] = 0.9f * run_var[ch] + 0.1f * (float)(P > 1 ? var * n / (n - 1.0) : var);
 }
-int k_bn_finalize(fg_ctx* c, double* acc, float* mean, float* istd, float* run_mean, float* run_var, int64_t P, int C) {
-  bn_finalize_kernel<<<(C + 127) / 128, 128, 0, c->stream>>>(acc, mean, istd, run_mean, run_var, P, C);
+int k_bn_finalize(fg_ctx* c, double* acc, float* mean, float* istd, float* run_mean, float* run_var, int64_t P, int C,
+                  BnFwdBound fb) {
+  bn_finalize_kernel<<<(C + 127) / 128, 128, 0, c->stream>>>(acc, mean, istd, run_mean, run_var, P, C, fb);
   LAUNCH_CHECK(c);
   return FG_OK;
 }
@@ -288,7 +315,8 @@
                                                                 double* __restrict__ slice_acc,
                                                                 unsigned int* __restrict__ ticket, float* __restrict__ mean,
                                                                 float* __restrict__ istd, float* __restrict__ run_mean,
-                                                                float* __restrict__ run_var, int64_t P, int C) {
+                                                                float* __restrict__ run_var, int64_t P, int C,
+                                                                BnFwdBound fb) {
   __shared__ double sm[4][8][32];
   __shared__ bool last;
   const int lane = threadIdx.x & 31, g = threadIdx.x >> 5;
@@ -348,13 +376,14 @@
   istd[ch] = (float)(1.0 / sqrt(var + 1e-5));
   if (run_mean) run_mean[ch] = 0.9f * run_mean[ch] + 0.1f * (float)m;
   if (run_var) run_var[ch] = 0.9f * run_var[ch] + 0.1f * (float)(P > 1 ? var * n / (n - 1.0) : var);
+  if (fb.pair) bound_commit(fb.pair, bn_prelu_fwd_bound(fb.gamma, fb.beta, fb.slope, ch, P));
 }
 int k_bn_finalize_parts(fg_ctx* c, const float* part, int nparts, int nphase, float* mean, float* istd, float* run_mean,
-                        float* run_var, int64_t P, int C) {
+                        float* run_var, int64_t P, int C, BnFwdBound fb) {
   double* acc = c->bn_slice_acc;
   unsigned int* ticket = reinterpret_cast<unsigned int*>(acc + (size_t)kBnSlices * 4 * 256);
   bn_finalize_parts_kernel<<<dim3((C + 31) / 32, kBnSlices), 256, 0, c->stream>>>(part, nparts, nphase, acc, ticket, mean, istd,
-                                                                                run_mean, run_var, P, C);
+                                                                                run_mean, run_var, P, C, fb);
   LAUNCH_CHECK(c);
   return FG_OK;
 }
@@ -374,8 +403,9 @@
                                       const float* __restrict__ istd, const float* __restrict__ gamma,
                                       const float* __restrict__ beta, const float* __restrict__ slope,
                                       float* __restrict__ h, float* __restrict__ hi, float* __restrict__ lo, int64_t n4,
-                                      int C, unsigned* __restrict__ amax) {
+                                      int C, unsigned* __restrict__ amax, float* __restrict__ f16_pair) {
   float am = 0.f;
+  const float sc = f16_pair ? pair_scale(f16_pair) : 1.f;
   const bool act = slope != nullptr;
   const float a = act ? *slope : 1.f;
   const float4* z4 = reinterpret_cast<const float4*>(z);
@@ -402,7 +432,9 @@
     }
     if (h) h4[i] = o;
     am = amax4(am, o.x, o.y, o.z, o.w);
-    if (hi) {
+    if (f16_pair) {
+      store_split_h4({o.x, o.y, o.z, o.w}, sc, hi, lo, i);
+    } else if (hi) {
       float4 vh, vl;
       vh.x = __uint_as_float((__float_as_uint(o.x) + 0x1000u) & 0xFFFFE000u);
       vh.y = __uint_as_float((__float_as_uint(o.y) + 0x1000u) & 0xFFFFE000u);
@@ -429,13 +461,14 @@
   }
 }
 int k_bn_prelu_apply(fg_ctx* c, const float* z, const float* mean, const float* istd, const float* gamma,
-                     const float* beta, const float* slope, float* h, int64_t P, int C, float* hi, float* lo) {
+                     const float* beta, const float* slope, float* h, int64_t P, int C, float* hi, float* lo,
+                     float* f16_pair) {
   const int64_t n = P * C;
   if (C % 4 == 0) {
     bn_prelu_apply_kernel<<<grid_for(n / 4, 256), 256, 0, c->stream>>>(z, mean, istd, gamma, beta, slope, h, hi, lo, n / 4, C,
-                                                                       take_amax(c));
+                                                                       f16_pair ? nullptr : take_amax(c), f16_pair);
   } else {
-    if (hi || !h) {
+    if (hi || !h || f16_pair) {
       fg_set_error("bn_prelu_apply: hi/lo outputs need C %% 4 == 0");
       return FG_ERR_UNSUPPORTED;
     }
@@ -503,9 +536,14 @@
 }
 int k_bn_prelu_bwd_reduce(fg_ctx* c, const float* dh, const float* z, const float* mean, const float* istd,
                           const float* gamma, const float* beta, const float* slope, double* acc, float* dslope, int B,
-                          int H, int W, int C, int pool) {
+                          int H, int W, int C, int pool, bool maxima) {
+  FG_REQUIRE(!maxima || C <= 256, "bn_prelu_bwd_reduce: per-channel maxima of %d channels do not fit behind the sums", C);
   if (!pool && k_bn4_ok(C))
-    return k_bn_bwd_reduce4(c, dh, z, mean, istd, gamma, beta, slope, acc, dslope, (int64_t)B * H * W, C);
+    return k_bn_bwd_reduce4(c, dh, z, mean, istd, gamma, beta, slope, acc, dslope, (int64_t)B * H * W, C, maxima);
+  if (maxima) {
+    fg_set_error("bn_prelu_bwd_reduce: per-channel maxima need the un-pooled float4 path");
+    return FG_ERR_UNSUPPORTED;
+  }
   if (C > 1024) return FG_ERR_UNSUPPORTED;
   FG_CUDA(cudaMemsetAsync(acc, 0, sizeof(double) * 2 * C, c->stream));
   const int64_t P = (int64_t)B * H * W;
@@ -521,16 +559,21 @@
   return FG_OK;
 }
 __global__ void bn_bwd_finalize_kernel(const double* __restrict__ acc, float* __restrict__ mg, float* __restrict__ dgamma,
-                                       float* __restrict__ dbeta, int64_t P, int C) {
+                                       float* __restrict__ dbeta, int64_t P, int C, BnBwdBound bb) {
   const int ch = blockIdx.x * blockDim.x + threadIdx.x;
   if (ch >= C) return;
-  mg[ch] = (float)(acc[ch] / (double)P);
-  mg[C + ch] = (float)(acc[C + ch] / (double)P);
+  const float m1 = (float)(acc[ch] / (double)P), m2 = (float)(acc[C + ch] / (double)P);
+  mg[ch] = m1;
+  mg[C + ch] = m2;
   if (dgamma) dgamma[ch] += (float)acc[C + ch];
   if (dbeta) dbeta[ch] += (float)acc[ch];
-}
-int k_bn_bwd_finalize(fg_ctx* c, double* acc, float* mg, float* dgamma, float* dbeta, int64_t P, int C) {
-  bn_bwd_finalize_kernel<<<(C + 127) / 128, 128, 0, c->stream>>>(acc, mg, dgamma, dbeta, P, C);
+  if (bb.pair) {
+    const float gmax = __uint_as_float(bb.chmax[ch]), xmax = __uint_as_float(bb.chmax[C + ch]);
+    bound_commit(bb.pair, fabsf(bb.gamma[ch]) * bb.istd[ch] * (gmax + fabsf(m1) + xmax * fabsf(m2)));
+  }
+}
+int k_bn_bwd_finalize(fg_ctx* c, double* acc, float* mg, float* dgamma, float* dbeta, int64_t P, int C, BnBwdBound bb) {
+  bn_bwd_finalize_kernel<<<(C + 127) / 128, 128, 0, c->stream>>>(acc, mg, dgamma, dbeta, P, C, bb);
   LAUNCH_CHECK(c);
   return FG_OK;
 }
@@ -588,8 +631,9 @@
                                            const float* __restrict__ slope, const float* __restrict__ mg,
                                            float* __restrict__ dz, float* __restrict__ hi, float* __restrict__ lo,
                                            float* __restrict__ dbias, int64_t n4, int C, unsigned* __restrict__ amax,
-                                           double* __restrict__ ws, unsigned* __restrict__ ticket) {
+                                           double* __restrict__ ws, unsigned* __restrict__ ticket, float* __restrict__ f16_pair) {
   float am = 0.f;
+  const float sc = f16_pair ? pair_scale(f16_pair) : 1.f;
   float bs[4] = {0.f, 0.f, 0.f, 0.f};
   const bool act = slope != nullptr;
   const float a = act ? *slope : 1.f;
@@ -615,10 +659,12 @@
       }
       o[j] = ga * is * (g - mg[ch + j] - xh * mg[C + ch + j]);
     }
-    dz4[i] = make_float4(o[0], o[1], o[2], o[3]);
+    if (dz) dz4[i] = make_float4(o[0], o[1], o[2], o[3]);
     am = amax4(am, o[0], o[1], o[2], o[3]);
     bs[0] += o[0]; bs[1] += o[1]; bs[2] += o[2]; bs[3] += o[3];
-    if (hi) {
+    if (f16_pair) {
+      store_split_h4(o, sc, hi, lo, i);
+    } else if (hi) {
       float h[4];
 #pragma unroll
       for (int j = 0; j < 4; ++j) h[j] = __uint_as_float((__float_as_uint(o[j]) + 0x1000u) & 0xFFFFE000u);
@@ -631,17 +677,18 @@
 }
 int k_bn_prelu_bwd_apply(fg_ctx* c, const float* dh, const float* z, const float* mean, const float* istd,
                          const float* gamma, const float* beta, const float* slope, const float* mg, float* dz, int B,
-                         int H, int W, int C, int pool, float* hi, float* lo, float* dbias) {
+                         int H, int W, int C, int pool, float* hi, float* lo, float* dbias, float* f16_pair) {
   const int64_t n = (int64_t)B * H * W * C;
   if (!pool && C % 4 == 0 && C <= 1024 && 256 % (C / 4) == 0) {
     const int grid = grid_for(n / 4, 256);
     FG_TRY(red_check(c, grid, C));
     bn_prelu_bwd_apply4_kernel<<<grid, 256, 0, c->stream>>>(dh, z, mean, istd, gamma, beta, slope, mg, dz, hi, lo, dbias, n / 4,
-                                                           C, take_amax(c), c->red_ws, c->red_ticket);
+                                                           C, f16_pair ? nullptr : take_amax(c), c->red_ws, c->red_ticket,
+                                                           f16_pair);
     LAUNCH_CHECK(c);
     return FG_OK;
   }
-  if (hi) {
+  if (hi || f16_pair || !dz) {
     fg_set_error("bn_prelu_bwd_apply: hi/lo outputs need the un-pooled float4 path");
     return FG_ERR_UNSUPPORTED;
   }
diff --git a/face_generator_b200/csrc/nets.cu b/face_generator_b200/csrc/nets.cu
--- a/face_generator_b200/csrc/nets.cu
+++ b/face_generator_b200/csrc/nets.cu
@@ -246,7 +246,7 @@
         real(real), noiseD(noiseD), noiseG(noiseG) {}
   int g_forward(int j, bool d_iter) override {
     const int rows = d_iter ? B / 2 : B;
-    return gen_forward(n->env, n->G, n->net, (d_iter ? noiseD : noiseG) + (size_t)j * rows * kNoiseDim, rows, true);
+    return gen_forward(n->env, n->G, n->net, (d_iter ? noiseD : noiseG) + (size_t)j * rows * kNoiseDim, rows, true, false);
   }
   int d_input(int j) override {
     const int Bh = B / 2;
@@ -260,7 +260,7 @@
   }
   int d_forward(bool on_g) override { return D_forward(n, on_g ? n->G.y : n->D_x, B, true, h); }
   int d_backward(bool want_wgrad, bool want_dx) override { return D_backward(n, n->D_dlogit, want_wgrad, want_dx); }
-  int g_backward() override { return gen_backward(n->env, n->G, n->net, n->D_dx, nullptr); }
+  int g_backward() override { return gen_backward(n->env, n->G, n->net, n->D_dx, nullptr, false); }
 };
 }
 
@@ -417,7 +417,7 @@
   n->net.G_pack = -1;
   const float* nd;
   FG_TRY(fg_to_dev(c, noise, (size_t)B * kNoiseDim, n->in_noiseG, &nd));
-  FG_TRY(gen_forward(n->env, n->G, n->net, nd, B, training != 0));
+  FG_TRY(gen_forward(n->env, n->G, n->net, nd, B, training != 0, true));
   if (images_out) {
     FG_TRY(k_nhwc_to_nchw(c, n->G.y, c->io_dev, B, c->C, 1024));
     FG_TRY(fg_to_user(c, images_out, c->io_dev, (size_t)B * c->C * 1024));
@@ -434,7 +434,7 @@
   FG_TRY(k_nchw_to_nhwc(c, dd, n->io_dev2, B, c->C, 1024));
   float* dn = nullptr;
   if (d_noise) dn = fg_is_dev(d_noise) ? d_noise : n->in_noiseD;
-  FG_TRY(gen_backward(n->env, n->G, n->net, n->io_dev2, dn));
+  FG_TRY(gen_backward(n->env, n->G, n->net, n->io_dev2, dn, true));
   if (d_noise && dn != d_noise) FG_TRY(fg_to_user(c, d_noise, dn, (size_t)B * kNoiseDim));
   return FG_OK;
 }
@@ -530,7 +530,7 @@
     const int b = std::min(chunk, N - s);
     const float* nd;
     FG_TRY(fg_to_dev(c, noise + (size_t)s * kNoiseDim, (size_t)b * kNoiseDim, n->in_noiseG, &nd));
-    FG_TRY(gen_forward(n->env, n->G, n->net, nd, b, true));
+    FG_TRY(gen_forward(n->env, n->G, n->net, nd, b, true, true));
     float* dst = images_out + (size_t)s * img;
     if (out_dev) {
       FG_TRY(k_nhwc_to_nchw(c, n->G.y, dst, b, c->C, 1024));
diff --git a/face_generator_b200/csrc/nets_s16.cu b/face_generator_b200/csrc/nets_s16.cu
--- a/face_generator_b200/csrc/nets_s16.cu
+++ b/face_generator_b200/csrc/nets_s16.cu
@@ -333,7 +333,7 @@
         noiseD(noiseD), noiseG(noiseG) {}
   int g_forward(int j, bool d_iter) override {
     const int rows = d_iter ? B / 2 : B;
-    return gen_forward(n->env, n->G, n->net, (d_iter ? noiseD : noiseG) + (size_t)j * rows * 100, rows, true);
+    return gen_forward(n->env, n->G, n->net, (d_iter ? noiseD : noiseG) + (size_t)j * rows * 100, rows, true, false);
   }
   int d_input(int j) override {
     const int Bh = B / 2;
@@ -347,7 +347,7 @@
   }
   int d_forward(bool on_g) override { return D_forward(n, on_g ? n->G.y : n->D_x, B, true); }
   int d_backward(bool want_wgrad, bool want_dx) override { return D_backward(n, n->D_dlogit, want_wgrad, want_dx); }
-  int g_backward() override { return gen_backward(n->env, n->G, n->net, n->D_dx, nullptr); }
+  int g_backward() override { return gen_backward(n->env, n->G, n->net, n->D_dx, nullptr, false); }
 };
 
 }
@@ -493,7 +493,7 @@
   FG_REQUIRE(noise && B >= 1 && B <= n->maxB, "fg_s16_G_forward: bad arguments (batch %d, max %d)", B, n->maxB);
   const float* nd;
   FG_TRY(fg_to_dev(n->c, noise, (size_t)B * 100, n->in_b, &nd));
-  FG_TRY(gen_forward(n->env, n->G, n->net, nd, B, training != 0));
+  FG_TRY(gen_forward(n->env, n->G, n->net, nd, B, training != 0, true));
   if (img_out) {
     FG_TRY(k_nhwc_to_nchw(n->c, n->G.y, n->io, B, n->C, 256));
     FG_TRY(fg_to_user(n->c, img_out, n->io, (size_t)B * n->C * 256));
@@ -506,7 +506,7 @@
   const float* dd;
   FG_TRY(fg_to_dev(n->c, d_img, (size_t)n->G.B * n->C * 256, n->in_a, &dd));
   FG_TRY(k_nchw_to_nhwc(n->c, dd, n->io, n->G.B, n->C, 256));
-  FG_TRY(gen_backward(n->env, n->G, n->net, n->io, d_noise ? n->in_c : nullptr));
+  FG_TRY(gen_backward(n->env, n->G, n->net, n->io, d_noise ? n->in_c : nullptr, true));
   if (d_noise) FG_TRY(fg_to_user(n->c, d_noise, n->in_c, (size_t)n->G.B * 100));
   return FG_OK;
 }
diff --git a/profiles/operand_split.py b/profiles/operand_split.py
--- /dev/null
+++ b/profiles/operand_split.py
@@ -0,0 +1,109 @@
+import argparse
+import json
+import os
+import re
+import subprocess
+import sys
+from collections import defaultdict
+
+import numpy as np
+
+sys.path.insert(0, os.path.dirname(os.path.dirname(os.path.abspath(__file__))))
+
+SPLIT = ("split_h_kernel", "amax_kernel")
+PRODUCERS = ("bn_prelu_apply_kernel", "bn_prelu_bwd_apply4_kernel", "bn_reduce4_kernel", "bn_finalize_parts_kernel",
+             "bn_bwd_finalize_kernel", "d_act_pool_fwd_kernel", "d_act_pool_bwd_kernel", "lin_act_drop_fwd_kernel",
+             "lin_act_drop_bwd_kernel", "prelu_fwd_kernel", "prelu_bwd_kernel")
+
+
+def gpu_info():
+    try:
+        out = subprocess.run(["nvidia-smi", "--query-gpu=name,power.limit,clocks.max.sm", "--format=csv,noheader"],
+                             capture_output=True, text=True, timeout=30).stdout.strip().splitlines()
+        return out[0] if out else "unknown"
+    except (OSError, subprocess.SubprocessError):
+        return "unknown"
+
+
+def base_name(name):
+    s = name.replace("(anonymous namespace)::", "")
+    s = re.sub(r"\(.*$", "", s)
+    s = re.sub(r"<.*>$", "", s)
+    return s.split("::")[-1].split()[-1]
+
+
+def main():
+    ap = argparse.ArgumentParser()
+    ap.add_argument("--batch", type=int, default=256)
+    ap.add_argument("--steps", type=int, default=20)
+    ap.add_argument("--warmup", type=int, default=10)
+    ap.add_argument("--trace", default=None, help="directory for the Chrome trace of the profiled steps")
+    args = ap.parse_args()
+    import torch
+    from torch.profiler import ProfilerActivity, profile
+
+    import face_generator_b200 as fg
+    from face_generator_b200 import layouts as LY
+    from face_generator_b200.lib import NET_D, NET_G
+    B, C, K = args.batch, 3, args.steps
+    rng = np.random.default_rng(1)
+    ctx = fg.Context(0, max_batch=B, channels=C)
+    ctx.set_params(NET_G, LY.trained_like_init(LY.G_layout(C), rng))
+    ctx.set_params(NET_D, LY.trained_like_init(LY.D_layout(C), rng, 1.4))
+    f = lambda a: np.ascontiguousarray(a, np.float32)
+    real = ctx.dev_array(f(rng.random((B // 2, C, 32, 32))))
+    nD, nG = ctx.dev_array(f(rng.uniform(-1, 1, (B // 2, 100)))), ctx.dev_array(f(rng.uniform(-1, 1, (B, 100))))
+    h = fg.hyper_default()
+    seed = [0]
+
+    def step():
+        seed[0] += 1
+        ctx.train_step(h, B, real, nD, nG, None, None, seed[0], want_stats=False)
+
+    for _ in range(args.warmup):
+        step()
+    ctx.sync()
+    l0 = ctx.launches()
+    ctx.event_record(0)
+    for _ in range(K):
+        step()
+    ctx.event_record(1)
+    ctx.sync()
+    step_ms = ctx.event_elapsed_ms(0, 1) / K
+    launches = (ctx.launches() - l0) / K
+
+    torch.cuda.init()
+    with profile(activities=[ProfilerActivity.CUDA]) as prof:
+        for _ in range(K):
+            step()
+        ctx.sync()
+    ctx.close()
+    per = defaultdict(lambda: [0.0, 0])
+    for ev in prof.events():
+        if ev.device_type == torch.autograd.DeviceType.CUDA and ev.device_time_total > 0:
+            n = base_name(ev.name)
+            per[n][0] += ev.device_time_total
+            per[n][1] += 1
+    if args.trace:
+        os.makedirs(args.trace, exist_ok=True)
+        prof.export_chrome_trace(os.path.join(args.trace, "operand_split.pt.trace.json"))
+    kern_us = sum(v[0] for v in per.values()) / K
+    row = lambda n: {"us_per_step": round(per[n][0] / K, 2), "launches_per_step": per[n][1] / K} if n in per else None
+    split = {n: row(n) for n in SPLIT}
+    prod = {n: row(n) for n in PRODUCERS}
+    split_us = sum(v["us_per_step"] for v in split.values() if v)
+    prod_us = sum(v["us_per_step"] for v in prod.values() if v)
+    top = sorted(per.items(), key=lambda kv: -kv[1][0])[:25]
+    out = {"gpu": gpu_info(), "batch": B, "steps": K,
+           "step_ms_events": round(step_ms, 4), "launches_per_step": launches,
+           "kernel_us_per_step_profiled": round(kern_us, 1),
+           "split_pass": split, "split_pass_us_per_step": round(split_us, 1),
+           "split_pass_share_of_step": round(split_us / (step_ms * 1e3), 4),
+           "producers": prod, "producers_us_per_step": round(prod_us, 1),
+           "split_plus_producers_us_per_step": round(split_us + prod_us, 1),
+           "top_kernels_us_per_step": [(n, round(v[0] / K, 1), v[1] / K) for n, v in top]}
+    print(json.dumps(out, indent=1))
+
+
+if __name__ == "__main__":
+    main()
```

Result: faster. 38390 (median of 6 runs) (+2.7%).
